# OminiX-ai/OminiX-MLX

Measured on AMD Instinct MI355X. Metric: decode_tokens_per_sec, higher is better.
Workload: dtype bf16

## Files before the change

ominix-mlx_amd/csrc/attn.hpp:

```cpp
#pragma once
#include "common.hpp"

namespace omx {

struct AttnDecodeArgs {
    const bf16_t* q;
    const bf16_t* k;
    const bf16_t* v;
    int64_t kv_batch_stride, kv_head_stride;
    int B, H, Hkv, Tk;
    float scale;
    int mask_mode;
    const void* mask;
    int nsplit;
    float* ws_o;
    float* ws_ml;
    bf16_t* out;
    int64_t q_bs, q_hs;
    int causal_tail;
};

constexpr int kAttnTraceWords = 16;
struct AttnStepArgs {
    const bf16_t* qkv;
    bf16_t* k;
    bf16_t* v;
    int64_t kv_head_stride;
    int H, Hkv, cap;
    float scale, eps;
    const bf16_t* q_norm_w;
    const bf16_t* k_norm_w;
    const float* rope_cur;
    const int* pos_ptr;
    const unsigned* seq_ptr;
    unsigned tag_mul, tag_add;
    int chunk;
    int nsplit;
    uint64_t* ws;
    bf16_t* out;
    unsigned* abort_flag;
    unsigned long long* trace;
    const bf16_t* o_w;
    const bf16_t* o_resid;
    bf16_t* o_out;
    float* o_out_f32;
    int o_rows;
    int o_rpw, o_nhi;
    uint64_t* xg;
    const uint32_t* o_wq;
    const uint32_t* o_sb;
    int o_group;
    int f16;
    const bf16_t* gu_gate;
    const bf16_t* gu_up;
    const bf16_t* gu_norm_w;
    bf16_t* gu_out;
    int gu_rows;
    uint64_t* hg;
};
bool attn_step_oproj_ok(int H, int Hkv, int D, int nsplit, int o_rows);
bool attn_step_gateup_ok(int H, int Hkv, int D, int nsplit, int o_rows, int gu_rows);
bool attn_step_oproj_q4_ok(int H, int Hkv, int D, int nsplit, int o_rows, int group);
int attn_step_block_tokens(int D);
void attn_step_plan(int tk_max, int Hkv, int G, int D, int* chunk, int* nsplit);
size_t attn_step_ws_granules(int H, int D);
int launch_attn_step(const AttnStepArgs& a, int D, hipStream_t s);

size_t attn_decode_ws_bytes(int BH, int nsplit, int D);
int decode_nsplit(int Tk, int BHkv);
int launch_attn_decode(const AttnDecodeArgs& a, int D, hipStream_t s);

}
```

ominix-mlx_amd/csrc/attn_step.hip:

```cpp
#include <algorithm>

#include "attn.hpp"
#include "act16.hpp"
#include "gemv_parts.hpp"
#include "granule.hpp"
#include "launch_timing.hpp"

namespace omx {

namespace {

constexpr int kBlock = 512;
constexpr int kWaves = 8;
constexpr unsigned kSpinLimit = 1u << 15;

template <int N>
__device__ __forceinline__ float swap_halves(float v) {
    if (N == 16) return dpp_f<0x128>(v);
    return dpp_f<0x1B>(dpp_f<kDppHalfMirror>(v));
}

template <bool F16 = false>
__device__ __forceinline__ void unpack8(const u32x4 r, float (&x)[8]) {
#pragma unroll
    for (int e = 0; e < 4; ++e) {
        x[2 * e] = Act16<F16>::lo(r[e]);
        x[2 * e + 1] = Act16<F16>::hi(r[e]);
    }
}

template <int D, int NB, bool F16 = false>
__device__ __forceinline__ void gather_head(const AttnStepArgs& a, const uint64_t* base, int n_active, unsigned tag, int lane,
                                            int dim, bf16_t* out, uint64_t* xg_head) {
    constexpr int STRIDE = D + 2;
    unsigned long long ml0 = 0, ml1 = 0, og[NB][16];
    bool ok_ml = false, ok_b[NB];
#pragma unroll
    for (int b = 0; b < NB; ++b) ok_b[b] = b * 16 >= n_active;
    const int sl = min(lane, n_active - 1);
    for (unsigned spins = 0;; ++spins) {
        if (!ok_ml) {
            ml0 = ld_granule(base + (size_t)sl * STRIDE + D);
            ml1 = ld_granule(base + (size_t)sl * STRIDE + D + 1);
        }
#pragma unroll
        for (int b = 0; b < NB; ++b) {
            if (ok_b[b]) continue;
#pragma unroll
            for (int j = 0; j < 16; ++j) og[b][j] = ld_granule(base + (size_t)min(b * 16 + j, n_active - 1) * STRIDE + dim);
        }
        bool all = true;
        if (!ok_ml) ok_ml = __all((unsigned)(ml0 >> 32) == tag && (unsigned)(ml1 >> 32) == tag);
        all = ok_ml;
#pragma unroll
        for (int b = 0; b < NB; ++b) {
            if (!ok_b[b]) {
                bool ok = true;
#pragma unroll
                for (int j = 0; j < 16; ++j) ok &= (unsigned)(og[b][j] >> 32) == tag;
                ok_b[b] = __all(ok);
            }
            all = all && ok_b[b];
        }
        if (all) break;
        if (spins >= kSpinLimit) {
            if (lane == 0) __hip_atomic_store(a.abort_flag, 1u, __ATOMIC_RELAXED, __HIP_MEMORY_SCOPE_AGENT);
            break;
        }
        __builtin_amdgcn_s_sleep(1);
    }
    const float m = lane < n_active ? __uint_as_float((unsigned)ml0) : -INFINITY;
    const float l = lane < n_active ? __uint_as_float((unsigned)ml1) : 0.f;
    const float M = wave_max(m);
    const float f = (m == -INFINITY) ? 0.f : __expf(m - M);
    const float L = wave_sum(f * l);
    float acc = 0.f;
#pragma unroll
    for (int b = 0; b < NB; ++b) {
        if (b * 16 >= n_active) break;
#pragma unroll
        for (int j = 0; j < 16; ++j)
            acc = fmaf(readlane_f(f, b * 16 + j), __uint_as_float((unsigned)og[b][j]), acc);
    }
    const bf16_t r = Act16<F16>::bits(acc / L);
    out[dim] = r;
    if (xg_head) {
        const float nb = dpp_f<kDppXor1>(bf16_to_f32(r));
        if (!(lane & 1)) st_granule_u32(xg_head + dim / 2, tag, (unsigned)r | ((unsigned)f32_to_bf16(nb) << 16));
    }
}

typedef __attribute__((ext_vector_type(2))) __bf16 bf16x2_t;
typedef __attribute__((ext_vector_type(2))) float f32x2;

typedef __attribute__((ext_vector_type(8))) __bf16 bf16x8_t;
__device__ __forceinline__ float dot8_bf16(const u32x4 a, const u32x4 b) {
    const bf16x8_t A = __builtin_bit_cast(bf16x8_t, a), B = __builtin_bit_cast(bf16x8_t, b);
    float d = 0.f;
    d = __builtin_amdgcn_fdot2_f32_bf16(__builtin_shufflevector(A, A, 0, 1), __builtin_shufflevector(B, B, 0, 1), d, false);
    d = __builtin_amdgcn_fdot2_f32_bf16(__builtin_shufflevector(A, A, 2, 3), __builtin_shufflevector(B, B, 2, 3), d, false);
    d = __builtin_amdgcn_fdot2_f32_bf16(__builtin_shufflevector(A, A, 4, 5), __builtin_shufflevector(B, B, 4, 5), d, false);
    d = __builtin_amdgcn_fdot2_f32_bf16(__builtin_shufflevector(A, A, 6, 7), __builtin_shufflevector(B, B, 6, 7), d, false);
    return d;
}

constexpr int kKU = 3;

template <bool F16>
__device__ __forceinline__ float dot8_16(const u32x4 a, const u32x4 b) {
    if constexpr (!F16) return dot8_bf16(a, b);
    float d = 0.f;
#pragma unroll
    for (int e = 0; e < 4; ++e) d = Act16<true>::dot2(a[e], b[e], d);
    return d;
}

__device__ __forceinline__ float dot8_chain(const u32x4 w, const u32x4 xp, float acc) {
#pragma unroll
    for (int i = 0; i < 4; ++i) {
        acc = fmaf(bf16lo(w[i]), bf16lo(xp[i]), acc);
        acc = fmaf(bf16hi(w[i]), bf16hi(xp[i]), acc);
    }
    return acc;
}

constexpr int kORows = 4;

constexpr int kGuBlockPairs = 48, kGuHidden = 4096, kGuNV = kGuHidden / 512;
enum { kGuTicket = 0, kGuReduced = 1, kGuWords = 4 };

__device__ __forceinline__ int gateup_claim(int* sm_gu, int lane) {
    int t = 0;
    if (lane == 0) t = __hip_atomic_fetch_add(sm_gu + kGuTicket, 1, __ATOMIC_RELAXED, __HIP_MEMORY_SCOPE_WORKGROUP);
    return __builtin_amdgcn_readfirstlane(t);
}

__device__ __forceinline__ void gateup_issue(const AttnStepArgs& a, u32x4 (*w)[kGuNV], int pair, int lane) {
    const u32x4* g = reinterpret_cast<const u32x4*>(a.gu_gate + (size_t)pair * kGuHidden);
    const u32x4* u = reinterpret_cast<const u32x4*>(a.gu_up + (size_t)pair * kGuHidden);
#pragma unroll
    for (int j = 0; j < kGuNV; ++j) {
        w[0][j] = ld_nt(g + j * 64 + lane);
        w[1][j] = ld_nt(u + j * 64 + lane);
    }
    __builtin_amdgcn_sched_barrier(0);
}

template <int NVW>
__device__ __forceinline__ void oproj_await_vector(const AttnStepArgs& a, u32x4* sm_x, unsigned tag, int lane, int wave) {
    asm volatile("s_waitcnt vmcnt(0)" ::: "memory");
    if (wave == 0) {
        constexpr int SEGS = NVW * 8;
        const uint64_t* probe = a.xg + (size_t)min(lane, SEGS - 1) * 32 + 31;
        for (unsigned spins = 0; spins < kSpinLimit; ++spins) {
            const unsigned long long g = ld_granule(probe);
            if (__all((unsigned)(g >> 32) == tag)) break;
            __builtin_amdgcn_s_sleep(4);
        }
    }
    __syncthreads();
    constexpr int GP = (NVW + 1) / 2;
    static_assert((NVW * 256) % GP == 0, "a thread takes all of its granules or none");
    bool done = (int)threadIdx.x * GP >= NVW * 256;
    unsigned* sx = reinterpret_cast<unsigned*>(sm_x);
    for (unsigned spins = 0;; ++spins) {
        if (!done) {
            unsigned long long g[GP];
#pragma unroll
            for (int i = 0; i < GP; ++i) g[i] = ld_granule(a.xg + (size_t)threadIdx.x * GP + i);
            bool ok = true;
#pragma unroll
            for (int i = 0; i < GP; ++i) ok &= (unsigned)(g[i] >> 32) == tag;
            if (ok) {
#pragma unroll
                for (int i = 0; i < GP; ++i) sx[threadIdx.x * GP + i] = (unsigned)g[i];
                done = true;
            }
        }
        if (__syncthreads_and(done)) break;
        if (spins >= kSpinLimit) {
            if (threadIdx.x == 0) __hip_atomic_store(a.abort_flag, 1u, __ATOMIC_RELAXED, __HIP_MEMORY_SCOPE_AGENT);
            break;
        }
        __builtin_amdgcn_s_sleep(2);
    }
}

__device__ __forceinline__ void gateup_reduce(const AttnStepArgs& a, const u32x4 (*w)[kGuNV], const u32x4* xs, int pair, int lane) {
    typedef Act16<false> A;
    float acc[2] = {0.f, 0.f};
#pragma unroll
    for (int j = 0; j < kGuNV; ++j) {
        const u32x4 xp = xs[j * 64 + lane];
        float xf[8];
#pragma unroll
        for (int q = 0; q < 4; ++q) {
            xf[2 * q] = A::lo(xp[q]);
            xf[2 * q + 1] = A::hi(xp[q]);
        }
#pragma unroll
        for (int r = 0; r < 2; ++r) acc[r] = dot8(w[r][j], xf, acc[r]);
    }
#pragma unroll
    for (int r = 0; r < 2; ++r) acc[r] = wave_sum(acc[r]);
    if (lane == 0) a.gu_out[pair] = epi_bits<EPI_SWIGLU, A>(acc[0], acc[1], (bf16_t)0, 0);
}

template <bool TRACE>
__device__ __forceinline__ void gateup_phase(const AttnStepArgs& a, u32x4* xs, float* red, int* sm_gu, const uint16_t* sm_pub, unsigned tag,
                                             int lane, int wave, int pub_row0, int pub_rows, unsigned long long* tr) {
    typedef Act16<false> A;
    const int pair0 = ((int)blockIdx.y * (int)gridDim.x + (int)blockIdx.x) * kGuBlockPairs;
    constexpr int PV = kGuNV * 64 / 256;
    u32x4 nwv[PV];
#pragma unroll
    for (int i = 0; i < PV; ++i) nwv[i] = *(reinterpret_cast<const u32x4*>(a.gu_norm_w) + (threadIdx.x & 255) + i * 256);
    u32x4 wA[2][kGuNV], wB[2][kGuNV];
    int tA = 0, tB;
    if (wave != 0) {
        tA = gateup_claim(sm_gu, lane);
        gateup_issue(a, wA, pair0 + tA, lane);
    }
    lds_barrier();
    if (wave == 0) {
        if (lane < pub_rows / 2) st_granule_u32(a.hg + pub_row0 / 2 + lane, tag, reinterpret_cast<const unsigned*>(sm_pub)[lane]);
        constexpr int GPL = kGuHidden / 2 / 64;
        for (unsigned spins = 0; spins < kSpinLimit; ++spins) {
            const unsigned long long g = ld_granule(a.hg + (size_t)lane * GPL + (GPL - 1));
            if (__all((unsigned)(g >> 32) == tag)) break;
            __builtin_amdgcn_s_sleep(4);
        }
        unsigned long long g[GPL];
#pragma unroll
        for (int i = 0; i < GPL; ++i) g[i] = ld_granule(a.hg + (size_t)i * 64 + lane);
        __builtin_amdgcn_sched_barrier(0);
        lds_barrier();
        tA = gateup_claim(sm_gu, lane);
        gateup_issue(a, wA, pair0 + tA, lane);
        unsigned bad = 0;
#pragma unroll
        for (int i = 0; i < GPL; ++i) bad |= (unsigned)(g[i] >> 32) ^ tag;
        asm volatile("; hidden row: tags read behind the first (gate, up) pair" : "+v"(bad));
        if (!__all(bad == 0)) {
            for (unsigned spins = 0;; ++spins) {
#pragma unroll
                for (int i = 0; i < GPL; ++i) g[i] = ld_granule(a.hg + (size_t)i * 64 + lane);
                bool ok = true;
#pragma unroll
                for (int i = 0; i < GPL; ++i) ok &= (unsigned)(g[i] >> 32) == tag;
                if (__all(ok)) break;
                if (spins >= kSpinLimit) {
                    if (lane == 0) __hip_atomic_store(a.abort_flag, 1u, __ATOMIC_RELAXED, __HIP_MEMORY_SCOPE_AGENT);
                    break;
                }
                __builtin_amdgcn_s_sleep(4);
            }
        }
        unsigned* sx = reinterpret_cast<unsigned*>(xs);
#pragma unroll
        for (int i = 0; i < GPL; ++i) sx[i * 64 + lane] = (unsigned)g[i];
        if (TRACE && lane == 0 && pub_rows > 0) tr[4] = wall_clock64();
        tB = gateup_claim(sm_gu, lane);
    } else {
        lds_barrier();
        tB = gateup_claim(sm_gu, lane);
        gateup_issue(a, wB, pair0 + tB, lane);
    }
    lds_barrier();
    rmsnorm_in_lds<A, PV>(xs, red, nwv, kGuHidden, a.eps, threadIdx.x < 256);
    if (wave == 0) {
        gateup_issue(a, wB, pair0 + tB, lane);
        gateup_reduce(a, wA, xs, pair0 + tA, lane);
        if (TRACE && threadIdx.x == 0) tr[7] = wall_clock64();
        asm volatile("; first pair reduced: wave 0, its second pair just asked for" ::: "memory");
    } else {
        gateup_reduce(a, wA, xs, pair0 + tA, lane);
        asm volatile("; first pair reduced: the second pair came in through the hop" ::: "memory");
    }
    int n_reduced = 1;
    int nA = gateup_claim(sm_gu, lane), nB;
    for (;;) {
        if (nA >= kGuBlockPairs) {
            gateup_reduce(a, wB, xs, pair0 + tB, lane);
            ++n_reduced;
            break;
        }
        tA = nA;
        gateup_issue(a, wA, pair0 + tA, lane);
        nB = gateup_claim(sm_gu, lane);
        gateup_reduce(a, wB, xs, pair0 + tB, lane);
        if (nB >= kGuBlockPairs) {
            gateup_reduce(a, wA, xs, pair0 + tA, lane);
            n_reduced += 2;
            break;
        }
        tB = nB;
        gateup_issue(a, wB, pair0 + tB, lane);
        nA = gateup_claim(sm_gu, lane);
        gateup_reduce(a, wA, xs, pair0 + tA, lane);
        n_reduced += 2;
    }
    if constexpr (TRACE) {
        if (lane == 0) {
            __hip_atomic_fetch_add(sm_gu + kGuReduced, n_reduced, __ATOMIC_RELAXED, __HIP_MEMORY_SCOPE_WORKGROUP);
            if (wave == 0) tr[8] = wall_clock64();
            if (wave == kWaves - 1) tr[9] = wall_clock64();
        }
        lds_barrier();
        if (threadIdx.x == 0) tr[10] = (unsigned long long)sm_gu[kGuReduced];
    }
}

template <int NVW, int R, bool GU = false>
__device__ __forceinline__ void oproj_phase(const AttnStepArgs& a, u32x4* sm_x, unsigned tag, int lane, int wave, int o_row0,
                                            unsigned long long* tr, uint16_t* sm_pub = nullptr, int pub_row0 = 0) {
    u32x4 ow[R][NVW];
#pragma unroll
    for (int r = 0; r < R; ++r) {
        const int row = min(o_row0 + r, a.o_rows - 1);
        const u32x4* p = reinterpret_cast<const u32x4*>(a.o_w + (size_t)row * (NVW * 512));
#pragma unroll
        for (int j = 0; j < NVW; ++j) ow[r][j] = __builtin_nontemporal_load(p + j * 64 + lane);
    }
    bf16_t o_res[R];
#pragma unroll
    for (int r = 0; r < R; ++r) o_res[r] = a.o_resid[min(o_row0 + r, a.o_rows - 1)];
    __builtin_amdgcn_sched_barrier(0);
    oproj_await_vector<NVW>(a, sm_x, tag, lane, wave);
    if (tr && threadIdx.x == 0) tr[5] = wall_clock64();
    float acc[R];
#pragma unroll
    for (int r = 0; r < R; ++r) acc[r] = 0.f;
#pragma unroll
    for (int j = 0; j < NVW; ++j) {
        const u32x4 xp = sm_x[j * 64 + lane];
#pragma unroll
        for (int r = 0; r < R; ++r) acc[r] = dot8_chain(ow[r][j], xp, acc[r]);
    }
#pragma unroll
    for (int r = 0; r < R; ++r) acc[r] = wave_sum(acc[r]);
    if (lane == 0) {
#pragma unroll
        for (int r = 0; r < R; ++r)
            if (o_row0 + r < a.o_rows) {
                if (a.o_out_f32) a.o_out_f32[o_row0 + r] = acc[r];
                else {
                    const bf16_t hb = f32_to_bf16(bf16_to_f32(o_res[r]) + round_bf16(acc[r]));
                    a.o_out[o_row0 + r] = hb;
                    if (GU) sm_pub[o_row0 + r - pub_row0] = hb;
                }
            }
    }
    if (tr && threadIdx.x == 0) tr[6] = wall_clock64();
}


template <int NVW, int R>
__device__ __forceinline__ void oproj_phase_q4(const AttnStepArgs& a, u32x4* sm_x, float* sm_xsum, unsigned tag, int lane, int wave,
                                               int o_row0, unsigned long long* tr) {
    static_assert(NVW % 4 == 0, "K must be a multiple of 2048");
    constexpr int ST = NVW / 4;
    u32x4 ow[R][ST];
    uint32_t sbv[R][ST];
    const int words_per_row = NVW * 64, groups_per_row = NVW * 512 / a.o_group;
#pragma unroll
    for (int r = 0; r < R; ++r) {
        const int row = min(o_row0 + r, a.o_rows - 1);
        const uint32_t* p = a.o_wq + (size_t)row * words_per_row;
        const uint32_t* psb = a.o_sb + (size_t)row * groups_per_row;
#pragma unroll
        for (int st = 0; st < ST; ++st) {
            const int chunk = st * 64 + lane;
            ow[r][st] = __builtin_nontemporal_load(reinterpret_cast<const u32x4*>(p + (size_t)chunk * 4));
            sbv[r][st] = psb[chunk * 32 / a.o_group];
        }
    }
    bf16_t o_res[R];
#pragma unroll
    for (int r = 0; r < R; ++r) o_res[r] = a.o_resid[min(o_row0 + r, a.o_rows - 1)];
    __builtin_amdgcn_sched_barrier(0);
    oproj_await_vector<NVW>(a, sm_x, tag, lane, wave);
    if ((int)threadIdx.x < NVW * 64) {
        const u32x4 o = sm_x[threadIdx.x];
        u32x4 t;
        t[0] = __builtin_amdgcn_perm(o[1], o[0], 0x05040100u); t[1] = __builtin_amdgcn_perm(o[3], o[2], 0x05040100u);
        t[2] = __builtin_amdgcn_perm(o[1], o[0], 0x07060302u); t[3] = __builtin_amdgcn_perm(o[3], o[2], 0x07060302u);
        sm_x[threadIdx.x] = t;
        float sv = 0.f;
#pragma unroll
        for (int q = 0; q < 4; ++q) sv += bf16lo(o[q]) + bf16hi(o[q]);
        sv += dpp_f<kDppXor1>(sv);
        sv += dpp_f<kDppXor2>(sv);
        if ((threadIdx.x & 3) == 0) sm_xsum[threadIdx.x >> 2] = sv;
    }
    __syncthreads();
    if (tr && threadIdx.x == 0) tr[5] = wall_clock64();
    float acc[R];
#pragma unroll
    for (int r = 0; r < R; ++r) acc[r] = 0.f;
#pragma unroll
    for (int st = 0; st < ST; ++st) {
        const int chunk = st * 64 + lane;
        uint32_t xp[16];
#pragma unroll
        for (int j = 0; j < 4; ++j) {
            const u32x4 xv = sm_x[chunk * 4 + j];
#pragma unroll
            for (int q = 0; q < 4; ++q) xp[j * 4 + q] = xv[q];
        }
        const float xsm = sm_xsum[chunk];
#pragma unroll
        for (int r = 0; r < R; ++r) {
            float d = 0.f;
            const float scl = bf16lo(sbv[r][st]);
            float bia = bf16hi(sbv[r][st]);
#pragma unroll
            for (int wi = 0; wi < 4; ++wi) {
                const uint32_t wdw = ow[r][st][wi];
                const uint32_t lo = wdw & 0x0F0F0F0Fu, hi = (wdw >> 4) & 0x0F0F0F0Fu;
                const uint32_t c43 = 0x43434343u;
                const uint32_t q0 = __builtin_amdgcn_perm(c43, lo, 0x04010400u), q1 = __builtin_amdgcn_perm(c43, lo, 0x04030402u);
                const uint32_t q2 = __builtin_amdgcn_perm(c43, hi, 0x04010400u), q3 = __builtin_amdgcn_perm(c43, hi, 0x04030402u);
                d = __builtin_amdgcn_fdot2_f32_bf16(__builtin_bit_cast(bf16x2_t, xp[wi * 4 + 0]), __builtin_bit_cast(bf16x2_t, q0), d, false);
                d = __builtin_amdgcn_fdot2_f32_bf16(__builtin_bit_cast(bf16x2_t, xp[wi * 4 + 1]), __builtin_bit_cast(bf16x2_t, q1), d, false);
                d = __builtin_amdgcn_fdot2_f32_bf16(__builtin_bit_cast(bf16x2_t, xp[wi * 4 + 2]), __builtin_bit_cast(bf16x2_t, q2), d, false);
                d = __builtin_amdgcn_fdot2_f32_bf16(__builtin_bit_cast(bf16x2_t, xp[wi * 4 + 3]), __builtin_bit_cast(bf16x2_t, q3), d, false);
            }
            bia = fmaf(-128.0f, scl, bia);
            acc[r] = fmaf(scl, d, acc[r]);
            acc[r] = fmaf(bia, xsm, acc[r]);
        }
    }
#pragma unroll
    for (int r = 0; r < R; ++r) acc[r] = wave_sum(acc[r]);
    if (lane == 0) {
#pragma unroll
        for (int r = 0; r < R; ++r)
            if (o_row0 + r < a.o_rows) a.o_out[o_row0 + r] = f32_to_bf16(bf16_to_f32(o_res[r]) + round_bf16(acc[r]));
    }
    if (tr && threadIdx.x == 0) tr[6] = wall_clock64();
}


template <int D, int GT, bool TRACE, int NVW, bool F16 = false, bool GU = false>
__global__ __launch_bounds__(kBlock, 1) void attn_step_kernel(const AttnStepArgs a) {
    static_assert(!F16 || NVW == 0, "the O projection rides in the launch for bfloat16 models only");
    static_assert(!GU || (NVW == kGuNV && D == 128), "gate/up follows the bf16 O projection of hidden 4096 only");
    typedef Act16<F16> A16;
    constexpr int LPR = D / 8;
    constexpr int TPW = 64 / LPR;
    constexpr bool QO = NVW >= 100;
    constexpr int NV = QO ? NVW - 100 : NVW;
    constexpr bool OPROJ = NV > 0;
    extern __shared__ __attribute__((aligned(16))) unsigned char smem[];
    float* sm_o = reinterpret_cast<float*>(smem);
    float* sm_m = sm_o + kWaves * TPW * GT * D;
    float* sm_l = sm_m + kWaves * GT;
    u32x4* sm_q = reinterpret_cast<u32x4*>(sm_l + kWaves * GT);
    u32x4* sm_x = sm_q + (GT + 1) * LPR;
    float* sm_xsum = reinterpret_cast<float*>(sm_x + NV * 64);
    int* sm_gu = reinterpret_cast<int*>(sm_x + NV * 64);

    const int lane = threadIdx.x & 63;
    const int wave = threadIdx.x >> 6;
    const int c = lane % LPR;
    const int sg = lane / LPR;
    const int kvh = blockIdx.x, split = blockIdx.y;
    const int G = a.H / a.Hkv;
    unsigned long long* tr = TRACE ? a.trace + ((size_t)split * a.Hkv + kvh) * kAttnTraceWords : nullptr;
    if (TRACE && threadIdx.x == 0) tr[0] = wall_clock64();
    if constexpr (GU) {
        if (threadIdx.x < kGuWords) sm_gu[threadIdx.x] = 0;
    }

    bf16_t* Kb = a.k + (size_t)kvh * a.kv_head_stride;
    bf16_t* Vb = a.v + (size_t)kvh * a.kv_head_stride;
    const int t_begin = split * a.chunk;
    const int n_units = a.chunk / TPW;

    const bf16_t* kraw = a.qkv + (size_t)a.H * D + (size_t)kvh * D;
    const bool does_q = wave < GT, does_k = wave == GT % kWaves;
    const bf16_t* my_raw = does_q ? a.qkv + (size_t)(kvh * G + min(wave, G - 1)) * D : kraw;
    const u32x4 raw0 = *reinterpret_cast<const u32x4*>(my_raw + c * 8);
    const u32x4 raw1 = *reinterpret_cast<const u32x4*>(kraw + c * 8);
    const u32x4 vnew = *reinterpret_cast<const u32x4*>(kraw + (size_t)a.Hkv * D + c * 8);
    const int i0 = (c % (LPR / 2)) * 8;
    const f32x4* cp = reinterpret_cast<const f32x4*>(a.rope_cur + i0);
    const f32x4* sp = reinterpret_cast<const f32x4*>(a.rope_cur + D / 2 + i0);
    const f32x4 c0 = cp[0], c1 = cp[1], s0 = sp[0], s1 = sp[1];
    u32x4 wq_raw = {0, 0, 0, 0}, wk_raw = {0, 0, 0, 0};
    if (a.q_norm_w) {
        wq_raw = *reinterpret_cast<const u32x4*>(a.q_norm_w + c * 8);
        wk_raw = *reinterpret_cast<const u32x4*>(a.k_norm_w + c * 8);
    }
    u32x4 kr[kKU], vr[kKU];
    auto issue_kv = [&](int u0) {
#pragma unroll
        for (int u = 0; u < kKU; ++u) {
            const int tc = min(t_begin + (u0 + u * kWaves) * TPW + sg, a.cap - 1);
            kr[u] = *reinterpret_cast<const u32x4*>(Kb + (size_t)tc * D + c * 8);
            vr[u] = *reinterpret_cast<const u32x4*>(Vb + (size_t)tc * D + c * 8);
        }
    };
    issue_kv(wave);
    const int pos = *a.pos_ptr;
    const unsigned tag = *a.seq_ptr * a.tag_mul + a.tag_add;

    {
        float cs[8], sn[8];
#pragma unroll
        for (int e = 0; e < 4; ++e) {
            cs[e] = c0[e]; cs[4 + e] = c1[e];
            sn[e] = s0[e]; sn[4 + e] = s1[e];
        }
        const bool first_half = c < LPR / 2;
        auto norm_rope = [&](const u32x4 raw, const u32x4 w_raw) -> u32x4 {
            float x[8], w[8];
            unpack8<F16>(raw, x);
            unpack8<F16>(w_raw, w);
            float ss = 0.f;
#pragma unroll
            for (int e = 0; e < 8; ++e) ss = fmaf(x[e], x[e], ss);
            ss = group_sum<LPR>(ss);
            const float rstd = a.q_norm_w ? 1.0f / sqrtf(ss / (float)D + a.eps) : 1.0f;
            float y[8];
#pragma unroll
            for (int e = 0; e < 8; ++e) {
                const float xn = a.q_norm_w ? A16::rnd(x[e] * rstd * w[e]) : x[e];
                const float other = swap_halves<LPR>(xn);
                y[e] = first_half ? xn * cs[e] - other * sn[e] : other * sn[e] + xn * cs[e];
            }
            u32x4 out;
#pragma unroll
            for (int e = 0; e < 4; ++e) out[e] = A16::pack(y[2 * e], y[2 * e + 1]);
            return out;
        };
        if (does_q && sg == 0) sm_q[wave * LPR + c] = norm_rope(raw0, wq_raw);
        if (does_k && sg == 0) sm_q[GT * LPR + c] = norm_rope(does_q ? raw1 : raw0, wk_raw);
    }
    asm volatile("s_waitcnt lgkmcnt(0)\n\ts_barrier" ::: "memory");
    u32x4 q[GT];
#pragma unroll
    for (int g = 0; g < GT; ++g) q[g] = sm_q[g * LPR + c];
    const u32x4 knew = sm_q[GT * LPR + c];

    const int Tk = pos + 1;
    const int n_active = (Tk + a.chunk - 1) / a.chunk;
    const int t_end = min(Tk, t_begin + a.chunk);
    const bool active = split < n_active;
    if (TRACE && threadIdx.x == 0) tr[1] = wall_clock64();

    float m[GT], l[GT];
    f32x2 o[GT][4];
#pragma unroll
    for (int g = 0; g < GT; ++g) {
        m[g] = -INFINITY;
        l[g] = 0.f;
#pragma unroll
        for (int e = 0; e < 4; ++e) o[g][e] = f32x2{0.f, 0.f};
    }
    auto round = [&](const int u0) {
        float s[kKU][GT];
        f32x2 vf[kKU][4];
#pragma unroll
        for (int u = 0; u < kKU; ++u) {
            const int unit = u0 + u * kWaves;
            const int tok = t_begin + unit * TPW + sg;
            const bool live = unit < n_units && tok < t_end;
            u32x4 kp = kr[u], vp = vr[u];
            if (tok == pos && unit < n_units) {
                kp = knew;
                vp = vnew;
                *reinterpret_cast<u32x4*>(Kb + (size_t)pos * D + c * 8) = kp;
                *reinterpret_cast<u32x4*>(Vb + (size_t)pos * D + c * 8) = vp;
            }
#pragma unroll
            for (int e = 0; e < 4; ++e)
                vf[u][e] = live ? f32x2{A16::lo(vp[e]), A16::hi(vp[e])} : f32x2{0.f, 0.f};
#pragma unroll
            for (int g = 0; g < GT; ++g) {
                const float d = group_sum<LPR>(dot8_16<F16>(q[g], kp)) * a.scale;
                s[u][g] = live ? d : -INFINITY;
            }
        }
        if (u0 + kWaves * kKU < n_units && t_begin + (u0 + kWaves * kKU) * TPW < t_end) issue_kv(u0 + kWaves * kKU);
#pragma unroll
        for (int g = 0; g < GT; ++g) {
            float mx = s[0][g];
#pragma unroll
            for (int u = 1; u < kKU; ++u) mx = fmaxf(mx, s[u][g]);
            float wmx = readlane_f(mx, 0);
#pragma unroll
            for (int r = 1; r < TPW; ++r) wmx = fmaxf(wmx, readlane_f(mx, r * LPR));
            const float mn = fmaxf(m[g], wmx);
            const float alpha = (mn == -INFINITY) ? 1.f : __expf(m[g] - mn);
            m[g] = mn;
            l[g] *= alpha;
            const f32x2 al = {alpha, alpha};
#pragma unroll
            for (int e = 0; e < 4; ++e) o[g][e] *= al;
#pragma unroll
            for (int u = 0; u < kKU; ++u) {
                const float p = (mn == -INFINITY) ? 0.f : __expf(s[u][g] - mn);
                l[g] += p;
                const f32x2 pp = {p, p};
#pragma unroll
                for (int e = 0; e < 4; ++e) o[g][e] = __builtin_elementwise_fma(pp, vf[u][e], o[g][e]);
            }
        }
    };
    if (wave < n_units && t_begin + wave * TPW < t_end) round(wave);
    for (int u0 = wave + kWaves * kKU; u0 < n_units && t_begin + u0 * TPW < t_end; u0 += kWaves * kKU) round(u0);
    if (TRACE && threadIdx.x == 0) tr[2] = wall_clock64();

    if (active) {
#pragma unroll
        for (int g = 0; g < GT; ++g) {
            float* dst = sm_o + (((size_t)(wave * TPW + sg) * GT + g) * D + c * 8);
            *reinterpret_cast<f32x4*>(dst) = f32x4{o[g][0][0], o[g][0][1], o[g][1][0], o[g][1][1]};
            *reinterpret_cast<f32x4*>(dst + 4) = f32x4{o[g][2][0], o[g][2][1], o[g][3][0], o[g][3][1]};
            float lw = readlane_f(l[g], 0);
#pragma unroll
            for (int r = 1; r < TPW; ++r) lw += readlane_f(l[g], r * LPR);
            if (lane == 0) {
                sm_m[wave * GT + g] = m[g];
                sm_l[wave * GT + g] = lw;
            }
        }
        __syncthreads();
        if (TRACE && !GU && threadIdx.x == 0) tr[7] = wall_clock64();
        for (int idx = threadIdx.x; idx < G * D; idx += kBlock) {
            const int g = idx / D, d = idx % D;
            float M = sm_m[g];
#pragma unroll
            for (int w = 1; w < kWaves; ++w) M = fmaxf(M, sm_m[w * GT + g]);
            float L = 0.f, O = 0.f;
#pragma unroll
            for (int w = 0; w < kWaves; ++w) {
                const float mw = sm_m[w * GT + g];
                const float f = (mw == -INFINITY) ? 0.f : __expf(mw - M);
                float ow = 0.f;
#pragma unroll
                for (int r = 0; r < TPW; ++r) ow += sm_o[((size_t)(w * TPW + r) * GT + g) * D + d];
                L = fmaf(f, sm_l[w * GT + g], L);
                O = fmaf(f, ow, O);
            }
            uint64_t* gr = a.ws + ((size_t)(kvh * G + g) * a.nsplit + split) * (D + 2);
            st_granule(gr + d, tag, O);
            if (d == 0) {
                st_granule(gr + D, tag, M);
                st_granule(gr + D + 1, tag, L);
            }
        }
    }
    if (TRACE && threadIdx.x == 0) tr[3] = wall_clock64();

    if (OPROJ && split >= G) {
        const int g = ((split - G) * (int)gridDim.x + kvh) * kWaves + wave;
        const bool hi = g < a.o_nhi;
        const int rows = hi ? a.o_rpw : a.o_rpw - 1;
        const int o_row0 = hi ? g * a.o_rpw : a.o_nhi * a.o_rpw + (g - a.o_nhi) * (a.o_rpw - 1);
        unsigned long long* otr = TRACE ? tr : nullptr;
        if constexpr (GU) {
            auto row0_of = [&](int w) { return w < a.o_nhi ? w * a.o_rpw : a.o_nhi * a.o_rpw + (w - a.o_nhi) * (a.o_rpw - 1); };
            const int pub_row0 = row0_of(g - wave), pub_rows = row0_of(g - wave + kWaves) - pub_row0;
            uint16_t* sm_pub = reinterpret_cast<uint16_t*>(sm_l);
            if (rows == 2) oproj_phase<NV, 2, true>(a, sm_x, tag, lane, wave, o_row0, otr, sm_pub, pub_row0);
            else oproj_phase<NV, 3, true>(a, sm_x, tag, lane, wave, o_row0, otr, sm_pub, pub_row0);
            gateup_phase<TRACE>(a, sm_x, sm_m, sm_gu, sm_pub, tag, lane, wave, pub_row0, pub_rows, otr);
            return;
        } else
        if constexpr (QO) {
            if (rows <= 1) oproj_phase_q4<NV, 1>(a, sm_x, sm_xsum, tag, lane, wave, o_row0, otr);
            else if (rows == 2) oproj_phase_q4<NV, 2>(a, sm_x, sm_xsum, tag, lane, wave, o_row0, otr);
            else if (rows == 3) oproj_phase_q4<NV, 3>(a, sm_x, sm_xsum, tag, lane, wave, o_row0, otr);
            else oproj_phase_q4<NV, 4>(a, sm_x, sm_xsum, tag, lane, wave, o_row0, otr);
        } else {
            if (rows <= 1) oproj_phase<(NV > 0 ? NV : 1), 1>(a, sm_x, tag, lane, wave, o_row0, otr);
            else if (rows == 2) oproj_phase<(NV > 0 ? NV : 1), 2>(a, sm_x, tag, lane, wave, o_row0, otr);
            else if (rows == 3) oproj_phase<(NV > 0 ? NV : 1), 3>(a, sm_x, tag, lane, wave, o_row0, otr);
            else oproj_phase<(NV > 0 ? NV : 1), 4>(a, sm_x, tag, lane, wave, o_row0, otr);
        }
        return;
    }

    if (split < G && wave < D / 64) {
        const int head = kvh * G + split;
        const uint64_t* base = a.ws + (size_t)head * a.nsplit * (D + 2);
        bf16_t* out = a.out + (size_t)head * D;
        const int dim = wave * 64 + lane;
        const int nb = (a.nsplit + 15) / 16;
        uint64_t* xg_head = OPROJ ? a.xg + (size_t)head * (D / 2) : nullptr;
        if (nb <= 1) gather_head<D, 1, F16>(a, base, n_active, tag, lane, dim, out, xg_head);
        else if (nb == 2) gather_head<D, 2, F16>(a, base, n_active, tag, lane, dim, out, xg_head);
        else gather_head<D, 3, F16>(a, base, n_active, tag, lane, dim, out, xg_head);
        if (TRACE && threadIdx.x == 0) tr[4] = wall_clock64();
    }
    if constexpr (GU) {
        lds_barrier();
        gateup_phase<TRACE>(a, sm_x, sm_m, sm_gu, nullptr, tag, lane, wave, 0, 0, TRACE ? tr : nullptr);
    }
}

}

int attn_step_block_tokens(int D) { return 64 / (D / 8); }

constexpr int kMaxSplits = 48;
void attn_step_plan(int tk_max, int Hkv, int G, int D, int* chunk, int* nsplit) {
    const int unit = attn_step_block_tokens(D);
    int target = std::max(1, std::min(kMaxSplits, 256 / std::max(Hkv, 1)));
    if (const char* v = getenv("OMX_ATTN_STEP_SPLITS")) target = std::max(1, std::min(kMaxSplits, atoi(v)));
    int ch = unit * ((tk_max + unit * target - 1) / (unit * target));
    if (ch < unit) ch = unit;
    int ns = (tk_max + ch - 1) / ch;
    if (ns < G) ns = G;
    *chunk = ch;
    *nsplit = ns;
}

size_t attn_step_ws_granules(int H, int D) { return (size_t)H * kMaxSplits * (D + 2); }

static int oproj_rows_per_wave(int H, int Hkv, int nsplit, int o_rows) {
    const int waves = (Hkv * nsplit - H) * kWaves;
    return waves > 0 ? (o_rows + waves - 1) / waves : 1 << 20;
}
bool attn_step_oproj_ok(int H, int Hkv, int D, int nsplit, int o_rows) {
    const int K = H * D, nvw = K / 512;
    return K % 512 == 0 && (nvw == 1 || nvw == 2 || nvw == 4 || nvw == 7 || nvw == 8) && oproj_rows_per_wave(H, Hkv, nsplit, o_rows) <= kORows;
}

bool attn_step_oproj_q4_ok(int H, int Hkv, int D, int nsplit, int o_rows, int group) {
    const int K = H * D;
    return (K == 2048 || K == 4096) && (group == 32 || group == 64 || group == 128) && attn_step_oproj_ok(H, Hkv, D, nsplit, o_rows);
}

bool attn_step_gateup_ok(int H, int Hkv, int D, int nsplit, int o_rows, int gu_rows) {
    const int blocks = Hkv * nsplit, waves = (blocks - H) * kWaves;
    if (D != 128 || H * D != kGuHidden || o_rows != kGuHidden || H / std::max(Hkv, 1) != 4 || blocks != 256) return false;
    if (gu_rows != blocks * kGuBlockPairs || !attn_step_oproj_ok(H, Hkv, D, nsplit, o_rows)) return false;
    return oproj_rows_per_wave(H, Hkv, nsplit, o_rows) == 3 && (o_rows - waves * 2) % kWaves == 0;
}

int launch_attn_step(const AttnStepArgs& a_in, int D, hipStream_t s) {
    AttnStepArgs a = a_in;
    const int G = a.H / a.Hkv;
    OMX_REQUIRE(a.H % a.Hkv == 0 && G >= 1 && G <= 8, "decode attention: %d query heads over %d KV heads unsupported (group of at most 8)", a.H, a.Hkv);
    OMX_REQUIRE(a.nsplit >= G && a.nsplit <= kMaxSplits && a.chunk > 0 && a.chunk % attn_step_block_tokens(D) == 0 && a.Hkv * a.nsplit <= 256,
                "decode attention: bad split plan (chunk %d, %d splits, group %d, %d kv heads)", a.chunk, a.nsplit, G, a.Hkv);
    OMX_REQUIRE(a.ws && a.rope_cur && a.pos_ptr && a.seq_ptr && a.abort_flag && a.tag_mul > a.tag_add - 1u && a.tag_add >= 1u,
                "decode attention: missing step state");
    int nvw = 0;
    const bool qo = a.o_wq != nullptr;
    if (qo)
        OMX_REQUIRE(!a.o_w && a.o_sb && a.o_out && !a.o_out_f32 && attn_step_oproj_q4_ok(a.H, a.Hkv, D, a.nsplit, a.o_rows, a.o_group),
                    "decode attention + packed O projection: shape does not qualify (H*D = %d, group %d)", a.H * D, a.o_group);
    if (a.o_w || qo) {
        OMX_REQUIRE(a.o_resid && (a.o_out || a.o_out_f32) && a.xg && attn_step_oproj_ok(a.H, a.Hkv, D, a.nsplit, a.o_rows),
                    "decode attention + O projection: shape does not qualify (H*D = %d, %d rows, %d blocks)", a.H * D, a.o_rows, a.Hkv * a.nsplit);
        nvw = a.H * D / 512;
        a.o_rpw = oproj_rows_per_wave(a.H, a.Hkv, a.nsplit, a.o_rows);
        const int waves = (a.Hkv * a.nsplit - a.H) * kWaves;
        a.o_nhi = a.o_rpw > 1 ? a.o_rows - waves * (a.o_rpw - 1) : waves;
    }
    if (a.gu_gate)
        OMX_REQUIRE(a.o_w && a.o_out && !a.o_out_f32 && !a.f16 && a.gu_up && a.gu_norm_w && a.gu_out && a.hg &&
                        attn_step_gateup_ok(a.H, a.Hkv, D, a.nsplit, a.o_rows, a.gu_rows),
                    "decode attention + gate/up: shape does not qualify (%d blocks, %d O rows, %d pairs)", a.Hkv * a.nsplit, a.o_rows, a.gu_rows);
    const dim3 grid(a.Hkv, a.nsplit), block(kBlock);
    const int gt = G <= 1 ? 1 : G <= 2 ? 2 : G <= 4 ? 4 : 8;
#define OMX_ATTN_LAUNCH(DD, GG, TT, NN)                                                                                  \
    {                                                                                                                    \
        if (shmem > 48 * 1024)                                                                                           \
            OMX_HIP_CHECK(hipFuncSetAttribute((const void*)attn_step_kernel<DD, GG, TT, NN>,                            \
                                              hipFuncAttributeMaxDynamicSharedMemorySize, (int)shmem));                  \
        OMX_LAUNCH_TIMED((attn_step_kernel<DD, GG, TT, NN>), grid, block, shmem, s, a);                                  \
        OMX_LAUNCH_CHECK();                                                                                              \
        return 0;                                                                                                        \
    }
#define OMX_ATTN_LAUNCH_GU(TT)                                                                                           \
    {                                                                                                                    \
        OMX_HIP_CHECK(hipFuncSetAttribute((const void*)attn_step_kernel<128, 4, TT, kGuNV, false, true>,                 \
                                          hipFuncAttributeMaxDynamicSharedMemorySize, (int)shmem));                      \
        OMX_LAUNCH_TIMED((attn_step_kernel<128, 4, TT, kGuNV, false, true>), grid, block, shmem, s, a);                  \
        OMX_LAUNCH_CHECK();                                                                                              \
        return 0;                                                                                                        \
    }
#define OMX_ATTN_STEP_CASE(DD, GG)                                                                                       \
    if (D == DD && gt == GG) {                                                                                           \
        const size_t shmem = ((size_t)kWaves * (64 / (DD / 8)) * GG * DD + 2 * kWaves * GG) * sizeof(float) +            \
                             (size_t)(GG + 1) * (DD / 8) * 16 + (size_t)nvw * 64 * 16 + (qo ? (size_t)nvw * 64 : 0) +    \
                             (a.gu_gate ? kGuWords * sizeof(int) : 0);                                                   \
        if (a.gu_gate) {                            \
            if constexpr (DD == 128 && GG == 4) {                                                                        \
                if (a.trace) OMX_ATTN_LAUNCH_GU(true)                                                                    \
                OMX_ATTN_LAUNCH_GU(false)                                                                                \
            }                                                                                                            \
            return set_error("decode attention + gate/up: no instantiation for head_dim %d, group %d", DD, GG);         \
        }                                                                                                                \
        if (a.trace && !qo) {                           \
            if (nvw == 0) OMX_ATTN_LAUNCH(DD, GG, true, 0)                                                               \
            if (nvw == 8) OMX_ATTN_LAUNCH(DD, GG, true, 8)                                                               \
            return set_error("decode attention: no traced instantiation for H*D = %d", a.H * DD);                       \
        }                                                                                                                \
        if (qo) {                                                                                                        \
            if (nvw == 4) OMX_ATTN_LAUNCH(DD, GG, false, 104)                                                            \
            OMX_ATTN_LAUNCH(DD, GG, false, 108)                                                                          \
        }                                                                                                                \
        if (a.f16) {    \
            if constexpr (DD == 128) {                                                                                   \
                if (nvw == 0) {                                                                                          \
                    if (shmem > 48 * 1024)                                                                               \
                        OMX_HIP_CHECK(hipFuncSetAttribute((const void*)attn_step_kernel<DD, GG, false, 0, true>,        \
                                                          hipFuncAttributeMaxDynamicSharedMemorySize, (int)shmem));      \
                    OMX_LAUNCH_TIMED((attn_step_kernel<DD, GG, false, 0, true>), grid, block, shmem, s, a);              \
                    OMX_LAUNCH_CHECK();                                                                                  \
                    return 0;                                                                                            \
                }                                                                                                        \
            }                                                                                                            \
            return set_error("decode attention: float16 models take head_dim 128 without the O projection in the launch"); \
        }                                                                                                                \
        if (nvw == 0) OMX_ATTN_LAUNCH(DD, GG, false, 0)                                                                  \
        if (nvw == 1) OMX_ATTN_LAUNCH(DD, GG, false, 1)                                                                  \
        if (nvw == 2) OMX_ATTN_LAUNCH(DD, GG, false, 2)                                                                  \
        if (nvw == 4) OMX_ATTN_LAUNCH(DD, GG, false, 4)                                                                  \
        if (nvw == 7) OMX_ATTN_LAUNCH(DD, GG, false, 7)                                                                  \
        OMX_ATTN_LAUNCH(DD, GG, false, 8)                                                                                \
    }
    OMX_ATTN_STEP_CASE(128, 1) OMX_ATTN_STEP_CASE(128, 2) OMX_ATTN_STEP_CASE(128, 4) OMX_ATTN_STEP_CASE(128, 8)
    OMX_ATTN_STEP_CASE(64, 1) OMX_ATTN_STEP_CASE(64, 2) OMX_ATTN_STEP_CASE(64, 4) OMX_ATTN_STEP_CASE(64, 8)
#undef OMX_ATTN_STEP_CASE
#undef OMX_ATTN_LAUNCH_GU
#undef OMX_ATTN_LAUNCH
    return set_error("decode attention: head_dim %d unsupported (64 or 128)", D);
}

}
```

ominix-mlx_amd/csrc/engine.hip:

```cpp
#include "engine_model.hpp"

namespace omx {
namespace {

__global__ void rope_table_kernel(float* cos_t, float* sin_t, int cap, int half, double neg_log_base_over_half,
                                  double scale) {
    const int idx = blockIdx.x * blockDim.x + threadIdx.x;
    if (idx >= cap * half) return;
    const int t = idx / half, i = idx % half;
    const double ang = ((double)t * scale) * exp((double)i * neg_log_base_over_half);
    double s, c;
    sincos(ang, &s, &c);
    cos_t[idx] = (float)c;
    sin_t[idx] = (float)s;
}


}
}

extern "C" {

int omx_qwen3_create(omx_qwen3* out, const omx_qwen3_config* cfg) {
    OMX_REQUIRE(out && cfg, "omx_qwen3_create: null argument");
    const omx_qwen3_config& c = *cfg;
    OMX_REQUIRE(c.tp_size >= 1 && c.tp_rank >= 0 && c.tp_rank < c.tp_size, "InvalidConfig: tp rank %d of %d", c.tp_rank, c.tp_size);
    OMX_REQUIRE(c.hidden_size > 0 && c.hidden_size % 64 == 0, "InvalidConfig: hidden_size %d must be a multiple of 64", c.hidden_size);
    OMX_REQUIRE(c.head_dim == 64 || c.head_dim == 128, "InvalidConfig: head_dim %d (64 or 128 supported)", c.head_dim);
    OMX_REQUIRE(c.num_attention_heads % c.num_key_value_heads == 0, "InvalidConfig: heads %d not a multiple of kv heads %d", c.num_attention_heads, c.num_key_value_heads);
    OMX_REQUIRE(c.num_attention_heads % c.tp_size == 0 && c.intermediate_size % c.tp_size == 0 && c.vocab_size % c.tp_size == 0,
                "InvalidConfig: heads %d / intermediate %d / vocab %d must divide by tp_size %d", c.num_attention_heads, c.intermediate_size, c.vocab_size, c.tp_size);
    OMX_REQUIRE(c.num_key_value_heads >= c.tp_size ? c.num_key_value_heads % c.tp_size == 0
                    : (c.tp_size % c.num_key_value_heads == 0 &&
                       (c.num_attention_heads / c.num_key_value_heads) % (c.tp_size / c.num_key_value_heads) == 0),
                "InvalidConfig: %d kv heads cannot be split or replicated over tp_size %d", c.num_key_value_heads, c.tp_size);
    OMX_REQUIRE(c.quant_bits == 0 || c.quant_bits == 2 || c.quant_bits == 3 || c.quant_bits == 4 || c.quant_bits == 5 || c.quant_bits == 6 ||
                    c.quant_bits == 8, "InvalidConfig: quantization bits %d (0 = bf16, 2, 3, 4, 5, 6, 8)", c.quant_bits);
    OMX_REQUIRE(!quant_chunked(c.quant_bits) || (c.num_experts == 0 && c.tp_size <= 1 && c.ep_size <= 1),
                "InvalidConfig: %d-bit quantization runs on dense single-rank models (num_experts %d, tp_size %d, ep_size %d; experts and "
                "tensor / expert parallelism take bits 4 or 8)", c.quant_bits, c.num_experts, c.tp_size, c.ep_size);
    omx_qwen3 m = new omx_qwen3_();
    m->cfg = c;
    if (m->cfg.rope_scale == 0.f) m->cfg.rope_scale = 1.f;
    if (m->cfg.ep_size < 1) m->cfg.ep_size = 1;
    if (m->cfg.quant_bits && m->cfg.quant_group == 0) m->cfg.quant_group = 64;
    OMX_REQUIRE(!m->cfg.quant_bits || m->cfg.quant_group == 32 || m->cfg.quant_group == 64 || m->cfg.quant_group == 128,
                "InvalidConfig: quantization group_size %d (32, 64, 128)", m->cfg.quant_group);
    OMX_REQUIRE(!m->cfg.quant_scales_f16 || (m->cfg.quant_bits && m->cfg.head_dim == 128),
                "InvalidConfig: a float16 checkpoint (quantization scales_dtype float16) runs as a packed model with head_dim 128");
    OMX_REQUIRE(!c.float16_weights || !c.quant_bits,
                "InvalidConfig: float16_weights marks a dense checkpoint (quant_bits 0, got %d); a packed float16 checkpoint sets quant_scales_f16", c.quant_bits);
    OMX_REQUIRE(!c.float16_weights || c.num_experts == 0, "InvalidConfig: float16_weights with experts (dense float16 MoE is not supported)");
    OMX_REQUIRE(!c.float16_weights || (c.tp_size <= 1 && m->cfg.ep_size <= 1),
                "InvalidConfig: float16_weights under tensor / expert parallelism (tp_size %d, ep_size %d) is not supported", c.tp_size, m->cfg.ep_size);
    OMX_REQUIRE(!c.float16_weights || !c.attention_bias, "InvalidConfig: float16_weights with attention_bias (dense float16 Qwen2) is not supported");
    OMX_REQUIRE(!c.float16_weights || c.head_dim == 128, "InvalidConfig: float16_weights needs head_dim 128 (got %d)", c.head_dim);
    m->f16 = c.quant_scales_f16 || c.float16_weights;
    m->H = c.num_attention_heads / c.tp_size;
    m->Hkv = c.num_key_value_heads >= c.tp_size ? c.num_key_value_heads / c.tp_size : 1;
    m->I = c.intermediate_size / c.tp_size;
    m->V = c.vocab_size / c.tp_size;
    OMX_REQUIRE(c.num_experts > 0 || m->I % 64 == 0, "InvalidConfig: per-rank intermediate %d must be a multiple of 64", m->I);
    OMX_REQUIRE(!c.quant_bits || (c.hidden_size % 512 == 0 && (m->H * c.head_dim) % 512 == 0 && (c.num_experts > 0 || m->I % 512 == 0)),
                "InvalidConfig: quantized checkpoints need hidden %d, attention width %d and intermediate %d to be multiples of 512", c.hidden_size, m->H * c.head_dim, m->I);
    OMX_REQUIRE(!c.attention_bias || !c.quant_bits, "InvalidConfig: attention_bias (Qwen2) runs on bf16 checkpoints");
    const int step = 256;
    m->cap = ((c.max_context > 0 ? c.max_context : 4096) + step - 1) / step * step;
    OMX_HIP_CHECK(hipStreamCreateWithFlags(&m->stream, hipStreamNonBlocking));
    OMX_HIP_CHECK(hipEventCreate(&m->ev0));
    OMX_HIP_CHECK(hipEventCreate(&m->ev1));
    const int D = c.head_dim, L = c.num_hidden_layers;
    m->kcache.resize(L);
    m->vcache.resize(L);
    for (int l = 0; l < L; ++l) {
        if (dev_alloc(m, &m->kcache[l], (size_t)m->Hkv * m->cap * D)) return 1;
        if (dev_alloc(m, &m->vcache[l], (size_t)m->Hkv * m->cap * D)) return 1;
    }
    if (dev_alloc(m, &m->rope_cos, (size_t)m->cap * D / 2) || dev_alloc(m, &m->rope_sin, (size_t)m->cap * D / 2)) return 1;
    {
        const int n = m->cap * D / 2;
        rope_table_kernel<<<(n + 255) / 256, 256, 0, m->stream>>>(m->rope_cos, m->rope_sin, m->cap, D / 2,
                                                                  -log((double)m->cfg.rope_theta) / (double)(D / 2),
                                                                  (double)m->cfg.rope_scale);
        OMX_LAUNCH_CHECK();
    }
    if (c.num_experts > 0) {
        OMX_REQUIRE(c.tp_size == 1 || (c.ep_size <= 1 && c.moe_intermediate_size % ((c.quant_bits ? 512 : 64) * c.tp_size) == 0),
                    "InvalidConfig: expert tensor parallelism (tp_size %d with experts) needs ep_size 1 and moe_intermediate_size %d divisible by %d * tp_size",
                    c.tp_size, c.moe_intermediate_size, c.quant_bits ? 512 : 64);
        m->moe_I = c.moe_intermediate_size / c.tp_size;
        OMX_REQUIRE(c.ep_size <= 1 || (c.ep_rank >= 0 && c.ep_rank < c.ep_size && c.num_experts % c.ep_size == 0),
                    "InvalidConfig: expert parallel rank %d of %d over %d experts", c.ep_rank, c.ep_size, c.num_experts);
        OMX_REQUIRE(!c.quant_bits || c.moe_intermediate_size % 512 == 0, "InvalidConfig: quantised experts need moe_intermediate_size %% 512 == 0 (%d)", c.moe_intermediate_size);
        OMX_REQUIRE(c.num_experts_per_tok >= 1 && c.num_experts_per_tok <= c.num_experts && c.moe_intermediate_size > 0 &&
                        c.moe_intermediate_size % 64 == 0 && (c.moe_mode == 0 || c.moe_mode == 1) && (c.tp_size > 1 || m->H * D >= c.hidden_size),
                    "InvalidConfig: experts %d top-%d moe_intermediate_size %d mode %d", c.num_experts, c.num_experts_per_tok,
                    c.moe_intermediate_size, c.moe_mode);
        size_t need = 0;
        omx_moe_workspace_bytes(m->cap, c.hidden_size, c.moe_intermediate_size, c.num_experts, c.num_experts_per_tok, &need);
        void* ws = nullptr;
        if (get_workspace(&ws, need)) return 1;
        if (c.ep_size > 1 && get_workspace_aux(&ws, need, m->stream)) return 1;
        if (c.tp_size > 1) {
            omx_moe_workspace_bytes(m->cap, c.hidden_size, m->moe_I, c.num_experts, c.num_experts_per_tok, &need);
            if (get_workspace_aux(&ws, need, m->stream)) return 1;
        }
        if (dev_alloc(m, &m->moe_xn, (size_t)c.hidden_size) || dev_alloc(m, &m->moe_out, (size_t)c.hidden_size)) return 1;
        if (c.tp_size > 1 && (dev_alloc(m, &m->moe_y, (size_t)c.num_experts_per_tok * c.hidden_size) ||
                              dev_alloc(m, &m->moe_inds, (size_t)c.num_experts_per_tok) || dev_alloc(m, &m->moe_scores, (size_t)c.num_experts_per_tok)))
            return 1;
    }
    if (dev_alloc(m, &m->rope_cur, (size_t)D) || dev_alloc(m, &m->attn_gran, attn_step_ws_granules(m->H, D)) ||
        dev_alloc(m, &m->attn_xg, (size_t)m->H * D / 2 + 8) || dev_alloc(m, &m->chain_gran, (size_t)c.hidden_size / 2 + 8) ||
        dev_alloc(m, &m->gateup_gran, (size_t)c.hidden_size / 2 + 8))
        return 1;
    if (dev_alloc(m, &m->step_seq, 16) || dev_alloc(m, &m->wait_abort, 16)) return 1;
    {
        int dev = 0;
        hipDeviceProp_t prop;
        OMX_HIP_CHECK(hipGetDevice(&dev));
        OMX_HIP_CHECK(hipGetDeviceProperties(&prop, dev));
        m->cus = prop.multiProcessorCount;
        if (c.num_experts == 0 && !c.quant_bits && dev_alloc(m, &m->se_gran, step_engine_granules(c.hidden_size, m->H, m->Hkv, D, m->I))) return 1;
    }
    if (dev_alloc(m, &m->st, 1) || dev_alloc(m, &m->out_ring, (size_t)m->ring_cap) ||
        dev_alloc(m, &m->h, (size_t)c.hidden_size) || dev_alloc(m, &m->h2, (size_t)c.hidden_size) ||
        dev_alloc(m, &m->qkv, (size_t)(m->H + 2 * m->Hkv) * D) || dev_alloc(m, &m->attn_out, (size_t)m->H * D) ||
        dev_alloc(m, &m->act, (size_t)m->I) || dev_alloc(m, &m->logits, (size_t)m->V) ||
        dev_alloc(m, &m->partial_a, (size_t)c.hidden_size) || dev_alloc(m, &m->partial_b, (size_t)c.hidden_size) ||
        dev_alloc(m, &m->argmax_key, 1))
        return 1;
    if (c.num_experts > 0 && dev_alloc(m, &m->moe_partials, (size_t)c.num_experts_per_tok * c.hidden_size)) return 1;
    m->prompt_cap = m->cap;
    if (dev_alloc(m, &m->prompt_dev, (size_t)m->prompt_cap + 1)) return 1;
    m->n_argmax_partials = m->cfg.quant_bits ? qgemv_grid(m->V) : gemv_grid(m->V, c.hidden_size, EPI_ARGMAX, 0);
    if (dev_alloc(m, &m->argmax_partials, (size_t)m->n_argmax_partials)) return 1;
    OMX_HIP_CHECK(hipStreamSynchronize(m->stream));
    *out = m;
    return 0;
}

int omx_qwen3_destroy(omx_qwen3 m) {
    if (!m) return 0;
    if (m->stream) (void)hipStreamSynchronize(m->stream);
    drop_graphs(m);
    for (const bf16_t* k : m->sb_keys) quant_unregister_sb(k);
    for (void* p : m->owned) (void)hipFree(p);
    if (m->dq_buf) (void)hipFree(m->dq_buf);
    if (m->dq_slab) (void)hipFree(m->dq_slab);
    if (m->verify_logits) (void)hipFree(m->verify_logits);
    if (m->verify_tokens) (void)hipFree(m->verify_tokens);
    score_release(m);
    if (m->pf_ep_partial) (void)hipFree(m->pf_ep_partial);
    for (bf16_t* p : {m->pf_h, m->pf_h2, m->pf_xn, m->pf_q, m->pf_k, m->pf_v, m->pf_qt, m->pf_attn, m->pf_g, m->pf_u})
        if (p) (void)hipFree(p);
    if (m->ev0) (void)hipEventDestroy(m->ev0);
    if (m->ev1) (void)hipEventDestroy(m->ev1);
    if (m->stream) {
        gemm_release_stream(m->stream);
        workspace_release_stream(m->stream);
        (void)hipStreamDestroy(m->stream);
    }
    delete m;
    return 0;
}

int omx_qwen3_set_comm(omx_qwen3 m, void* comm, void* allreduce_fn) {
    OMX_REQUIRE(m, "omx_qwen3_set_comm: null model");
    OMX_REQUIRE(m->g_full == nullptr && !m->eager, "omx_qwen3_set_comm: communicator must be set before the first step");
    m->comm = comm;
    m->allreduce = (nccl_allreduce_fn)allreduce_fn;
    const bool fused = env_on("OMX_PEER_FUSED");
    m->peer_dev = (allreduce_fn == omx_peer_allreduce_fn() && fused && m->cfg.hidden_size <= kPeerMaxWords)
                      ? static_cast<const PeerDev*>(omx_peer_comm_device(comm)) : nullptr;
    return 0;
}

int omx_qwen3_set_sampler(omx_qwen3 m, float temperature, uint64_t seed) {
    OMX_REQUIRE(m, "omx_qwen3_set_sampler: null model");
    OMX_REQUIRE(temperature >= 0.f && temperature == temperature, "omx_qwen3_set_sampler: temperature %f must be >= 0", (double)temperature);
    if (!m->rng && dev_alloc(m, &m->rng, 4)) return 1;
    if (omx_random_key(m->rng, seed, (omx_stream)m->stream)) return 1;
    OMX_HIP_CHECK(hipStreamSynchronize(m->stream));
    if (temperature != m->temperature) {
        recapture_step(m);
        m->temperature = temperature;
    }
    if (m->filter_on) {
        recapture_step(m);
        m->filter_on = false;
        m->sampling = {temperature, 0, 1.f, 1.f, 0.f};
    }
    return 0;
}

int omx_qwen3_set_sampling(omx_qwen3 m, const omx_sampling* p, uint64_t seed) {
    OMX_REQUIRE(m && p, "omx_qwen3_set_sampling: null argument");
    OMX_REQUIRE(p->temperature >= 0.f && p->temperature == p->temperature, "omx_qwen3_set_sampling: temperature %f must be >= 0", (double)p->temperature);
    OMX_REQUIRE(p->top_k >= 0, "omx_qwen3_set_sampling: top_k %d must be >= 0 (0 = off)", p->top_k);
    OMX_REQUIRE(p->top_p > 0.f && p->top_p <= 1.f, "omx_qwen3_set_sampling: top_p %f must be in (0, 1] (1 = off)", (double)p->top_p);
    OMX_REQUIRE(p->repetition_penalty > 0.f && p->repetition_penalty < INFINITY,
                "omx_qwen3_set_sampling: repetition_penalty %f must be positive (1 = off)", (double)p->repetition_penalty);
    OMX_REQUIRE(fabsf(p->presence_penalty) < INFINITY, "omx_qwen3_set_sampling: presence_penalty %f must be finite (0 = off)", (double)p->presence_penalty);
    const bool on = sampling_penalised(*p) || (p->temperature != 0.f && (p->top_k > 0 || p->top_p < 1.f));
    if (!on) return omx_qwen3_set_sampler(m, p->temperature, seed);
    OMX_REQUIRE(m->cfg.tp_size <= 1 && m->allreduce == nullptr,
                "omx_qwen3_set_sampling: filtered sampling is not supported under tensor parallelism (tp_size %d): each rank holds a "
                "vocabulary shard, the selection would need a histogram all-reduce", m->cfg.tp_size);
    OMX_REQUIRE(env_int("OMX_STEP_ENGINE", 0) <= 0 && env_int("OMX_STEP_AQL", 0) <= 0,
                "omx_qwen3_set_sampling: filtered sampling is not supported with the OMX_STEP_ENGINE / OMX_STEP_AQL step modes");
    OMX_REQUIRE(m->V <= (1 << 23), "omx_qwen3_set_sampling: vocabulary %d exceeds 2^23 entries", m->V);
    if (!m->rng && dev_alloc(m, &m->rng, 4)) return 1;
    if (!m->seen && dev_alloc(m, &m->seen, (size_t)m->V)) return 1;
    if (!m->sel && dev_alloc(m, &m->sel, sample_select_ws_bytes())) return 1;
    if (omx_random_key(m->rng, seed, (omx_stream)m->stream)) return 1;
    if (reset_sampler_history(m)) return 1;
    OMX_HIP_CHECK(hipStreamSynchronize(m->stream));
    recapture_step(m);
    m->temperature = p->temperature;
    m->sampling = *p;
    m->filter_on = true;
    return 0;
}

int omx_qwen3_set_logprobs(omx_qwen3 m, int top_n) {
    OMX_REQUIRE(m, "omx_qwen3_set_logprobs: null model");
    const omx_qwen3_config& c = m->cfg;
    OMX_REQUIRE(top_n < 0 || (c.tp_size <= 1 && c.ep_size <= 1 && m->allreduce == nullptr),
                "omx_qwen3_set_logprobs: tensor / expert parallel models are not supported (tp_size %d, ep_size %d: a rank holds a "
                "vocabulary shard, the row's log-sum-exp would need an all-reduce)", c.tp_size, c.ep_size);
    OMX_REQUIRE(top_n < 0 || !m->f16, "omx_qwen3_set_logprobs: float16 models (float16 weights or float16 triplets) are not supported: the row reduction "
                "reads bfloat16 logits");
    OMX_REQUIRE(top_n >= -1 && top_n <= OMX_LOGPROBS_MAX_TOP && top_n <= m->V,
                "omx_qwen3_set_logprobs: top_n = %d is outside -1..min(%d, V = %d) (-1 = off, 0 = the drawn token only)", top_n,
                OMX_LOGPROBS_MAX_TOP, m->V);
    OMX_REQUIRE(top_n < 0 || (m->V % 8 == 0 && m->V <= (1 << 20)),
                "omx_qwen3_set_logprobs: vocabulary %d must be a multiple of 8 and at most 2^20 (omx_logprob_rows' shapes)", m->V);
    if (top_n >= 0 && !m->lp_ring) {
        uint8_t* scratch = nullptr;
        if (dev_alloc(m, &m->lp_ring, (size_t)m->ring_cap) || dev_alloc(m, &m->top_lp_ring, (size_t)m->ring_cap * OMX_LOGPROBS_MAX_TOP) ||
            dev_alloc(m, &m->top_id_ring, (size_t)m->ring_cap * OMX_LOGPROBS_MAX_TOP) ||
            dev_alloc(m, &scratch, logprob_top_scratch_bytes(1, m->V, OMX_LOGPROBS_MAX_TOP)))
            return 1;
        m->lp_scratch = scratch;
        OMX_HIP_CHECK(hipStreamSynchronize(m->stream));
    }
    if (top_n != m->lp_top) {
        recapture_step(m);
        m->lp_top = top_n;
        m->lp_valid = false;
    }
    return 0;
}

int omx_qwen3_sampler_state(omx_qwen3 m, uint32_t* state2, int set) {
    OMX_REQUIRE(m && state2, "omx_qwen3_sampler_state: null argument");
    OMX_REQUIRE(m->rng, "omx_qwen3_sampler_state: no sampler set (omx_qwen3_set_sampler)");
    if (set) OMX_HIP_CHECK(hipMemcpyAsync(m->rng, state2, 8, hipMemcpyHostToDevice, m->stream));
    else OMX_HIP_CHECK(hipMemcpyAsync(state2, m->rng, 8, hipMemcpyDeviceToHost, m->stream));
    OMX_HIP_CHECK(hipStreamSynchronize(m->stream));
    return 0;
}

int omx_qwen3_encode(omx_qwen3 m, const uint32_t* ids, int n, const uint8_t* attention_mask, const int* tap_layers, int n_taps,
                     void* out_dev) {
    OMX_REQUIRE(m && ids && tap_layers && out_dev, "omx_qwen3_encode: null argument");
    OMX_REQUIRE(n >= 1 && n <= m->cap, "omx_qwen3_encode: %d tokens exceed max_context %d", n, m->cap);
    OMX_REQUIRE(n_taps >= 1 && n_taps <= 16, "omx_qwen3_encode: %d taps (1..16)", n_taps);
    OMX_REQUIRE(m->cfg.tp_size == 1 && !m->allreduce, "omx_qwen3_encode: single-GPU only");
    for (int i = 0; i < n_taps; ++i)
        OMX_REQUIRE(tap_layers[i] >= 0 && tap_layers[i] < m->cfg.num_hidden_layers && (i == 0 || tap_layers[i] > tap_layers[i - 1]),
                    "omx_qwen3_encode: tap layers must be ascending and < %d", m->cfg.num_hidden_layers);
    if (resolve_weights(m)) return 1;
    hipStream_t s = m->stream;
    OMX_HIP_CHECK(hipMemcpyAsync(m->prompt_dev, ids, (size_t)n * 4, hipMemcpyHostToDevice, s));
    bf16_t* mask = nullptr;
    uint8_t* am = nullptr;
    if (attention_mask) {
        OMX_HIP_CHECK(hipMalloc((void**)&mask, (size_t)n * n * 2));
        OMX_HIP_CHECK(hipMalloc((void**)&am, (size_t)n));
        OMX_HIP_CHECK(hipMemcpyAsync(am, attention_mask, (size_t)n, hipMemcpyHostToDevice, s));
        launch_encoder_mask(mask, am, n, s);
    }
    const EncodeOpts enc = {tap_layers, n_taps, (bf16_t*)out_dev, mask};
    OMX_HIP_CHECK(hipEventRecord(m->ev0, s));
    const int rc = prefill_prefix_batched(m, n, 0, &enc);
    OMX_HIP_CHECK(hipEventRecord(m->ev1, s));
    OMX_HIP_CHECK(hipStreamSynchronize(s));
    if (mask) { (void)hipFree(mask); (void)hipFree(am); }
    if (rc) return 1;
    OMX_HIP_CHECK(hipEventElapsedTime(&m->last_prefill_ms, m->ev0, m->ev1));
    return 0;
}

int omx_qwen3_reset(omx_qwen3 m) {
    OMX_REQUIRE(m, "omx_qwen3_reset: null model");
    OMX_HIP_CHECK(hipMemsetAsync(m->st, 0, sizeof(StepState), m->stream));
    m->lp_valid = false;
    if (reset_sampler_history(m)) return 1;
    OMX_HIP_CHECK(hipStreamSynchronize(m->stream));
    return 0;
}

int omx_qwen3_offset(omx_qwen3 m, int* offset) {
    OMX_REQUIRE(m && offset, "omx_qwen3_offset: null argument");
    StepState st;
    if (read_step_state(m, &st)) return 1;
    *offset = st.pos;
    return 0;
}

static int prefill_prompt(omx_qwen3 m, const uint32_t* prompt, int n_prompt, uint32_t* first_token, const RowSpan* span) {
    OMX_REQUIRE(n_prompt >= 1, "omx_qwen3_prefill: empty prompt");
    int off = 0;
    if (omx_qwen3_offset(m, &off)) return 1;
    OMX_REQUIRE(off + n_prompt + 1 <= m->cap, "omx_qwen3_prefill: %d cached + %d prompt tokens exceed max_context %d", off, n_prompt, m->cap);
    for (int i = 0; i < n_prompt; ++i) OMX_REQUIRE(prompt[i] < (uint32_t)m->cfg.vocab_size, "omx_qwen3_prefill: token id %u out of range (vocab %d)", prompt[i], m->cfg.vocab_size);
    OMX_REQUIRE(n_prompt <= m->prompt_cap, "omx_qwen3_prefill: prompt of %d tokens exceeds max_context %d", n_prompt, m->prompt_cap);
    const bool serial_on = env_on("OMX_PREFILL_SERIAL");
    if (span) {
        OMX_REQUIRE(!serial_on, "InvalidConfig: omx_qwen3_prefill_embeds: OMX_PREFILL_SERIAL=1 sends the prompt through the decode step, which "
                    "cannot take embedding rows; unset it");
        OMX_REQUIRE(!env_on("OMX_PREFILL_TAIL_STEP"), "InvalidConfig: omx_qwen3_prefill_embeds: OMX_PREFILL_TAIL_STEP=1 sends the last token through "
                    "the decode step, which cannot take embedding rows; unset it");
        OMX_REQUIRE(n_prompt >= 2, "InvalidConfig: omx_qwen3_prefill_embeds: a one-row prompt goes through the decode step, which cannot take "
                    "embedding rows; pass at least 2 rows");
        OMX_REQUIRE(!(m->f16 && n_prompt <= 16), "InvalidConfig: omx_qwen3_prefill_embeds: a float16 model sends prompts of 16 rows or fewer "
                    "through the decode step, which cannot take embedding rows (%d rows); pass at least 17", n_prompt);
    }
    const bool f16_serial = m->f16 && n_prompt <= 16;
    const bool serial = serial_on || n_prompt < 2 || f16_serial;
    if (prepare_step(m, serial ? off : off + n_prompt - 1)) return 1;
    if (!serial && m->cfg.quant_bits) dq_cache_prepare(m);
    if (!serial && prefill_reserve(m, n_prompt)) return 1;
    OMX_HIP_CHECK(hipMemcpyAsync(m->prompt_dev, prompt, (size_t)n_prompt * 4, hipMemcpyHostToDevice, m->stream));
    if (reset_sampler_history(m)) return 1;
    StepState st;
    if (read_step_state(m, &st)) return 1;
    st.cur_token = prompt[0];
    st.prompt_idx = 0;
    const int count_before = st.out_count;
    OMX_HIP_CHECK(hipEventRecord(m->ev0, m->stream));
    bool batched_head = false;
    if (serial) {
        if (write_step_state(m, st)) return 1;
        for (int i = 0; i < n_prompt - 1; ++i)
            if (run_step(m, false, st.pos + i)) return 1;
    } else {
        const bool tail_step = env_on("OMX_PREFILL_TAIL_STEP");
        const int nb = tail_step ? n_prompt - 1 : n_prompt;
        if (prefill_prefix_batched(m, nb, st.pos, nullptr, !tail_step, false, nullptr, nullptr, span)) return 1;
        st.pos += n_prompt - 1;
        st.prompt_idx = n_prompt - 1;
        st.cur_token = prompt[n_prompt - 1];
        if (write_step_state(m, st)) return 1;
        if (!tail_step) {
            const bool tp = m->allreduce != nullptr && m->cfg.ep_size <= 1;
            if (enqueue_step_tail(m, true, m->pf_h + (size_t)(n_prompt - 1) * m->cfg.hidden_size, nullptr, 0, tp)) return 1;
            batched_head = true;
        }
    }
    if (!batched_head && run_step(m, true, serial ? st.pos + n_prompt - 1 : st.pos)) return 1;
    OMX_HIP_CHECK(hipEventRecord(m->ev1, m->stream));
    OMX_HIP_CHECK(hipMemcpyAsync(first_token, m->out_ring + (count_before % m->ring_cap), 4, hipMemcpyDeviceToHost, m->stream));
    OMX_HIP_CHECK(hipStreamSynchronize(m->stream));
    OMX_HIP_CHECK(hipEventElapsedTime(&m->last_prefill_ms, m->ev0, m->ev1));
    m->lp_valid = m->lp_top >= 0;
    return step_health(m);
}

int omx_qwen3_prefill(omx_qwen3 m, const uint32_t* prompt, int n_prompt, uint32_t* first_token) {
    OMX_REQUIRE(m && prompt && first_token, "omx_qwen3_prefill: null argument");
    return prefill_prompt(m, prompt, n_prompt, first_token, nullptr);
}

int omx_qwen3_prefill_embeds(omx_qwen3 m, const uint32_t* prompt, int n_prompt, const void* rows, omx_dtype rows_dtype, int first_row,
                             int n_rows, uint32_t* first_token) {
    OMX_REQUIRE(m && prompt && first_token, "omx_qwen3_prefill_embeds: null argument");
    OMX_REQUIRE(n_rows >= 0, "omx_qwen3_prefill_embeds: n_rows %d is negative", n_rows);
    if (n_rows == 0) return prefill_prompt(m, prompt, n_prompt, first_token, nullptr);
    OMX_REQUIRE(rows != nullptr, "omx_qwen3_prefill_embeds: null rows with n_rows %d", n_rows);
    OMX_REQUIRE(rows_dtype == OMX_FLOAT32 || rows_dtype == OMX_BFLOAT16 || rows_dtype == OMX_FLOAT16,
                "omx_qwen3_prefill_embeds: rows of dtype %d (float32, bfloat16 or float16)", (int)rows_dtype);
    OMX_REQUIRE(first_row >= 0 && first_row <= n_prompt && n_rows <= n_prompt - first_row,
                "omx_qwen3_prefill_embeds: rows [%d, %d + %d) lie outside the prompt of %d tokens", first_row, first_row, n_rows, n_prompt);
    OMX_REQUIRE(m->allreduce == nullptr && m->cfg.tp_size <= 1 && m->cfg.ep_size <= 1,
                "omx_qwen3_prefill_embeds: tensor-parallel / expert-parallel engines are not supported (single-rank models only)");
    OMX_REQUIRE(m->cfg.num_experts == 0, "omx_qwen3_prefill_embeds: sparse-MoE models are not supported (dense models only)");
    const RowSpan span = {rows, rows_dtype, first_row, n_rows};
    return prefill_prompt(m, prompt, n_prompt, first_token, &span);
}

int omx_qwen3_embed_tokens(omx_qwen3 m, const uint32_t* ids, int n, void* out_rows) {
    OMX_REQUIRE(m && ids && out_rows, "omx_qwen3_embed_tokens: null argument");
    OMX_REQUIRE(n >= 1 && n <= m->prompt_cap, "omx_qwen3_embed_tokens: %d ids (1..%d, the prompt buffer)", n, m->prompt_cap);
    for (int i = 0; i < n; ++i) OMX_REQUIRE(ids[i] < (uint32_t)m->cfg.vocab_size, "omx_qwen3_embed_tokens: token id %u out of range (vocab %d)", ids[i], m->cfg.vocab_size);
    OMX_REQUIRE(m->allreduce == nullptr && m->cfg.tp_size <= 1 && m->cfg.ep_size <= 1,
                "omx_qwen3_embed_tokens: tensor-parallel / expert-parallel engines are not supported (single-rank models only)");
    if (resolve_weights(m)) return 1;
    if (m->cfg.quant_bits && prefill_reserve(m, n, false)) return 1;
    OMX_HIP_CHECK(hipMemcpyAsync(m->prompt_dev, ids, (size_t)n * 4, hipMemcpyHostToDevice, m->stream));
    if (embed_rows(m, (bf16_t*)out_rows, n, false)) return 1;
    OMX_HIP_CHECK(hipStreamSynchronize(m->stream));
    return 0;
}

int omx_qwen3_verify(omx_qwen3 m, const uint32_t* tokens, int n, uint32_t* greedy_out) {
    OMX_REQUIRE(m && tokens && greedy_out, "omx_qwen3_verify: null argument");
    OMX_REQUIRE(n >= 1 && n <= 64, "omx_qwen3_verify: %d tokens (1..64 per call)", n);
    OMX_REQUIRE(!m->filter_on, "omx_qwen3_verify: filtered sampling (top-k / top-p / penalties, omx_qwen3_set_sampling) is on: speculative "
                "verify draws from unfiltered rows; call omx_qwen3_set_sampler first");
    OMX_REQUIRE(m->allreduce == nullptr && m->cfg.tp_size <= 1 && m->cfg.ep_size <= 1,
                "omx_qwen3_verify: tensor / expert parallel models are not supported (single-rank models only)");
    const bool packed = m->cfg.quant_bits != 0;
    OMX_REQUIRE(!m->cfg.float16_weights, "omx_qwen3_verify: dense float16 models (float16_weights) are not supported; speculative verify runs "
                "on bf16 weights or bf16-scale packed weights");
    OMX_REQUIRE(!packed || !m->cfg.quant_scales_f16,
                "omx_qwen3_verify: float16 triplets (scales_dtype float16) are not supported on packed models; bf16 scales only");
    OMX_REQUIRE(!packed || m->cfg.num_experts == 0, "omx_qwen3_verify: packed models with experts (MoE) are not supported; dense models only");
    for (int i = 0; i < n; ++i) OMX_REQUIRE(tokens[i] < (uint32_t)m->cfg.vocab_size, "omx_qwen3_verify: token id %u out of range (vocab %d)", tokens[i], m->cfg.vocab_size);
    StepState st;
    if (read_step_state(m, &st)) return 1;
    OMX_REQUIRE(st.pos + n + 1 <= m->cap, "omx_qwen3_verify: %d cached + %d tokens exceed max_context %d", st.pos, n, m->cap);
    OMX_REQUIRE(n <= m->prompt_cap, "omx_qwen3_verify: %d tokens exceed the prompt buffer", n);
    if (resolve_weights(m)) return 1;
    hipStream_t s = m->stream;
    const int hd = m->cfg.hidden_size, V = m->V;
    if (n > m->verify_cap) {
        OMX_HIP_CHECK(hipStreamSynchronize(s));
        if (m->verify_logits) OMX_HIP_CHECK(hipFree(m->verify_logits));
        if (m->verify_tokens) OMX_HIP_CHECK(hipFree(m->verify_tokens));
        m->verify_logits = nullptr; m->verify_tokens = nullptr; m->verify_cap = 0;
        const int cap = std::max(n, 16);
        OMX_HIP_CHECK(hipMalloc((void**)&m->verify_logits, (size_t)cap * V * sizeof(bf16_t)));
        OMX_HIP_CHECK(hipMalloc((void**)&m->verify_tokens, (size_t)cap * 4));
        m->verify_cap = cap;
    }
    OMX_HIP_CHECK(hipMemcpyAsync(m->prompt_dev, tokens, (size_t)n * 4, hipMemcpyHostToDevice, s));
    if (prefill_prefix_batched(m, n, st.pos, nullptr, true, packed)) return 1;
    if (packed) {
        QGemvArgs a = {};
        a.m[0] = m->q_head; a.m[0].n = V; a.N = V; a.K = hd; a.group = m->q_head.group;
        a.x = m->pf_h; a.norm_w = m->final_norm; a.eps = m->cfg.rms_norm_eps; a.out = m->verify_logits;
        if (packed_rows(a, n, nullptr, m->q_head.bits, PRO_RMSNORM, EPI_STORE, s)) return 1;
    } else {
        if (omx_rms_norm(m->pf_xn, m->pf_h, m->final_norm, n, hd, m->cfg.rms_norm_eps, OMX_BFLOAT16, s)) return 1;
        if (launch_gemm_bf16(m->verify_logits, m->pf_xn, m->lm_head, nullptr, n, V, hd, s)) return 1;
    }
    if (m->temperature == 0.f) {
        if (omx_argmax(m->verify_tokens, m->verify_logits, n, V, OMX_BFLOAT16, s)) return 1;
    } else {
        for (int i = 0; i < n; ++i) {
            if (launch_rng_next(m->rng, s)) return 1;
            if (omx_random_categorical(m->verify_tokens + i, m->verify_logits + (size_t)i * V, 1, V, 1, 1.0f / m->temperature, m->rng + 2,
                                       OMX_BFLOAT16, (omx_stream)s))
                return 1;
        }
    }
    OMX_HIP_CHECK(hipMemcpyAsync(greedy_out, m->verify_tokens, (size_t)n * 4, hipMemcpyDeviceToHost, s));
    OMX_HIP_CHECK(hipStreamSynchronize(s));
    st.pos += n;
    st.cur_token = greedy_out[n - 1];
    if (write_step_state(m, st)) return 1;
    OMX_HIP_CHECK(hipStreamSynchronize(s));
    m->verify_rows = n;
    return 0;
}

int omx_qwen3_verify_logits(omx_qwen3 m, int row, void* host_bf16, int n) {
    OMX_REQUIRE(m && host_bf16, "omx_qwen3_verify_logits: null argument");
    OMX_REQUIRE(row >= 0 && row < m->verify_rows, "omx_qwen3_verify_logits: row %d of %d", row, m->verify_rows);
    OMX_REQUIRE(n == m->V, "omx_qwen3_verify_logits: expected %d entries, got %d", m->V, n);
    OMX_HIP_CHECK(hipMemcpyAsync(host_bf16, m->verify_logits + (size_t)row * m->V, (size_t)n * 2, hipMemcpyDeviceToHost, m->stream));
    OMX_HIP_CHECK(hipStreamSynchronize(m->stream));
    return 0;
}

int omx_qwen3_trim(omx_qwen3 m, int n, uint32_t next_token) {
    OMX_REQUIRE(m, "omx_qwen3_trim: null argument");
    OMX_REQUIRE(!m->filter_on, "omx_qwen3_trim: filtered sampling (top-k / top-p / penalties, omx_qwen3_set_sampling) is on: the token "
                "history on the device cannot be trimmed; call omx_qwen3_set_sampler first");
    OMX_REQUIRE(next_token < (uint32_t)m->cfg.vocab_size, "omx_qwen3_trim: token id %u out of range (vocab %d)", next_token, m->cfg.vocab_size);
    StepState st;
    if (read_step_state(m, &st)) return 1;
    OMX_REQUIRE(n >= 0 && n <= st.pos, "omx_qwen3_trim: cannot drop %d of %d cached tokens", n, st.pos);
    st.pos -= n;
    st.cur_token = next_token;
    if (write_step_state(m, st)) return 1;
    OMX_HIP_CHECK(hipStreamSynchronize(m->stream));
    return 0;
}

int omx_qwen3_dequant_bytes(omx_qwen3 m, size_t* bytes) {
    OMX_REQUIRE(m && bytes, "omx_qwen3_dequant_bytes: null argument");
    *bytes = (m->dq_slab ? m->dq_slab_bytes : 0) + (m->dq_buf ? m->dq_cap * sizeof(bf16_t) : 0);
    return 0;
}

int omx_qwen3_last_prefill_ms(omx_qwen3 m, float* ms) {
    OMX_REQUIRE(m && ms, "omx_qwen3_last_prefill_ms: null argument");
    *ms = m->last_prefill_ms;
    return 0;
}

static int decode_steps(omx_qwen3 m, int n, uint32_t* tokens_out, float* logprobs, uint32_t* top_ids, float* top_logprobs) {
    OMX_REQUIRE(n >= 0 && n <= m->ring_cap, "omx_qwen3_decode: n=%d out of range (1..%d per call)", n, m->ring_cap);
    if (n == 0) return 0;
    StepState st;
    if (read_step_state(m, &st)) return 1;
    if (prepare_step(m, st.pos)) return 1;
    OMX_REQUIRE(st.pos + n <= m->cap, "omx_qwen3_decode: %d cached + %d new tokens exceed max_context %d", st.pos, n, m->cap);
    for (;;) {
        const bool aql = m->aql_full && step_aql_mode(m) && context_bucket(m, st.pos + n) == m->graph_tk_max;
        if (aql) {
            double ms = 0.0;
            if (aql_replay(m->aql_full, n, &ms)) {
                m->aql_disabled = true;
                return 1;
            }
            m->last_decode_ms = (float)ms;
        } else {
            OMX_HIP_CHECK(hipEventRecord(m->ev0, m->stream));
            for (int i = 0; i < n; ++i)
                if (run_step(m, true, st.pos + i)) return 1;
            OMX_HIP_CHECK(hipEventRecord(m->ev1, m->stream));
            OMX_HIP_CHECK(hipStreamSynchronize(m->stream));
            OMX_HIP_CHECK(hipEventElapsedTime(&m->last_decode_ms, m->ev0, m->ev1));
        }
        unsigned gave_up = 0;
        if (step_gave_up(m, &gave_up)) return 1;
        if (!gave_up) break;
        if (step_fallback(m, st)) return step_health(m);
        if (prepare_step(m, st.pos)) return 1;
    }
    std::vector<uint32_t> ring(m->ring_cap);
    OMX_HIP_CHECK(hipMemcpy(ring.data(), m->out_ring, (size_t)m->ring_cap * 4, hipMemcpyDeviceToHost));
    for (int i = 0; i < n; ++i) tokens_out[i] = ring[(st.out_count + i) % m->ring_cap];
    m->lp_valid = m->lp_top >= 0;
    if (!logprobs) return 0;
    const size_t top = (size_t)m->lp_top;
    std::vector<float> lp(m->ring_cap), tlp(top_logprobs ? m->ring_cap * top : 0);
    std::vector<uint32_t> ids(top_ids ? m->ring_cap * top : 0);
    OMX_HIP_CHECK(hipMemcpy(lp.data(), m->lp_ring, lp.size() * 4, hipMemcpyDeviceToHost));
    if (!tlp.empty()) OMX_HIP_CHECK(hipMemcpy(tlp.data(), m->top_lp_ring, tlp.size() * 4, hipMemcpyDeviceToHost));
    if (!ids.empty()) OMX_HIP_CHECK(hipMemcpy(ids.data(), m->top_id_ring, ids.size() * 4, hipMemcpyDeviceToHost));
    for (int i = 0; i < n; ++i) {
        const size_t at = (size_t)((st.out_count + i) % m->ring_cap);
        logprobs[i] = lp[at];
        if (!tlp.empty()) memcpy(top_logprobs + i * top, tlp.data() + at * top, top * 4);
        if (!ids.empty()) memcpy(top_ids + i * top, ids.data() + at * top, top * 4);
    }
    return 0;
}

int omx_qwen3_decode(omx_qwen3 m, int n, uint32_t* tokens_out) {
    OMX_REQUIRE(m && tokens_out, "omx_qwen3_decode: null argument");
    return decode_steps(m, n, tokens_out, nullptr, nullptr, nullptr);
}

int omx_qwen3_decode_logprobs(omx_qwen3 m, int n, uint32_t* tokens_out, float* logprobs, uint32_t* top_ids, float* top_logprobs) {
    OMX_REQUIRE(m && tokens_out && logprobs, "omx_qwen3_decode_logprobs: null argument");
    OMX_REQUIRE(m->lp_top >= 0, "omx_qwen3_decode_logprobs: log-probabilities are off (omx_qwen3_set_logprobs)");
    return decode_steps(m, n, tokens_out, logprobs, top_ids, top_logprobs);
}

int omx_qwen3_last_logprobs(omx_qwen3 m, float* logprob, uint32_t* top_ids, float* top_logprobs) {
    OMX_REQUIRE(m && logprob, "omx_qwen3_last_logprobs: null argument");
    OMX_REQUIRE(m->lp_top >= 0, "omx_qwen3_last_logprobs: log-probabilities are off (omx_qwen3_set_logprobs)");
    OMX_REQUIRE(m->lp_valid, "omx_qwen3_last_logprobs: no token has been sampled since omx_qwen3_set_logprobs / omx_qwen3_reset");
    StepState st;
    if (read_step_state(m, &st)) return 1;
    OMX_REQUIRE(st.out_count >= 1, "omx_qwen3_last_logprobs: no token has been sampled yet");
    const size_t at = (size_t)((st.out_count - 1) % m->ring_cap), top = (size_t)m->lp_top;
    OMX_HIP_CHECK(hipMemcpy(logprob, m->lp_ring + at, 4, hipMemcpyDeviceToHost));
    if (top_ids && top) OMX_HIP_CHECK(hipMemcpy(top_ids, m->top_id_ring + at * top, top * 4, hipMemcpyDeviceToHost));
    if (top_logprobs && top) OMX_HIP_CHECK(hipMemcpy(top_logprobs, m->top_lp_ring + at * top, top * 4, hipMemcpyDeviceToHost));
    return 0;
}

int omx_qwen3_last_logits(omx_qwen3 m, void* host_bf16, int n) {
    OMX_REQUIRE(m && host_bf16, "omx_qwen3_last_logits: null argument");
    OMX_REQUIRE(n == m->V, "omx_qwen3_last_logits: expected %d entries, got %d", m->V, n);
    OMX_HIP_CHECK(hipMemcpyAsync(host_bf16, m->logits, (size_t)n * 2, hipMemcpyDeviceToHost, m->stream));
    OMX_HIP_CHECK(hipStreamSynchronize(m->stream));
    return 0;
}

static void* debug_buffer(omx_qwen3 m, const char* name) {
    void* src = nullptr;
    const std::string s(name);
    if (s == "h") src = m->h;
    else if (s == "h2") src = m->h2;
    else if (s == "qkv") src = m->qkv;
    else if (s == "attn_out") src = m->attn_out;
    else if (s == "act") src = m->act;
    else if (s.rfind("g_", 0) == 0 && m->se_gran) {
        const size_t hd = m->cfg.hidden_size, D = m->cfg.head_dim;
        uint64_t* g = m->se_gran;
        if (s == "g_x") src = g;
        else if (s == "g_x1") src = g + hd / 2;
        else if (s == "g_qkv") src = g + hd;
        else if (s == "g_attn") src = g + hd + (size_t)(m->H + 2 * m->Hkv) * D / 2;
        else if (s == "g_act") src = g + hd + (size_t)(m->H + 2 * m->Hkv) * D / 2 + (size_t)m->H * D / 2;
    }
    else if (s.size() > 1 && (s[0] == 'k' || s[0] == 'v')) {
        const int l = atoi(s.c_str() + 1);
        if (l >= 0 && l < (int)m->kcache.size()) src = s[0] == 'k' ? m->kcache[l] : m->vcache[l];
    }
    return src;
}

int omx_qwen3_debug_read(omx_qwen3 m, const char* name, void* host, size_t n_elems) {
    OMX_REQUIRE(m && name && host, "omx_qwen3_debug_read: null argument");
    const void* src = debug_buffer(m, name);
    OMX_REQUIRE(src != nullptr, "omx_qwen3_debug_read: unknown buffer or layer %s", name);
    OMX_HIP_CHECK(hipMemcpyAsync(host, src, n_elems * 2, hipMemcpyDeviceToHost, m->stream));
    OMX_HIP_CHECK(hipStreamSynchronize(m->stream));
    return 0;
}

int omx_qwen3_debug_write(omx_qwen3 m, const char* name, const void* host, size_t n_elems) {
    OMX_REQUIRE(m && name && host, "omx_qwen3_debug_write: null argument");
    void* dst = debug_buffer(m, name);
    OMX_REQUIRE(dst != nullptr, "omx_qwen3_debug_write: unknown buffer %s", name);
    OMX_HIP_CHECK(hipMemcpyAsync(dst, host, n_elems * 2, hipMemcpyHostToDevice, m->stream));
    OMX_HIP_CHECK(hipStreamSynchronize(m->stream));
    return 0;
}

int omx_qwen3_last_decode_ms(omx_qwen3 m, float* ms) {
    OMX_REQUIRE(m && ms, "omx_qwen3_last_decode_ms: null argument");
    *ms = m->last_decode_ms;
    return 0;
}

int omx_qwen3_stream(omx_qwen3 m, omx_stream* s) {
    OMX_REQUIRE(m && s, "omx_qwen3_stream: null argument");
    *s = (omx_stream)m->stream;
    return 0;
}

int omx_qwen3_debug_trace_step(omx_qwen3 m, unsigned long long* host, size_t n_words, int* blocks) {
    OMX_REQUIRE(m && host && blocks, "omx_qwen3_debug_trace_step: null argument");
    StepState st;
    if (read_step_state(m, &st)) return 1;
    if (prepare_step(m, st.pos)) return 1;
    const size_t per_layer = (size_t)m->attn_nsplit * m->Hkv * kAttnTraceWords, need = per_layer * m->cfg.num_hidden_layers;
    OMX_REQUIRE(n_words >= need, "omx_qwen3_debug_trace_step: buffer of %zu words, need %zu", n_words, need);
    unsigned long long* dev = nullptr;
    OMX_HIP_CHECK(hipMalloc(&dev, need * 8));
    OMX_HIP_CHECK(hipMemsetAsync(dev, 0, need * 8, m->stream));
    m->attn_trace = dev;
    const int rc = enqueue_step(m, true);
    m->attn_trace = nullptr;
    if (!rc) {
        OMX_HIP_CHECK(hipStreamSynchronize(m->stream));
        OMX_HIP_CHECK(hipMemcpy(host, dev, need * 8, hipMemcpyDeviceToHost));
    }
    (void)hipFree(dev);
    *blocks = m->attn_nsplit * m->Hkv;
    return rc ? 1 : step_health(m);
}

int omx_qwen3_time_step_kernels(omx_qwen3 m, int steps, float* us) {
    OMX_REQUIRE(m && us && steps > 0, "omx_qwen3_time_step_kernels: bad arguments");
    OMX_REQUIRE(!m->cfg.quant_bits && m->cfg.num_experts == 0 && m->allreduce == nullptr, "omx_qwen3_time_step_kernels: dense bf16 single-rank models only");
    const int L = m->cfg.num_hidden_layers;
    std::vector<hipEvent_t> ev((size_t)(L * kLayerClasses + 2) * 2);
    for (auto& e : ev) OMX_HIP_CHECK(hipEventCreate(&e));
    double sum[KC_COUNT] = {};
    int rc = 0;
    bool fused_o = false, engine = false, hybrid = false, chain = false;
    const double o_bytes = (double)m->H * m->cfg.head_dim * m->cfg.hidden_size, gu_bytes = 2.0 * m->cfg.hidden_size * m->I;
    const double qkv_bytes = (double)(m->H + 2 * m->Hkv) * m->cfg.head_dim * m->cfg.hidden_size, down_bytes = (double)m->cfg.hidden_size * m->I;
    arm_launch_events(nullptr, nullptr);
    for (int it = 0; it < steps && !rc; ++it) {
        StepState st;
        if (read_step_state(m, &st)) { rc = 1; break; }
        if (st.pos + 1 > m->cap) { set_error("omx_qwen3_time_step_kernels: context full"); rc = 1; break; }
        if (prepare_step(m, st.pos)) { rc = 1; break; }
        fused_o = any_layer_takes_oproj(m);
        engine = step_engine_mode(m) == 1;
        hybrid = step_engine_mode(m) == 2;
        chain = !engine && !hybrid && down_takes_qkv(m);
        m->kernel_events = &ev;
        rc = enqueue_step(m, true);
        m->kernel_events = nullptr;
        if (rc) break;
        OMX_HIP_CHECK(hipStreamSynchronize(m->stream));
        for (int l = (engine ? L : 0); l <= L; ++l)
            for (int k = 0; k < (l == L ? (engine ? 2 : 1) : kLayerClasses); ++k) {
                float ms = 0.f;
                const size_t i = ((size_t)l * kLayerClasses + k) * 2;
                if (l < L && k == KC_O && fused_o) continue;
                if (hybrid && l < L && (k == KC_GATE_UP || (k == KC_DOWN && l != L - 1))) continue;
                if (chain && l > 0 && l < L && k == KC_QKV) continue;
                const bool gateup = l < L && !engine && !hybrid && attention_takes_gateup(m, l);
                if (gateup && k == KC_GATE_UP) continue;
                OMX_HIP_CHECK(hipEventElapsedTime(&ms, ev[i], ev[i + 1]));
                if (gateup && k == KC_ATTN) {
                    const double attn_bytes = 2.0 * m->Hkv * m->cfg.head_dim * (st.pos + 1) + o_bytes;
                    sum[KC_GATE_UP] += ms * 1e3 * (gu_bytes / (gu_bytes + attn_bytes));
                    ms *= (float)(attn_bytes / (gu_bytes + attn_bytes));
                }
                if (chain && l < L - 1 && k == KC_DOWN) {
                    sum[KC_QKV] += ms * 1e3 * (qkv_bytes / (qkv_bytes + down_bytes));
                    ms *= (float)(down_bytes / (qkv_bytes + down_bytes));
                }
                sum[l == L ? (k == 0 ? KC_HEAD : KC_ENGINE) : k] += ms * 1e3;
            }
        rc = step_health(m);
    }
    arm_launch_events(nullptr, nullptr);
    for (auto& e : ev) (void)hipEventDestroy(e);
    if (rc) return 1;
    for (int k = 0; k < KC_COUNT; ++k) us[k] = (float)(sum[k] / ((k == KC_HEAD || k == KC_ENGINE ? 1.0 : (double)L) * steps));
    if (fused_o) us[KC_O] = 0.f;
    return 0;
}

int omx_qwen3_debug_trace_engine(omx_qwen3 m, unsigned long long* host, size_t n_words, int* cus_out) {
    OMX_REQUIRE(m && host && cus_out, "omx_qwen3_debug_trace_engine: null argument");
    StepState st;
    if (read_step_state(m, &st)) return 1;
    if (prepare_step(m, st.pos)) return 1;
    OMX_REQUIRE(step_engine_takes(m), "omx_qwen3_debug_trace_engine: the persistent step is off or the model does not qualify");
    const size_t need = (size_t)m->cus * kStepEngineTraceWords;
    OMX_REQUIRE(n_words >= need, "omx_qwen3_debug_trace_engine: buffer of %zu words, need %zu", n_words, need);
    unsigned long long* dev = nullptr;
    OMX_HIP_CHECK(hipMalloc(&dev, need * 8));
    OMX_HIP_CHECK(hipMemsetAsync(dev, 0, need * 8, m->stream));
    m->se_trace = dev;
    const int rc = enqueue_step(m, true);
    m->se_trace = nullptr;
    if (!rc) {
        OMX_HIP_CHECK(hipStreamSynchronize(m->stream));
        OMX_HIP_CHECK(hipMemcpy(host, dev, need * 8, hipMemcpyDeviceToHost));
    }
    (void)hipFree(dev);
    *cus_out = m->cus;
    return rc ? 1 : step_health(m);
}

int omx_qwen3_decode_path(omx_qwen3 m, int* path) {
    OMX_REQUIRE(m && path, "omx_qwen3_decode_path: null argument");
    *path = m->eager ? 2 : (m->aql_full && step_aql_mode(m)) ? 3 : m->g_full ? 1 : 0;
    *path |= (m->gateup_disabled ? 1 : 0) << 8 | (m->chain_disabled ? 1 : 0) << 9 | (m->se_disabled ? 1 : 0) << 10 | (m->oproj_disabled ? 1 : 0) << 11;
    return 0;
}

int omx_qwen3_step_bytes(omx_qwen3 m, int ctx, double* bytes) {
    OMX_REQUIRE(m && bytes, "omx_qwen3_step_bytes: null argument");
    const omx_qwen3_config& c = m->cfg;
    const double D = c.head_dim, hd = c.hidden_size;
    const double moe_i = c.tp_size > 1 && c.num_experts > 0 ? m->moe_I : c.moe_intermediate_size;
    const double ffn = c.num_experts > 0 ? hd * c.num_experts + 3.0 * hd * moe_i * c.num_experts_per_tok : 3.0 * hd * m->I;
    const double per_layer = hd * m->H * D + 2.0 * hd * m->Hkv * D + m->H * D * hd + ffn;
    const double bpe = c.quant_bits ? c.quant_bits / 8.0 + 4.0 / c.quant_group : 2.0;
    double w = bpe * (c.num_hidden_layers * per_layer + (double)m->V * hd);
    if (c.quant_bits && c.num_experts == 0 && !m->quant_formats.empty()) {
        auto at = [&](const std::string& prefix, double n, double k) {
            const std::pair<int, int> f = quant_format_of(m, prefix);
            return n * k * (f.first / 8.0 + 4.0 / f.second);
        };
        w = at(c.tie_word_embeddings ? "model.embed_tokens" : "lm_head", m->V, hd);
        for (int l = 0; l < c.num_hidden_layers; ++l) {
            const std::string p = "model.layers." + std::to_string(l) + ".";
            w += at(p + "self_attn.q_proj", m->H * D, hd) + at(p + "self_attn.k_proj", m->Hkv * D, hd) + at(p + "self_attn.v_proj", m->Hkv * D, hd) +
                 at(p + "self_attn.o_proj", hd, m->H * D) + at(p + "mlp.gate_proj", m->I, hd) + at(p + "mlp.up_proj", m->I, hd) + at(p + "mlp.down_proj", hd, m->I);
        }
    }
    const double kv = (double)ctx * (2.0 * c.num_hidden_layers * m->Hkv * D * 2.0) + 2.0 * c.num_hidden_layers * m->Hkv * D * 2.0;
    *bytes = w + kv;
    return 0;
}

}
```

ominix-mlx_amd/csrc/engine_model.hpp:

```cpp
#pragma once
#include <math.h>
#include <stdlib.h>
#include <string.h>

#include <algorithm>
#include <map>
#include <string>
#include <vector>

#include "attn.hpp"
#include "workspace.hpp"
#include "step_state.hpp"
#include "gemm.hpp"
#include "gemv.hpp"
#include "random.hpp"
#include "sample_filter.hpp"
#include "logprob.hpp"
#include "prefill.hpp"
#include "quant.hpp"
#include "launch_timing.hpp"
#include "aql_step.hpp"
#include "act16.hpp"
#include "peer.hpp"
#include "step_engine.hpp"
#include <hip/hip_fp16.h>

namespace omx {

typedef int (*nccl_allreduce_fn)(const void*, void*, size_t, int, int, void*, hipStream_t);

constexpr int kNcclFloat32 = 7, kNcclUint64 = 5, kNcclBfloat16 = 9, kNcclSum = 0, kNcclMax = 2;

struct LayerW {
    const bf16_t *q, *k, *v, *o, *gate, *up, *down, *q_norm, *k_norm, *in_ln, *post_ln;
    const bf16_t *moe_gate, *moe_wg, *moe_wu, *moe_wd;
    const bf16_t *q_bias, *k_bias, *v_bias, *qkv_bias;
};

struct LayerQ {
    QMat q, k, v, o, gate, up, down;
    QMat moe_router, moe_g, moe_u, moe_d;
};

enum { KC_QKV = 0, KC_ATTN, KC_O, KC_GATE_UP, KC_DOWN, KC_HEAD, KC_ENGINE, KC_COUNT };
constexpr int kLayerClasses = KC_HEAD;

struct EncodeOpts {
    const int* taps;
    int n_taps;
    bf16_t* out;
    const bf16_t* mask;
};


struct Kv8Layer {
    uint8_t *kq, *vq;
    uint32_t *ksb, *vsb;
};

struct KvSlabs {
    bf16_t* const* k;
    bf16_t* const* v;
    int cap;
    const Kv8Layer* packed = nullptr;
};

struct RaggedRows {
    BatchSlot* slots;
    const int* row_slot;
    bf16_t* const* kbase;
    bf16_t* const* vbase;
    size_t slot_stride;
    int cap, chunk, nsplit, nsplit_cap;
    float *ws_o, *ws_ml;
    int grp_owner[8], grp_shared[8];
    bool grouped;
    int group_min, group_rows;
    const Kv8Layer* kv8;
    size_t sb_stride;
};

struct RowSpan {
    const void* rows;
    omx_dtype dtype;
    int first, n;
};

}

using namespace omx;

struct omx_qwen3_ {
    omx_qwen3_config cfg;
    bool f16 = false;
    int H, Hkv, I, V;
    int cap;
    std::map<std::string, const void*> named;
    std::vector<void*> owned;
    std::vector<LayerW> layers;
    std::vector<LayerQ> qlayers;
    QMat q_embed = {}, q_head = {};
    std::map<std::string, std::pair<int, int>> quant_formats;
    std::vector<const bf16_t*> sb_keys;
    bf16_t* dq_buf = nullptr;
    size_t dq_cap = 0;
    std::map<const uint32_t*, bf16_t*> dq_cache;
    char* dq_slab = nullptr;
    size_t dq_slab_bytes = 0, dq_cache_bytes = 0;
    int dq_cache_mode = -1;
    const bf16_t *embed = nullptr, *final_norm = nullptr, *lm_head = nullptr;
    bool weights_resolved = false;

    hipStream_t stream = nullptr;
    std::vector<bf16_t*> kcache, vcache;
    float *rope_cos = nullptr, *rope_sin = nullptr;
    StepState* st = nullptr;
    uint32_t *out_ring = nullptr, *prompt_dev = nullptr;
    int ring_cap = 4096, prompt_cap = 0;
    bf16_t *h = nullptr, *h2 = nullptr, *qkv = nullptr, *attn_out = nullptr, *act = nullptr, *logits = nullptr;
    bf16_t *moe_xn = nullptr, *moe_out = nullptr;
    float *partial_a = nullptr, *partial_b = nullptr;
    float* moe_partials = nullptr;
    int moe_I = 0;
    float* moe_y = nullptr;
    uint32_t* moe_inds = nullptr;
    bf16_t* moe_scores = nullptr;
    unsigned long long *argmax_partials = nullptr, *argmax_key = nullptr;
    int n_argmax_partials = 0;
    unsigned *step_seq = nullptr, *wait_abort = nullptr;
    float* rope_cur = nullptr;
    uint64_t* attn_gran = nullptr;
    uint64_t* attn_xg = nullptr;
    uint64_t* chain_gran = nullptr;
    uint64_t* gateup_gran = nullptr;
    int attn_chunk = 0, attn_nsplit = 0, graph_tk_max = 0;
    unsigned long long* attn_trace = nullptr;
    bf16_t* verify_logits = nullptr;
    uint32_t* verify_tokens = nullptr;
    int verify_cap = 0, verify_rows = 0;
    bf16_t *score_panel_buf = nullptr, *score_dq = nullptr;
    float *score_part = nullptr, *score_tgt = nullptr, *score_lp = nullptr;
    uint32_t *score_arg = nullptr, *score_targets = nullptr, *score_greedy = nullptr;
    int score_rows = 0, score_panel = 0;
    bool score_dq_on = false;
    hipEvent_t score_ev[3] = {nullptr, nullptr, nullptr};
    float last_score_pass_ms = 0.f, last_score_head_ms = 0.f;
    std::vector<hipEvent_t>* kernel_events = nullptr;

    void* comm = nullptr;
    nccl_allreduce_fn allreduce = nullptr;
    const PeerDev* peer_dev = nullptr;

    float temperature = 0.f;
    uint32_t* rng = nullptr;
    bool filter_on = false;
    omx_sampling sampling = {0.f, 0, 1.f, 1.f, 0.f};
    uint8_t* seen = nullptr;
    uint8_t* sel = nullptr;

    int lp_top = -1;
    float *lp_ring = nullptr, *top_lp_ring = nullptr;
    uint32_t* top_id_ring = nullptr;
    void* lp_scratch = nullptr;
    bool lp_valid = false;

    int pf_cap = 0;
    bf16_t *pf_h = nullptr, *pf_h2 = nullptr, *pf_xn = nullptr, *pf_q = nullptr, *pf_k = nullptr, *pf_v = nullptr,
           *pf_qt = nullptr, *pf_attn = nullptr, *pf_g = nullptr, *pf_u = nullptr;
    float* pf_ep_partial = nullptr;
    int pf_ep_cap = 0;
    float last_prefill_ms = 0.f;

    int cus = 0;
    std::vector<StepEngineLayer> se_layers_host;
    StepEngineLayer* se_layers = nullptr;
    uint64_t* se_gran = nullptr;
    unsigned long long* se_trace = nullptr;
    bool se_disabled = false;
    bool oproj_disabled = false;
    bool chain_disabled = false;
    bool gateup_disabled = false;

    hipGraphExec_t g_full = nullptr, g_nohead = nullptr;
    AqlProgram* aql_full = nullptr;
    bool aql_disabled = false;
    bool eager = false;
    hipEvent_t ev0 = nullptr, ev1 = nullptr;
    float last_decode_ms = 0.f;
};

namespace omx {

inline bool env_on(const char* name, bool dflt = false) {
    const char* e = getenv(name);
    return e ? e[0] == '1' : dflt;
}

inline bool env_off(const char* name) {
    const char* e = getenv(name);
    return e && e[0] == '0';
}

inline int env_int(const char* name, int dflt) {
    const char* e = getenv(name);
    return e ? atoi(e) : dflt;
}

inline bool env_is(const char* name, const char* value) {
    const char* e = getenv(name);
    return e && strcmp(e, value) == 0;
}

#define OMX_QMAT3(q) (q).w, (q).scales, (q).biases
#define OMX_QMOE_ARGS(Q) OMX_QMAT3((Q).moe_router), OMX_QMAT3((Q).moe_g), OMX_QMAT3((Q).moe_u), OMX_QMAT3((Q).moe_d)

template <class T>
inline int dev_alloc(omx_qwen3 m, T** p, size_t n) {
    void* q = nullptr;
    OMX_HIP_CHECK(hipMalloc(&q, n * sizeof(T) + 64));
    OMX_HIP_CHECK(hipMemsetAsync(q, 0, n * sizeof(T) + 64, m->stream));
    *p = (T*)q;
    m->owned.push_back(q);
    return 0;
}

int resolve_weights(omx_qwen3 m);
std::pair<int, int> quant_format_of(omx_qwen3 m, const std::string& prefix);

void drop_graphs(omx_qwen3 m);
void recapture_step(omx_qwen3 m);
int rank_allreduce(omx_qwen3 m, void* buf, size_t n, int dtype, int op);
int allreduce_sum(omx_qwen3 m, float* buf, size_t n);
int read_step_state(omx_qwen3 m, StepState* st);
int write_step_state(omx_qwen3 m, const StepState& st);
int reset_sampler_history(omx_qwen3 m);
bool sampling_penalised(const omx_sampling& p);
bool attention_takes_oproj(omx_qwen3 m, int layer);
bool any_layer_takes_oproj(omx_qwen3 m);
bool down_takes_qkv(omx_qwen3 m);
bool attention_takes_gateup(omx_qwen3 m, int layer);
int step_engine_mode(omx_qwen3 m);
bool step_engine_takes(omx_qwen3 m);
int step_aql_mode(omx_qwen3 m);
int enqueue_step(omx_qwen3 m, bool with_head);
int enqueue_step_tail(omx_qwen3 m, bool with_head, const bf16_t* h, const float* pending, int pending_n, bool tp);
int context_bucket(omx_qwen3 m, int tk);
int prepare_step(omx_qwen3 m, int pos);
int run_step(omx_qwen3 m, bool with_head, int pos);
int step_gave_up(omx_qwen3 m, unsigned* code);
int step_health(omx_qwen3 m);
int step_fallback(omx_qwen3 m, const StepState& st);
int launch_ep_fold(int grid, bf16_t* out, const bf16_t* resid, const float* partial, int64_t n, bool f16, hipStream_t s);

int prefill_reserve(omx_qwen3 m, int T, bool dequant = true);
void dq_cache_prepare(omx_qwen3 m);
int packed_rows(const QGemvArgs& g, int T, bf16_t* const* mout, int bits, int pro, int epi, hipStream_t s);
int prefill_prefix_batched(omx_qwen3 m, int T, int off, const EncodeOpts* enc = nullptr, bool full_last = false, bool packed_rows_pass = false,
                           const KvSlabs* kv = nullptr, const RaggedRows* rag = nullptr, const RowSpan* span = nullptr);
int embed_rows(omx_qwen3 m, bf16_t* out, int T, bool rows_form);
void launch_encoder_mask(bf16_t* mask, const uint8_t* am, int T, hipStream_t s);

void score_release(omx_qwen3 m);

int launch_batch_embed(omx_qwen3 m, const RaggedRows& rag, int T, hipStream_t s);
int launch_batch_scatter(omx_qwen3 m, int layer, const RaggedRows& rag, int T, hipStream_t s);
int launch_batch_attention(omx_qwen3 m, int layer, const RaggedRows& rag, int T, hipStream_t s);
int launch_kv8_rows(const Kv8Layer& L, bf16_t* ks, bf16_t* vs, int Hkv, int D, int cap, int r0, int n, bool pack, hipStream_t s);

}
```

ominix-mlx_amd/csrc/engine_step.hip:

```cpp
#include "engine_model.hpp"

namespace omx {
namespace {

__device__ __forceinline__ void step_begin(const StepState* st, unsigned* seq, float* rope_cur, const float* rope_cos,
                                           const float* rope_sin, int half) {
    if (blockIdx.x != 0) return;
    if (seq && threadIdx.x == 0) *seq += 1u;
    if (rope_cur && (int)threadIdx.x < 2 * half) {
        const int t = threadIdx.x, pos = st->pos;
        rope_cur[t] = t < half ? rope_cos[(size_t)pos * half + t] : rope_sin[(size_t)pos * half + t - half];
    }
}

template <int BITS>
__global__ __launch_bounds__(256) void qembed_kernel(bf16_t* __restrict__ h, const uint32_t* __restrict__ w,
                                                     const bf16_t* __restrict__ scales, const bf16_t* __restrict__ biases,
                                                     const StepState* st, int hidden, int group, unsigned* seq, float* rope_cur,
                                                     const float* rope_cos, const float* rope_sin, int half, bool scales_f16) {
    constexpr int EPW = 32 / BITS;
    step_begin(st, seq, rope_cur, rope_cos, rope_sin, half);
    const size_t row = st->cur_token;
    const int words = hidden / EPW;
    for (int i = blockIdx.x * blockDim.x + threadIdx.x; i < words; i += gridDim.x * blockDim.x) {
        const uint32_t wd = w[row * words + i];
        const int g = i * EPW / group;
        const bf16_t sb16 = scales[row * (hidden / group) + g], bb16 = biases ? biases[row * (hidden / group) + g] : (bf16_t)0;
        const float sc = scales_f16 ? __half2float(__ushort_as_half(sb16)) : bf16_to_f32(sb16);
        const float bi = scales_f16 ? __half2float(__ushort_as_half(bb16)) : bf16_to_f32(bb16);
#pragma unroll
        for (int e = 0; e < EPW; ++e) {
            const float v = (float)((wd >> (e * BITS)) & ((1u << BITS) - 1u)) * sc + bi;
            h[i * EPW + e] = scales_f16 ? Act16<true>::bits(v) : f32_to_bf16(v);
        }
    }
}

template <int BITS>
__global__ __launch_bounds__(256) void qembed_chunk_kernel(bf16_t* __restrict__ h, const uint32_t* __restrict__ w,
                                                           const bf16_t* __restrict__ scales, const bf16_t* __restrict__ biases,
                                                           const StepState* st, int hidden, int group, unsigned* seq, float* rope_cur,
                                                           const float* rope_cos, const float* rope_sin, int half, bool scales_f16) {
    step_begin(st, seq, rope_cur, rope_cos, rope_sin, half);
    const size_t row = st->cur_token;
    const int chunks = hidden / 32;
    for (int i = blockIdx.x * blockDim.x + threadIdx.x; i < chunks; i += gridDim.x * blockDim.x) {
        uint32_t wd[BITS];
#pragma unroll
        for (int k = 0; k < BITS; ++k) wd[k] = w[(row * chunks + i) * BITS + k];
        const int g = i * 32 / group;
        const bf16_t sb16 = scales[row * (hidden / group) + g], bb16 = biases ? biases[row * (hidden / group) + g] : (bf16_t)0;
        const float sc = scales_f16 ? __half2float(__ushort_as_half(sb16)) : bf16_to_f32(sb16);
        const float bi = scales_f16 ? __half2float(__ushort_as_half(bb16)) : bf16_to_f32(bb16);
#pragma unroll
        for (int e = 0; e < 32; ++e) {
            const float v = (float)qfield<BITS>(wd, e) * sc + bi;
            h[i * 32 + e] = scales_f16 ? Act16<true>::bits(v) : f32_to_bf16(v);
        }
    }
}

__global__ void ep_fold_kernel(bf16_t* __restrict__ out, const bf16_t* __restrict__ resid, const float* __restrict__ partial, int64_t n, bool f16 = false) {
    for (int64_t i = blockIdx.x * (int64_t)blockDim.x + threadIdx.x; i < n; i += (int64_t)gridDim.x * blockDim.x) {
        if (f16) out[i] = Act16<true>::bits(Act16<true>::val(resid[i]) + Act16<true>::rnd(partial[i]));
        else out[i] = f32_to_bf16(bf16_to_f32(resid[i]) + round_bf16(partial[i]));
    }
}

__global__ void feed_prompt_kernel(StepState* st, const uint32_t* prompt) {
    st->pos += 1;
    st->prompt_idx += 1;
    st->cur_token = prompt[st->prompt_idx];
}

__global__ __launch_bounds__(256) void sample_finalize_kernel(StepState* st, const unsigned long long* partials,
                                                               int n_partials, uint32_t* out_ring, int ring_cap,
                                                               unsigned long long* key_out) {
    __shared__ unsigned long long red[4];
    unsigned long long best = 0;
    constexpr int kInFlight = 20;
    for (int i0 = threadIdx.x; i0 < n_partials; i0 += 256 * kInFlight) {
        unsigned long long k[kInFlight];
#pragma unroll
        for (int u = 0; u < kInFlight; ++u) k[u] = partials[min(i0 + u * 256, n_partials - 1)];
#pragma unroll
        for (int u = 0; u < kInFlight; ++u) best = k[u] > best ? k[u] : best;
    }
#pragma unroll
    for (int o = 32; o > 0; o >>= 1) {
        const unsigned long long other = __shfl_xor(best, o, 64);
        best = other > best ? other : best;
    }
    if ((threadIdx.x & 63) == 0) red[threadIdx.x >> 6] = best;
    __syncthreads();
    if (threadIdx.x == 0) {
        for (int w = 1; w < 4; ++w) best = red[w] > best ? red[w] : best;
        if (key_out) {
            *key_out = best;
        } else {
            const uint32_t tok = ~(uint32_t)(best & 0xFFFFFFFFull);
            out_ring[st->out_count % ring_cap] = tok;
            st->out_count += 1;
            st->cur_token = tok;
            st->pos += 1;
        }
    }
}

__global__ void apply_token_kernel(StepState* st, const unsigned long long* key, uint32_t* out_ring, int ring_cap) {
    const uint32_t tok = ~(uint32_t)(*key & 0xFFFFFFFFull);
    out_ring[st->out_count % ring_cap] = tok;
    st->out_count += 1;
    st->cur_token = tok;
    st->pos += 1;
}

__global__ __launch_bounds__(256) void embed_kernel(bf16_t* __restrict__ h, const bf16_t* __restrict__ table,
                                                    const StepState* st, int hidden, unsigned* seq, float* rope_cur,
                                                    const float* rope_cos, const float* rope_sin, int half) {
    step_begin(st, seq, rope_cur, rope_cos, rope_sin, half);
    const u32x4* src = reinterpret_cast<const u32x4*>(table + (size_t)st->cur_token * hidden);
    u32x4* dst = reinterpret_cast<u32x4*>(h);
    for (int i = blockIdx.x * blockDim.x + threadIdx.x; i < hidden / 8; i += gridDim.x * blockDim.x) dst[i] = src[i];
}

}

int launch_ep_fold(int grid, bf16_t* out, const bf16_t* resid, const float* partial, int64_t n, bool f16, hipStream_t s) {
    ep_fold_kernel<<<grid, 256, 0, s>>>(out, resid, partial, n, f16);
    OMX_LAUNCH_CHECK();
    return 0;
}

void drop_graphs(omx_qwen3 m) {
    if (m->g_full) { (void)hipGraphExecDestroy(m->g_full); m->g_full = nullptr; }
    if (m->g_nohead) { (void)hipGraphExecDestroy(m->g_nohead); m->g_nohead = nullptr; }
    if (m->aql_full) { aql_destroy(m->aql_full); m->aql_full = nullptr; }
    if (m->cfg.num_experts > 0 && (m->cfg.ep_size > 1 || m->cfg.tp_size > 1) && m->stream) workspace_aux_pin(m->stream, false);
}

void recapture_step(omx_qwen3 m) {
    drop_graphs(m);
    m->eager = false;
}

int rank_allreduce(omx_qwen3 m, void* buf, size_t n, int dtype, int op) {
    OMX_REQUIRE(m->allreduce != nullptr, "more than one rank (tp_size / ep_size) but no communicator set (omx_qwen3_set_comm)");
    OMX_REQUIRE(m->allreduce(buf, buf, n, dtype, op, m->comm, m->stream) == 0, "ncclAllReduce failed");
    return 0;
}

int allreduce_sum(omx_qwen3 m, float* buf, size_t n) { return rank_allreduce(m, buf, n, kNcclFloat32, kNcclSum); }

int read_step_state(omx_qwen3 m, StepState* st) {
    OMX_HIP_CHECK(hipMemcpyAsync(st, m->st, sizeof(*st), hipMemcpyDeviceToHost, m->stream));
    OMX_HIP_CHECK(hipStreamSynchronize(m->stream));
    return 0;
}

int write_step_state(omx_qwen3 m, const StepState& st) {
    OMX_HIP_CHECK(hipMemcpyAsync(m->st, &st, sizeof(st), hipMemcpyHostToDevice, m->stream));
    return 0;
}

int reset_sampler_history(omx_qwen3 m) {
    if (m->seen) OMX_HIP_CHECK(hipMemsetAsync(m->seen, 0, (size_t)m->V, m->stream));
    if (m->sel) OMX_HIP_CHECK(hipMemsetAsync(m->sel, 0, sample_select_ws_bytes(), m->stream));
    return 0;
}

bool sampling_penalised(const omx_sampling& p) { return p.repetition_penalty != 1.f || p.presence_penalty != 0.f; }

static int add_filtered_sampling(omx_qwen3 m, hipStream_t s) {
    const omx_sampling& p = m->sampling;
    const bool greedy = p.temperature == 0.f;
    const uint8_t* seen = sampling_penalised(p) ? m->seen : nullptr;
    if (!greedy && launch_rng_next(m->rng, s)) return 1;
    if (launch_sample_select(m->sel, m->logits, m->f16, m->V, p, seen, s)) return 1;
    return launch_sample_filtered_noise(m->argmax_partials, m->n_argmax_partials, m->logits, m->f16, m->V, p, seen, m->sel, m->rng + 2, s);
}

static int mark_sampled_token(omx_qwen3 m, hipStream_t s) {
    if (!m->filter_on || !sampling_penalised(m->sampling)) return 0;
    return launch_mark_seen(m->seen, m->V, m->st, s);
}

static int add_step_logprobs(omx_qwen3 m, hipStream_t s) {
    if (m->lp_top < 0) return 0;
    LogprobTopOut o = {};
    o.logprobs = m->lp_ring; o.top_ids = m->top_id_ring; o.top_lp = m->top_lp_ring;
    o.ring_count = &m->st->out_count; o.ring_cap = m->ring_cap;
    return launch_logprob_top(o, m->lp_scratch, m->logits, m->V, &m->st->cur_token, 1, m->V, m->lp_top, s);
}

static int add_sampling_noise(omx_qwen3 m, hipStream_t s) {
    if (m->filter_on) return add_filtered_sampling(m, s);
    if (m->temperature == 0.f) return 0;
    const omx_qwen3_config& c = m->cfg;
    const int tp = c.tp_size > 1 ? c.tp_size : 1;
    if (launch_rng_next(m->rng, s)) return 1;
    return launch_sample_noise(m->argmax_partials, m->n_argmax_partials, m->logits, m->rng + 2, m->V, c.tp_rank * m->V,
                               m->V * tp, 1.0f / m->temperature, m->f16, s);
}

bool attention_takes_oproj(omx_qwen3 m, int layer) {
    const bool off = env_off("OMX_ATTN_OPROJ");
    const omx_qwen3_config& c = m->cfg;
    if (off || m->oproj_disabled || m->Hkv * m->attn_nsplit > m->cus) return false;
    if (c.quant_bits) {
        if (c.ep_size > 1 || c.tp_size > 1 || c.quant_scales_f16 || layer < 0 || layer >= (int)m->qlayers.size()) return false;
        const QMat& o = m->qlayers[layer].o;
        return o.bits == 4 && o.sb != nullptr && attn_step_oproj_q4_ok(m->H, m->Hkv, c.head_dim, m->attn_nsplit, c.hidden_size, o.group);
    }
    return !m->f16 && attn_step_oproj_ok(m->H, m->Hkv, c.head_dim, m->attn_nsplit, c.hidden_size);
}

bool any_layer_takes_oproj(omx_qwen3 m) {
    for (int l = 0; l < m->cfg.num_hidden_layers; ++l)
        if (attention_takes_oproj(m, l)) return true;
    return false;
}

bool down_takes_qkv(omx_qwen3 m) {
    const bool off = env_off("OMX_DOWN_QKV");
    const omx_qwen3_config& c = m->cfg;
    if (off || m->chain_disabled || c.quant_bits != 0 || m->f16 || c.num_experts > 0 || c.tp_size > 1 || c.ep_size > 1 || m->allreduce != nullptr) return false;
    if (step_engine_mode(m) != 0 || env_int("OMX_GEMV_RPW_QKV", 0) != 0 || env_int("OMX_GEMV_RPW_DOWN", 0) != 0) return false;
    if (!m->chain_gran || !gemv_chain_ok(c.hidden_size, m->I, (m->H + 2 * m->Hkv) * c.head_dim)) return false;
    return gemv_chain_grid(c.hidden_size) <= kGemvChainBlocksPerCU * m->cus;
}

bool attention_takes_gateup(omx_qwen3 m, int layer) {
    const bool off = env_off("OMX_ATTN_GATEUP");
    const omx_qwen3_config& c = m->cfg;
    if (off || m->gateup_disabled || c.quant_bits != 0 || m->f16 || c.num_experts > 0 || c.tp_size > 1 || c.ep_size > 1 || m->allreduce != nullptr) return false;
    if (step_engine_mode(m) != 0 || env_int("OMX_GEMV_RPW_O", 0) != 0 || env_int("OMX_GEMV_RPW_GU", 0) != 0) return false;
    if (!m->gateup_gran || m->cus < 256 || !attention_takes_oproj(m, layer)) return false;
    return attn_step_gateup_ok(m->H, m->Hkv, c.head_dim, m->attn_nsplit, c.hidden_size, m->I);
}

static bool peer_fused_fits(omx_qwen3 m, int N, int K) {
    return m->peer_dev != nullptr && gemv_grid(N, K, EPI_F32, 0) <= 2 * m->cus;
}

static int enqueue_attention(omx_qwen3 m, int l, hipStream_t s, const bf16_t* resid = nullptr, bf16_t* out = nullptr, float* out_f32 = nullptr,
                             bool gateup = false) {
    const omx_qwen3_config& c = m->cfg;
    const int D = c.head_dim;
    const LayerW& L = m->layers[l];
    AttnStepArgs a = {};
    a.qkv = m->qkv;
    a.k = m->kcache[l]; a.v = m->vcache[l];
    a.kv_head_stride = (int64_t)m->cap * D;
    a.H = m->H; a.Hkv = m->Hkv; a.cap = m->cap;
    a.scale = 1.0f / sqrtf((float)D);
    a.eps = c.rms_norm_eps;
    a.q_norm_w = L.q_norm; a.k_norm_w = L.k_norm;
    a.rope_cur = m->rope_cur;
    a.pos_ptr = &m->st->pos;
    a.seq_ptr = m->step_seq;
    a.tag_mul = (unsigned)c.num_hidden_layers; a.tag_add = (unsigned)l + 1u;
    a.chunk = m->attn_chunk; a.nsplit = m->attn_nsplit;
    a.ws = m->attn_gran;
    a.out = m->attn_out;
    a.abort_flag = m->wait_abort;
    a.trace = m->attn_trace ? m->attn_trace + (size_t)l * m->attn_nsplit * m->Hkv * kAttnTraceWords : nullptr;
    a.f16 = m->f16;
    if (resid && (out || out_f32)) {
        a.o_resid = resid; a.o_out = out; a.o_out_f32 = out_f32; a.o_rows = c.hidden_size; a.xg = m->attn_xg;
        if (c.quant_bits) {
            const QMat& o = m->qlayers[l].o;
            a.o_wq = o.w; a.o_sb = o.sb; a.o_group = o.group;
        } else {
            a.o_w = L.o;
        }
    }
    if (gateup) {
        a.gu_gate = L.gate; a.gu_up = L.up; a.gu_norm_w = L.post_ln; a.gu_out = m->act; a.gu_rows = m->I;
        a.hg = m->gateup_gran;
    }
    return launch_attn_step(a, D, s);
}

int enqueue_step_tail(omx_qwen3 m, bool with_head, const bf16_t* h, const float* pending, int pending_n, bool tp) {
    const omx_qwen3_config& c = m->cfg;
    hipStream_t s = m->stream;
    if (!with_head) {
        OMX_LAUNCH(feed_prompt_kernel, 1, 1, 0, s, m->st, m->prompt_dev);
        OMX_LAUNCH_CHECK();
        return 0;
    }
    if (c.quant_bits) {
        QGemvArgs a = {};
        a.m[0] = m->q_head; a.m[0].n = m->V; a.N = m->V; a.K = c.hidden_size; a.group = m->q_head.group;
        a.x = h; a.norm_w = m->final_norm; a.eps = c.rms_norm_eps; a.out = m->logits; a.scales_f16 = c.quant_scales_f16 != 0;
        a.argmax_slot = m->argmax_partials;
        a.row_offset = c.tp_rank * m->V;
        if (launch_qgemv(a, m->q_head.bits, PRO_RMSNORM, EPI_ARGMAX, s)) return 1;
    } else {
        GemvArgs a = {};
        a.w0 = m->lm_head; a.n0 = m->V; a.N = m->V; a.K = c.hidden_size;
        a.x = h; a.x_partial = pending; a.x_partial_n = pending_n;
        a.norm_w = m->final_norm; a.eps = c.rms_norm_eps;
        a.out = m->logits;
        a.argmax_slot = m->argmax_partials;
        a.row_offset = c.tp_rank * m->V;
        a.f16 = m->f16;
        if (launch_gemv(a, PRO_RMSNORM, EPI_ARGMAX, s)) return 1;
    }
    if (add_sampling_noise(m, s)) return 1;
    OMX_LAUNCH(sample_finalize_kernel, 1, 256, 0, s, m->st, m->argmax_partials, m->n_argmax_partials, m->out_ring,
               m->ring_cap, tp ? m->argmax_key : nullptr);
    OMX_LAUNCH_CHECK();
    if (!tp) return mark_sampled_token(m, s) || add_step_logprobs(m, s);
    if (rank_allreduce(m, m->argmax_key, 1, kNcclUint64, kNcclMax)) return 1;
    OMX_LAUNCH(apply_token_kernel, 1, 1, 0, s, m->st, m->argmax_key, m->out_ring, m->ring_cap);
    OMX_LAUNCH_CHECK();
    return 0;
}

static int enqueue_step_quant(omx_qwen3 m, bool with_head) {
    const omx_qwen3_config& c = m->cfg;
    hipStream_t s = m->stream;
    const int hd = c.hidden_size, D = c.head_dim;
    const bool sf16 = c.quant_scales_f16 != 0;
#define OMX_QEMBED(KERNEL, B)                                                                                                      \
    case B: OMX_LAUNCH(KERNEL<B>, 4, 256, 0, s, m->h, m->q_embed.w, m->q_embed.scales, m->q_embed.biases, m->st, hd, m->q_embed.group, m->step_seq, \
                       m->rope_cur, m->rope_cos, m->rope_sin, D / 2, sf16); break;
    switch (m->q_embed.bits) {
        OMX_QEMBED(qembed_chunk_kernel, 2) OMX_QEMBED(qembed_chunk_kernel, 3) OMX_QEMBED(qembed_kernel, 4)
        OMX_QEMBED(qembed_chunk_kernel, 5) OMX_QEMBED(qembed_chunk_kernel, 6) OMX_QEMBED(qembed_kernel, 8)
    }
#undef OMX_QEMBED
    OMX_LAUNCH_CHECK();
    bf16_t* h = m->h;
    bf16_t* hn = m->h2;
    const bool tp = c.ep_size <= 1 && (c.tp_size > 1 || m->allreduce != nullptr);
    auto reduce_fold = [&](float* partial) -> int {
        if (allreduce_sum(m, partial, hd)) return 1;
        ep_fold_kernel<<<8, 256, 0, s>>>(hn, h, partial, (int64_t)hd, sf16);
        OMX_LAUNCH_CHECK();
        std::swap(h, hn);
        return 0;
    };
    for (int l = 0; l < c.num_hidden_layers; ++l) {
        const LayerW& L = m->layers[l];
        const LayerQ& Q = m->qlayers[l];
        {
            QGemvArgs a = {};
            a.m[0] = Q.q; a.m[1] = Q.k; a.m[2] = Q.v;
            a.N = (m->H + 2 * m->Hkv) * D; a.K = hd; a.group = Q.q.group;
            a.x = h; a.norm_w = L.in_ln; a.eps = c.rms_norm_eps; a.out = m->qkv; a.scales_f16 = sf16;
            if (launch_qgemv(a, Q.q.bits, PRO_RMSNORM, EPI_STORE, s)) return 1;
        }
        const bool fused_o = !tp && attention_takes_oproj(m, l);
        if (enqueue_attention(m, l, s, fused_o ? h : nullptr, fused_o ? hn : nullptr)) return 1;
        if (fused_o) {
            std::swap(h, hn);
        } else if (tp) {
            QGemvArgs a = {};
            a.m[0] = Q.o; a.N = hd; a.K = m->H * D; a.group = Q.o.group;
            a.x = m->attn_out; a.out_f32 = m->partial_a; a.scales_f16 = sf16;
            if (launch_qgemv(a, Q.o.bits, PRO_NONE, EPI_F32, s) || reduce_fold(m->partial_a)) return 1;
        } else {
            QGemvArgs a = {};
            a.m[0] = Q.o; a.N = hd; a.K = m->H * D; a.group = Q.o.group;
            a.x = m->attn_out; a.resid = h; a.out = hn; a.scales_f16 = sf16;
            if (launch_qgemv(a, Q.o.bits, PRO_NONE, EPI_RESIDUAL, s)) return 1;
            std::swap(h, hn);
        }
        if (c.num_experts > 0 && c.tp_size > 1) {
            if (omx_moe_block_partial_tp_q(m->moe_y, m->moe_inds, m->moe_scores, h, L.post_ln, c.rms_norm_eps, OMX_QMOE_ARGS(Q), 1, hd, m->moe_I, c.num_experts, c.num_experts_per_tok, c.moe_mode,
                                           c.norm_topk_prob, c.quant_group, c.quant_bits, sf16 ? 1 : 0, s))
                return 1;
            if (allreduce_sum(m, m->moe_y, (size_t)c.num_experts_per_tok * hd)) return 1;
            if (omx_moe_combine_slots_ex(hn, m->moe_y, m->moe_scores, h, 1, hd, c.num_experts_per_tok, sf16 ? 1 : 0, s)) return 1;
            std::swap(h, hn);
            continue;
        }
        if (c.num_experts > 0 && c.ep_size > 1) {
            const int el = c.num_experts / c.ep_size;
            if (omx_moe_block_partial_ep_q(m->partial_b, h, L.post_ln, c.rms_norm_eps, m->moe_xn, OMX_QMOE_ARGS(Q), 1, hd, c.moe_intermediate_size, c.num_experts,
                                           c.num_experts_per_tok, c.moe_mode, c.norm_topk_prob, c.ep_rank * el, el, c.quant_group, c.quant_bits, sf16 ? 1 : 0, s))
                return 1;
            if (reduce_fold(m->partial_b)) return 1;
            continue;
        }
        if (c.num_experts > 0) {
            if (omx_moe_block_forward_q_ex(hn, h, h, L.post_ln, c.rms_norm_eps, m->moe_xn, OMX_QMOE_ARGS(Q), 1, hd, c.moe_intermediate_size,
                                           c.num_experts, c.num_experts_per_tok, c.moe_mode, c.norm_topk_prob, c.quant_group, c.quant_bits, sf16 ? 1 : 0, s))
                return 1;
            std::swap(h, hn);
            continue;
        }
        {
            QGemvArgs a = {};
            a.m[0] = Q.gate; a.m[1] = Q.up; a.N = m->I; a.K = hd; a.group = Q.gate.group;
            a.x = h; a.norm_w = L.post_ln; a.eps = c.rms_norm_eps; a.out = m->act; a.scales_f16 = sf16;
            if (launch_qgemv(a, Q.gate.bits, PRO_RMSNORM, EPI_SWIGLU, s)) return 1;
        }
        if (tp) {
            QGemvArgs a = {};
            a.m[0] = Q.down; a.N = hd; a.K = m->I; a.group = Q.down.group;
            a.x = m->act; a.out_f32 = m->partial_b; a.scales_f16 = sf16;
            if (launch_qgemv(a, Q.down.bits, PRO_NONE, EPI_F32, s) || reduce_fold(m->partial_b)) return 1;
        } else {
            QGemvArgs a = {};
            a.m[0] = Q.down; a.N = hd; a.K = m->I; a.group = Q.down.group;
            a.x = m->act; a.resid = h; a.out = hn; a.scales_f16 = sf16;
            if (launch_qgemv(a, Q.down.bits, PRO_NONE, EPI_RESIDUAL, s)) return 1;
            std::swap(h, hn);
        }
    }
    return enqueue_step_tail(m, with_head, h, nullptr, 1, tp);
}

int step_engine_mode(omx_qwen3 m) {
    const int mode = env_int("OMX_STEP_ENGINE", 0);
    const omx_qwen3_config& c = m->cfg;
    const bool ok = mode > 0 && !m->se_disabled && !m->filter_on && m->lp_top < 0 && c.quant_bits == 0 && !m->f16 && c.num_experts == 0 && c.tp_size == 1 && c.ep_size <= 1 && m->allreduce == nullptr &&
           !c.attention_bias && m->se_gran != nullptr && m->cus > 0 &&
           step_engine_ok(c.hidden_size, m->H, m->Hkv, c.head_dim, m->I, m->attn_nsplit, m->cus);
    return ok ? (mode == 2 ? 2 : 1) : 0;
}

bool step_engine_takes(omx_qwen3 m) { return step_engine_mode(m) != 0; }

static int enqueue_step_engine(omx_qwen3 m, hipStream_t s, int seg_layer = -1) {
    const omx_qwen3_config& c = m->cfg;
    const int D = c.head_dim, hd = c.hidden_size;
    StepEngineArgs a = {};
    a.layers = m->se_layers;
    a.L = c.num_hidden_layers; a.hidden = hd; a.H = m->H; a.Hkv = m->Hkv; a.D = D; a.I = m->I; a.cap = m->cap;
    a.eps = c.rms_norm_eps; a.scale = 1.0f / sqrtf((float)D);
    a.embed = m->embed; a.st = m->st; a.seq_ptr = m->step_seq;
    a.rope_cos = m->rope_cos; a.rope_sin = m->rope_sin;
    a.chunk = m->attn_chunk; a.nsplit = m->attn_nsplit;
    uint64_t* g = m->se_gran;
    a.g_x = g; g += hd / 2;
    a.g_x1 = g; g += hd / 2;
    a.g_qkv = g; g += (size_t)(m->H + 2 * m->Hkv) * D / 2;
    a.g_attn = g; g += (size_t)m->H * D / 2;
    a.g_act = g;
    a.g_part = m->attn_gran;
    a.h_out = seg_layer < 0 ? m->h2 : m->h;
    a.seg_layer = seg_layer;
    a.x_in = m->h; a.x1_in = m->h2; a.qkv_out = m->qkv;
    if (seg_layer > 0) a.seg_m = m->se_layers_host[seg_layer - 1];
    if (seg_layer >= 0 && seg_layer < c.num_hidden_layers) a.seg_a = m->se_layers_host[seg_layer];
    a.xcd_major = env_int("OMX_SE_XCD_MAJOR", 1);
    a.abort_flag = m->wait_abort;
    a.nsweep = env_int("OMX_SE_NSWEEP", 1);
    a.inflight = env_int("OMX_SE_INFLIGHT", 2);
    a.thin_gather = env_int("OMX_SE_THIN", 1);
    a.trace = m->se_trace;
    return launch_step_engine(a, m->cus, s);
}

inline void time_next_launch(omx_qwen3 m, int layer, int cls) {
    if (g_launch_recorder) g_launch_recorder->next_tag = cls;
    if (!m->kernel_events) return;
    const size_t i = (cls == KC_HEAD ? (size_t)m->cfg.num_hidden_layers * kLayerClasses
                      : cls == KC_ENGINE ? (size_t)m->cfg.num_hidden_layers * kLayerClasses + 1 : (size_t)layer * kLayerClasses + cls) * 2;
    arm_launch_events((*m->kernel_events)[i], (*m->kernel_events)[i + 1]);
}

static int enqueue_step_hybrid(omx_qwen3 m, bool with_head) {
    const omx_qwen3_config& c = m->cfg;
    hipStream_t s = m->stream;
    const int hd = c.hidden_size, D = c.head_dim, L = c.num_hidden_layers;
    OMX_LAUNCH(embed_kernel, 2, 256, 0, s, m->h, m->embed, m->st, hd, m->step_seq, m->rope_cur, m->rope_cos, m->rope_sin, D / 2);
    OMX_LAUNCH_CHECK();
    for (int l = 0; l < L; ++l) {
        time_next_launch(m, l, KC_QKV);
        if (enqueue_step_engine(m, s, l)) return 1;
        const bool fused_o = attention_takes_oproj(m, l);
        time_next_launch(m, l, KC_ATTN);
        if (enqueue_attention(m, l, s, fused_o ? m->h : nullptr, fused_o ? m->h2 : nullptr, nullptr)) return 1;
        if (!fused_o) {
            GemvArgs a = {};
            a.w0 = m->layers[l].o; a.n0 = hd; a.N = hd; a.K = m->H * D;
            a.x = m->attn_out; a.resid = m->h; a.out = m->h2;
            time_next_launch(m, l, KC_O);
            if (launch_gemv(a, PRO_NONE, EPI_RESIDUAL, s)) return 1;
        }
    }
    time_next_launch(m, L - 1, KC_DOWN);
    if (enqueue_step_engine(m, s, L)) return 1;
    if (with_head) time_next_launch(m, 0, KC_HEAD);
    return enqueue_step_tail(m, with_head, m->h, nullptr, 1, false);
}

int enqueue_step(omx_qwen3 m, bool with_head) {
    if (m->cfg.quant_bits) return enqueue_step_quant(m, with_head);
    const omx_qwen3_config& c = m->cfg;
    hipStream_t s = m->stream;
    const int hd = c.hidden_size, D = c.head_dim;
    const bool ep = c.ep_size > 1;
    const bool tp = !ep && (c.tp_size > 1 || m->allreduce != nullptr);
    const int engine_mode = step_engine_mode(m);
    if (engine_mode == 2) return enqueue_step_hybrid(m, with_head);
    const bool engine = engine_mode == 1;
    if (engine) {
        time_next_launch(m, 0, KC_ENGINE);
        if (enqueue_step_engine(m, s)) return 1;
    } else {
        OMX_LAUNCH(embed_kernel, 2, 256, 0, s, m->h, m->embed, m->st, hd, m->step_seq, m->rope_cur, m->rope_cos, m->rope_sin, D / 2);
        OMX_LAUNCH_CHECK();
    }
    bf16_t* h = engine ? m->h2 : m->h;
    bf16_t* hn = engine ? m->h : m->h2;
    const float* pending = nullptr;
    int pending_n = 1;
    const bool moe_fold = env_on("OMX_MOE_FOLD", c.num_experts_per_tok <= 2) && c.num_experts > 0 && !ep && !tp;
    const bool chain = !engine && down_takes_qkv(m);
    for (int l = 0; l < (engine ? 0 : c.num_hidden_layers); ++l) {
        const LayerW& L = m->layers[l];
        if (!(chain && l > 0)) {
            GemvArgs a = {};
            a.w0 = L.q; a.n0 = m->H * D;
            a.w1 = L.k; a.n1 = m->Hkv * D;
            a.w2 = L.v; a.n2 = m->Hkv * D;
            a.N = (m->H + 2 * m->Hkv) * D;
            a.K = hd;
            a.x = h; a.x_partial = pending; a.x_partial_n = pending_n; a.x_out = pending ? hn : nullptr;
            a.norm_w = L.in_ln; a.eps = c.rms_norm_eps;
            a.out = m->qkv;
            a.out_bias = L.qkv_bias;
            a.f16 = m->f16;
            a.rows_per_wave = env_int("OMX_GEMV_RPW_QKV", 0);
            time_next_launch(m, l, KC_QKV);
            if (launch_gemv(a, PRO_RMSNORM, EPI_STORE, s)) return 1;
            if (pending) { std::swap(h, hn); pending = nullptr; pending_n = 1; }
        }
        const bool fused_o = attention_takes_oproj(m, l);
        time_next_launch(m, l, KC_ATTN);
        const bool gateup = fused_o && !tp && !pending && attention_takes_gateup(m, l);
        if (enqueue_attention(m, l, s, fused_o ? h : nullptr, fused_o && !tp ? hn : nullptr, fused_o && tp ? m->partial_a : nullptr, gateup)) return 1;
        if (fused_o && tp) {
            if (allreduce_sum(m, m->partial_a, hd)) return 1;
            pending = m->partial_a;
        } else if (fused_o) {
            std::swap(h, hn);
        } else {
            GemvArgs a = {};
            a.w0 = L.o; a.n0 = hd; a.N = hd; a.K = m->H * D;
            a.x = m->attn_out;
            a.f16 = m->f16;
            a.rows_per_wave = env_int("OMX_GEMV_RPW_O", 0);
            if (!tp) {
                a.resid = h; a.out = hn;
                time_next_launch(m, l, KC_O);
                if (launch_gemv(a, PRO_NONE, EPI_RESIDUAL, s)) return 1;
                std::swap(h, hn);
            } else {
                a.out = m->partial_a;
                a.peer = peer_fused_fits(m, a.N, a.K) ? m->peer_dev : nullptr;
                if (launch_gemv(a, PRO_NONE, EPI_F32, s)) return 1;
                if (!a.peer && allreduce_sum(m, m->partial_a, hd)) return 1;
                pending = m->partial_a;
            }
        }
        if (c.num_experts > 0 && tp && c.tp_size > 1) {
            ep_fold_kernel<<<8, 256, 0, s>>>(hn, h, pending, (int64_t)hd);
            OMX_LAUNCH_CHECK();
            std::swap(h, hn); pending = nullptr; pending_n = 1;
            if (omx_moe_block_partial_tp(m->moe_y, m->moe_inds, m->moe_scores, h, L.post_ln, c.rms_norm_eps, m->moe_xn, L.moe_gate, L.moe_wg,
                                         L.moe_wu, L.moe_wd, 1, hd, m->moe_I, c.num_experts, c.num_experts_per_tok, c.moe_mode, c.norm_topk_prob, s))
                return 1;
            if (allreduce_sum(m, m->moe_y, (size_t)c.num_experts_per_tok * hd)) return 1;
            if (omx_moe_combine_slots(hn, m->moe_y, m->moe_scores, h, 1, hd, c.num_experts_per_tok, s)) return 1;
            std::swap(h, hn);
            continue;
        }
        if (c.num_experts > 0 && ep) {
            const int el = c.num_experts / c.ep_size;
            if (omx_moe_block_partial_ep(m->partial_b, h, L.post_ln, c.rms_norm_eps, m->moe_xn, L.moe_gate, L.moe_wg, L.moe_wu, L.moe_wd,
                                         1, hd, c.moe_intermediate_size, c.num_experts, c.num_experts_per_tok, c.moe_mode,
                                         c.norm_topk_prob, c.ep_rank * el, el, s))
                return 1;
            if (allreduce_sum(m, m->partial_b, hd)) return 1;
            pending = m->partial_b;
            continue;
        }
        if (c.num_experts > 0) {
            if (moe_fold) {
                const int rc = omx_moe_block_partials(m->moe_partials, h, L.post_ln, c.rms_norm_eps, m->moe_xn, L.moe_gate, L.moe_wg, L.moe_wu,
                                                      L.moe_wd, hd, c.moe_intermediate_size, c.num_experts, c.num_experts_per_tok, c.moe_mode,
                                                      c.norm_topk_prob, s);
                if (rc == 0) { pending = m->moe_partials; pending_n = c.num_experts_per_tok; continue; }
                if (rc != 2) return 1;
            }
            if (omx_moe_block_forward(hn, h, h, L.post_ln, c.rms_norm_eps, m->moe_xn, L.moe_gate, L.moe_wg, L.moe_wu, L.moe_wd, 1, hd,
                                      c.moe_intermediate_size, c.num_experts, c.num_experts_per_tok, c.moe_mode, c.norm_topk_prob, s))
                return 1;
            std::swap(h, hn);
            continue;
        }
        if (!gateup) {
            GemvArgs a = {};
            a.w0 = L.gate; a.w1 = L.up; a.n0 = m->I; a.N = m->I; a.K = hd;
            a.x = h; a.x_partial = pending; a.x_partial_n = pending_n; a.x_out = pending ? hn : nullptr;
            a.norm_w = L.post_ln; a.eps = c.rms_norm_eps;
            a.out = m->act;
            a.f16 = m->f16;
            a.rows_per_wave = env_int("OMX_GEMV_RPW_GU", 0);
            time_next_launch(m, l, KC_GATE_UP);
            if (launch_gemv(a, PRO_RMSNORM, EPI_SWIGLU, s)) return 1;
            if (pending) { std::swap(h, hn); pending = nullptr; pending_n = 1; }
        }
        if (chain && l + 1 < c.num_hidden_layers) {
            const LayerW& Ln = m->layers[l + 1];
            GemvChainArgs a = {};
            a.w_down = L.down; a.N = hd; a.K = m->I;
            a.x = m->act; a.resid = h; a.out = hn;
            a.xg = m->chain_gran; a.seq_ptr = m->step_seq; a.abort_flag = m->wait_abort;
            a.tag_mul = (unsigned)c.num_hidden_layers; a.tag_add = (unsigned)l + 1u;
            a.w0 = Ln.q; a.n0 = m->H * D;
            a.w1 = Ln.k; a.n1 = m->Hkv * D;
            a.w2 = Ln.v; a.n2 = m->Hkv * D;
            a.NQ = (m->H + 2 * m->Hkv) * D;
            a.norm_w = Ln.in_ln; a.eps = c.rms_norm_eps;
            a.out_bias = Ln.qkv_bias;
            a.qkv_out = m->qkv;
            time_next_launch(m, l, KC_DOWN);
            if (launch_gemv_chain(a, s)) return 1;
            std::swap(h, hn);
        } else {
            GemvArgs a = {};
            a.w0 = L.down; a.n0 = hd; a.N = hd; a.K = m->I;
            a.x = m->act;
            a.f16 = m->f16;
            a.rows_per_wave = env_int("OMX_GEMV_RPW_DOWN", 0);
            if (!tp) {
                a.resid = h; a.out = hn;
                time_next_launch(m, l, KC_DOWN);
                if (launch_gemv(a, PRO_NONE, EPI_RESIDUAL, s)) return 1;
                std::swap(h, hn);
            } else {
                a.out = m->partial_b;
                a.peer = peer_fused_fits(m, a.N, a.K) ? m->peer_dev : nullptr;
                if (launch_gemv(a, PRO_NONE, EPI_F32, s)) return 1;
                if (!a.peer && allreduce_sum(m, m->partial_b, hd)) return 1;
                pending = m->partial_b;
            }
        }
    }
    if (with_head) time_next_launch(m, 0, KC_HEAD);
    return enqueue_step_tail(m, with_head, h, pending, pending_n, tp);
}

int step_aql_mode(omx_qwen3 m) {
    const int mode = env_int("OMX_STEP_AQL", 0);
    const omx_qwen3_config& c = m->cfg;
    if (mode <= 0 || m->aql_disabled || m->eager || m->allreduce != nullptr || c.tp_size > 1 || c.ep_size > 1 || c.num_experts > 0 ||
        m->temperature != 0.f || m->filter_on || m->lp_top >= 0 || step_engine_mode(m) != 0)
        return 0;
    return mode;
}

static void build_aql(omx_qwen3 m) {
    const int mode = step_aql_mode(m);
    if (!mode || m->aql_full) return;
    LaunchRecorder rec;
    hipGraph_t g = nullptr;
    if (hipStreamBeginCapture(m->stream, hipStreamCaptureModeThreadLocal) != hipSuccess) { (void)hipGetLastError(); m->aql_disabled = true; return; }
    g_launch_recorder = &rec;
    const int rc = enqueue_step(m, true);
    g_launch_recorder = nullptr;
    const hipError_t e = hipStreamEndCapture(m->stream, &g);
    size_t nodes = 0;
    if (g) { (void)hipGraphGetNodes(g, nullptr, &nodes); (void)hipGraphDestroy(g); }
    AqlProgram* p = nullptr;
    if (!rc && e == hipSuccess && nodes == 0) {
        const int fence = mode == 2 ? AQL_FENCE_NONE : mode == 3 ? AQL_FENCE_ACQUIRE : mode == 4 ? AQL_FENCE_RELEASE : AQL_FENCE_AGENT;
        p = aql_build(rec, fence);
    } else if (!rc && e == hipSuccess) {
        set_error("aql: %zu launches of the step are not recording sites", nodes);
    }
    if (!p) {
        if (getenv("OMX_STEP_AQL_VERBOSE")) fprintf(stderr, "omx: AQL step unavailable: %s\n", omx_last_error());
        (void)hipGetLastError();
        omx_clear_error();
        m->aql_disabled = true;
        return;
    }
    m->aql_full = p;
}

static int build_graphs(omx_qwen3 m) {
    if (m->g_full || m->eager) return 0;
    if (resolve_weights(m)) return 1;
    if (env_on("OMX_NO_GRAPH")) {
        m->eager = true;
        return 0;
    }
    for (int which = 0; which < 2; ++which) {
        hipGraph_t g = nullptr;
        OMX_HIP_CHECK(hipStreamBeginCapture(m->stream, hipStreamCaptureModeThreadLocal));
        const int rc = enqueue_step(m, which == 0);
        hipError_t e = hipStreamEndCapture(m->stream, &g);
        hipGraphExec_t ge = nullptr;
        if (!rc && e == hipSuccess) e = hipGraphInstantiate(&ge, g, nullptr, nullptr, 0);
        if (g) (void)hipGraphDestroy(g);
        if (rc || e != hipSuccess) {
            (void)hipGetLastError();
            if (m->allreduce != nullptr) {
                if (m->g_full) { (void)hipGraphExecDestroy(m->g_full); m->g_full = nullptr; }
                m->eager = true;
                omx_clear_error();
                return 0;
            }
            return rc ? 1 : set_error("step graph capture failed: %s", hipGetErrorString(e));
        }
        (which == 0 ? m->g_full : m->g_nohead) = ge;
    }
    if (m->cfg.num_experts > 0 && (m->cfg.ep_size > 1 || m->cfg.tp_size > 1)) workspace_aux_pin(m->stream, true);
    build_aql(m);
    return 0;
}

int context_bucket(omx_qwen3 m, int tk) {
    const int gran = tk <= 8192 ? 1024 : 4096;
    return std::min(m->cap, (tk + gran - 1) / gran * gran);
}
int prepare_step(omx_qwen3 m, int pos) {
    const int want = context_bucket(m, pos + 1);
    if (want != m->graph_tk_max) {
        drop_graphs(m);
        attn_step_plan(want, m->Hkv, m->H / m->Hkv, m->cfg.head_dim, &m->attn_chunk, &m->attn_nsplit);
        m->graph_tk_max = want;
    }
    return build_graphs(m);
}

int run_step(omx_qwen3 m, bool with_head, int pos) {
    if (prepare_step(m, pos)) return 1;
    if (m->eager) return enqueue_step(m, with_head);
    OMX_HIP_CHECK(hipGraphLaunch(with_head ? m->g_full : m->g_nohead, m->stream));
    return 0;
}

int step_gave_up(omx_qwen3 m, unsigned* code) {
    OMX_HIP_CHECK(hipMemcpy(code, m->wait_abort, 4, hipMemcpyDeviceToHost));
    return 0;
}
int step_health(omx_qwen3 m) {
    unsigned gave_up = 0;
    if (step_gave_up(m, &gave_up)) return 1;
    OMX_REQUIRE(gave_up == 0, "decode step: a wait inside a launch gave up (code 0x%x: a workgroup of the launch was not resident?)", gave_up);
    return 0;
}

int step_fallback(omx_qwen3 m, const StepState& st) {
    if (m->temperature != 0.f || m->filter_on) return 1;
    if (m->allreduce != nullptr || m->cfg.tp_size > 1 || m->cfg.ep_size > 1) return 1;
    bool gateup = false;
    for (int l = 0; l < m->cfg.num_hidden_layers && !m->gateup_disabled; ++l) gateup = gateup || attention_takes_gateup(m, l);
    const bool chain = !m->chain_disabled && down_takes_qkv(m);
    if (gateup || chain) {
        m->gateup_disabled = m->gateup_disabled || gateup;
        m->chain_disabled = m->chain_disabled || chain;
    }
    else if (!m->se_disabled && step_engine_takes(m)) m->se_disabled = true;
    else if (!m->oproj_disabled && any_layer_takes_oproj(m)) m->oproj_disabled = true;
    else return 1;
    drop_graphs(m);
    OMX_HIP_CHECK(hipMemsetAsync(m->wait_abort, 0, 4, m->stream));
    if (write_step_state(m, st)) return 1;
    OMX_HIP_CHECK(hipStreamSynchronize(m->stream));
    return 0;
}

}
```

ominix-mlx_amd/engine.py:

```python
from __future__ import annotations

import ctypes
import sys
from typing import Dict, Iterator, Optional

import numpy as np

from . import OmxError, Sampling, check, lib, require_device
from .ops import Tensor

c_int, c_float, c_void_p, c_uint32 = ctypes.c_int, ctypes.c_float, ctypes.c_void_p, ctypes.c_uint32


class Qwen3Config(ctypes.Structure):
    _fields_ = [("hidden_size", c_int), ("num_hidden_layers", c_int), ("intermediate_size", c_int),
                ("num_attention_heads", c_int), ("num_key_value_heads", c_int), ("head_dim", c_int),
                ("vocab_size", c_int), ("rms_norm_eps", c_float), ("rope_theta", c_float), ("rope_scale", c_float),
                ("tie_word_embeddings", c_int), ("max_context", c_int), ("tp_rank", c_int), ("tp_size", c_int),
                ("quant_bits", c_int), ("quant_group", c_int), ("num_experts", c_int), ("num_experts_per_tok", c_int),
                ("moe_intermediate_size", c_int), ("moe_mode", c_int), ("norm_topk_prob", c_int), ("no_qk_norm", c_int),
                ("ep_rank", c_int), ("ep_size", c_int), ("attention_bias", c_int), ("quant_scales_f16", c_int),
                ("float16_weights", c_int)]


# ... 245 lines not shown
    if stem == "model.norm":
        return (hd,) if leaf_kind == "weight" else None
    parts = stem.split(".")
    if len(parts) < 4 or parts[0] != "model" or parts[1] != "layers":
        return None
    sub = ".".join(parts[3:])
    table = {"self_attn.q_proj": (H * D, hd), "self_attn.k_proj": (Hkv * D, hd), "self_attn.v_proj": (Hkv * D, hd),
             "self_attn.o_proj": (hd, H * D), "mlp.gate_proj": (I, hd), "mlp.up_proj": (I, hd), "mlp.down_proj": (hd, I)}
    if sub in table:
        return lin(*table[sub])
    if sub in ("input_layernorm", "post_attention_layernorm"):
        return (hd,) if leaf_kind == "weight" else None
    if sub in ("self_attn.q_norm", "self_attn.k_norm"):
        return (D,) if leaf_kind == "weight" else None
    if E > 0:
        El = E // ep
        for mp in ("block_sparse_moe.", "mlp."):
            if sub == mp + "gate":
                return lin(E, hd)
            if sub in (mp + "switch_mlp.gate_proj", mp + "switch_mlp.up_proj"):
                return lin(Im, hd, (El,))
            if sub == mp + "switch_mlp.down_proj":
                return lin(hd, Im, (El,))
    return None


class Model:

    logprobs_top = None

    def __init__(self, *, hidden_size, num_hidden_layers, intermediate_size, num_attention_heads,
                 num_key_value_heads, head_dim, vocab_size, rms_norm_eps=1e-6, rope_theta=1e6,
                 tie_word_embeddings=False, rope_scaling=None, max_context=4096, tp_rank=0, tp_size=1, quantization=None,
                 num_experts=0, num_experts_per_tok=0, moe_intermediate_size=0, moe_mode="qwen3_moe", norm_topk_prob=False,
                 qk_norm=True, ep_rank=0, ep_size=1, attention_bias=False, dtype="bfloat16", **_ignored):
        require_device()
        q = quantization or {}
        _, table = quant_formats(quantization)
        f16_weights = dense_dtype_is_f16(dtype)
        self.cfg = Qwen3Config(hidden_size, num_hidden_layers, intermediate_size, num_attention_heads,
                               num_key_value_heads, head_dim, vocab_size, rms_norm_eps, rope_theta,
                               rope_scale_from_config(rope_scaling), int(bool(tie_word_embeddings)), max_context,
                               tp_rank, tp_size, int(q.get("bits", 0)), int(q.get("group_size", 64 if q else 0)),
                               int(num_experts), int(num_experts_per_tok), int(moe_intermediate_size),
                               {"mixtral": 0, "qwen3_moe": 1}[moe_mode], int(bool(norm_topk_prob)), int(not qk_norm),
                               int(ep_rank), int(ep_size), int(bool(attention_bias)),
                               int(str(q.get("scales_dtype", "bfloat16")).lower() in ("float16", "f16", "half")),
                               int(f16_weights))
        self._h = c_void_p()
        check(lib.omx_qwen3_create(ctypes.byref(self._h), ctypes.byref(self.cfg)))
        self._keep = []
        base = (self.cfg.quant_bits, self.cfg.quant_group)
        self.quant_table = {p: f for p, f in table.items() if f != base and not (p == "lm_head" and self.cfg.tie_word_embeddings)}
        for prefix, (bits, group) in self.quant_table.items():
            check(lib.omx_qwen3_set_quant_format(self._h, prefix.encode(), bits, group))

    def close(self) -> None:
        h = getattr(self, "_h", None)
        if h is not None and h.value:
            lib.omx_qwen3_destroy(h)
            self._h = c_void_p()

    def __del__(self):
        if sys is not None and not sys.is_finalizing():
            self.close()

    @property
    def f16(self) -> bool:
        return bool(self.cfg.quant_scales_f16 or self.cfg.float16_weights)

    @property
    def vocab_local(self) -> int:
        return self.cfg.vocab_size // self.cfg.tp_size

    def load_weights(self, weights: Dict[str, np.ndarray]) -> None:
        if self.cfg.tp_size > 1:
            from . import tp
            weights = tp.shard_state_dict(weights, self.cfg.tp_rank, self.cfg.tp_size, bool(self.cfg.tie_word_embeddings),
                                          self.cfg.num_key_value_heads, self.cfg.head_dim)
        if self.cfg.ep_size > 1:
            from . import ep
            weights = {k: (ep.shard_experts(v, self.cfg.ep_rank, self.cfg.ep_size) if ".switch_mlp." in k else v)
                       for k, v in weights.items()}
        for name, arr in weights.items():
            want = self.expected_shape(name)
            if want is not None and tuple(arr.shape) != want:
                raise OmxError(f"ShapeMismatch: {name} has shape {tuple(arr.shape)}, the config expects {want}")
            dt = np.asarray(arr).dtype
            if self.cfg.quant_bits and name.endswith((".scales", ".biases")):
                f16 = dt == np.float16
                if f16 != bool(self.cfg.quant_scales_f16):
                    raise OmxError(f"{name}: {'float16' if f16 else str(dt)} scales / biases, but the model was created with "
                                   f"quantization scales_dtype={'float16' if self.cfg.quant_scales_f16 else 'bfloat16'}")
                if f16:
                    t = Tensor.from_numpy(arr, "f16")
                    self._keep.append(t)
                    check(lib.omx_qwen3_set_weight(self._h, name.encode(), t.ptr, t.nbytes))
                    continue
            if self.cfg.quant_bits and name.endswith(".weight") and name[:-7] + ".scales" in weights and dt != np.uint32:
                raise OmxError(f"{name}: a quantized weight must be packed uint32, found {dt}")
            if self.f16 and dt != np.uint32 and type(arr).__name__ == "Bf16Bits":
                arr = (np.asarray(arr).astype(np.uint32) << np.uint32(16)).view(np.float32)
            t = Tensor.from_numpy(arr, "u32" if dt == np.uint32 else "f16" if self.f16 else "bf16")
            self._keep.append(t)
            check(lib.omx_qwen3_set_weight(self._h, name.encode(), t.ptr, t.nbytes))

    def expected_shape(self, name: str):
        return expected_shape(self.cfg, name, self.quant_table)

    def quant_format(self, prefix: str) -> tuple:
        bits, group = c_int(), c_int()
        check(lib.omx_qwen3_quant_format(self._h, prefix.encode(), ctypes.byref(bits), ctypes.byref(group)))
        return bits.value, group.value

    def synth_weights(self, base_seed: int = 0x0C0FFEE5, peaked: bool = False) -> None:
        fn = lib.omx_qwen3_synth_weights_peaked if peaked else lib.omx_qwen3_synth_weights
        check(fn(self._h, base_seed & 0xFFFFFFFF))

    def set_comm(self, comm_ptr: int, allreduce_fn_ptr: int) -> None:
        check(lib.omx_qwen3_set_comm(self._h, comm_ptr, allreduce_fn_ptr))

    def encode(self, input_ids, attention_mask=None, extract_layers=(8, 17, 26)):
        from .ops import Tensor
        ids = np.ascontiguousarray(np.asarray(input_ids, dtype=np.uint32).ravel())
        taps = (c_int * len(extract_layers))(*[int(t) for t in extract_layers])
        out = Tensor((ids.size, len(extract_layers) * self.cfg.hidden_size), "f16" if self.f16 else "bf16")
        am = None
        if attention_mask is not None:
            am = np.ascontiguousarray(np.asarray(attention_mask).ravel() != 0, dtype=np.uint8)
            if am.size != ids.size:
                raise OmxError("encode: attention_mask and input_ids differ in length")
        check(lib.omx_qwen3_encode(self._h, ids.ctypes.data_as(ctypes.POINTER(c_uint32)), ids.size,
                                   am.ctypes.data if am is not None else None, taps, len(extract_layers), out.ptr))
        return out

    def set_sampler(self, temperature: float, seed: int = 0, *, top_k: int = 0, top_p: float = 1.0, repetition_penalty: float = 1.0,
                    presence_penalty: float = 0.0) -> None:
        if top_k == 0 and top_p == 1.0 and repetition_penalty == 1.0 and presence_penalty == 0.0:
            check(lib.omx_qwen3_set_sampler(self._h, float(temperature), int(seed) & 0xFFFFFFFFFFFFFFFF))
            return
        p = Sampling(temperature, top_k, top_p, repetition_penalty, presence_penalty)
        check(lib.omx_qwen3_set_sampling(self._h, ctypes.byref(p), int(seed) & 0xFFFFFFFFFFFFFFFF))

    def sampler_state(self) -> tuple:
        st = (c_uint32 * 2)()
        check(lib.omx_qwen3_sampler_state(self._h, st, 0))
        return int(st[0]), int(st[1])

    def set_sampler_state(self, state) -> None:
        st = (c_uint32 * 2)(int(state[0]), int(state[1]))
        check(lib.omx_qwen3_sampler_state(self._h, st, 1))

    def reset(self) -> None:
        check(lib.omx_qwen3_reset(self._h))

    def offset(self) -> int:
        v = c_int()
        check(lib.omx_qwen3_offset(self._h, ctypes.byref(v)))
        return v.value

    def embed_tokens(self, ids):
        from .ops import Tensor
        p = np.ascontiguousarray(np.asarray(ids, dtype=np.uint32).ravel())
        out = Tensor((p.size, self.cfg.hidden_size), "f16" if self.f16 else "bf16")
        check(lib.omx_qwen3_embed_tokens(self._h, p.ctypes.data_as(ctypes.POINTER(c_uint32)), p.size, out.ptr))
        return out

    def prefill(self, prompt, embeds=None, embeds_at: int = 0) -> int:
        p = np.ascontiguousarray(prompt, dtype=np.uint32)
        first = c_uint32()
        if embeds is None:
            check(lib.omx_qwen3_prefill(self._h, p.ctypes.data_as(ctypes.POINTER(c_uint32)), p.size, ctypes.byref(first)))
            return first.value
        from .ops import Tensor
        if not isinstance(embeds, Tensor):
            a = np.asarray(embeds)
            embeds = Tensor.from_numpy(a, "f16" if a.dtype == np.float16 else "f32")
        if len(embeds.shape) != 2 or embeds.shape[1] != self.cfg.hidden_size:
            raise OmxError(f"ShapeMismatch: embeds has shape {embeds.shape}, the model expects [n_rows, {self.cfg.hidden_size}]")
        check(lib.omx_synchronize(None))
        check(lib.omx_qwen3_prefill_embeds(self._h, p.ctypes.data_as(ctypes.POINTER(c_uint32)), p.size, embeds.ptr if embeds.shape[0] else None,
                                           embeds.dtype, int(embeds_at), embeds.shape[0], ctypes.byref(first)))
        return first.value

    def set_logprobs(self, top_n=None) -> None:
        check(lib.omx_qwen3_set_logprobs(self._h, -1 if top_n is None else int(top_n)))
        self.logprobs_top = None if top_n is None or int(top_n) < 0 else int(top_n)

    def decode(self, n: int, return_logprobs: bool = False):
        out = np.empty(n, dtype=np.uint32)
        if not return_logprobs:
            check(lib.omx_qwen3_decode(self._h, n, out.ctypes.data_as(ctypes.POINTER(c_uint32))))
            return out
        top = self.logprobs_top or 0
        lp, ids, tlp = np.zeros(n, np.float32), np.zeros((n, top), np.uint32), np.zeros((n, top), np.float32)
        check(lib.omx_qwen3_decode_logprobs(self._h, n, out.ctypes.data_as(ctypes.POINTER(c_uint32)), lp.ctypes.data_as(ctypes.POINTER(c_float)),
                                            ids.ctypes.data if top else None, tlp.ctypes.data if top else None))
        return (out, lp, ids, tlp) if top else (out, lp)

    def last_logprobs(self):
        top = self.logprobs_top or 0
        lp, ids, tlp = c_float(), np.zeros(top, np.uint32), np.zeros(top, np.float32)
        check(lib.omx_qwen3_last_logprobs(self._h, ctypes.byref(lp), ids.ctypes.data if top else None, tlp.ctypes.data if top else None))
        return (np.float32(lp.value), ids, tlp) if top else np.float32(lp.value)

    def verify(self, tokens) -> np.ndarray:
        ids = np.ascontiguousarray(np.asarray(tokens, dtype=np.uint32).ravel())
        out = np.empty(ids.size, dtype=np.uint32)
        check(lib.omx_qwen3_verify(self._h, ids.ctypes.data_as(ctypes.POINTER(c_uint32)), ids.size, out.ctypes.data_as(ctypes.POINTER(c_uint32))))
        return out

    def verify_logits(self, row: int) -> np.ndarray:
        raw = np.empty(self.vocab_local, dtype=np.uint16)
        check(lib.omx_qwen3_verify_logits(self._h, row, raw.ctypes.data, raw.size))
        return (raw.astype(np.uint32) << np.uint32(16)).view(np.float32)

    def trim(self, n: int, next_token: int) -> None:
        check(lib.omx_qwen3_trim(self._h, n, int(next_token)))

    def score(self, tokens, next_token=None, return_greedy=False):
        ids = np.ascontiguousarray(np.asarray(tokens, dtype=np.uint32).ravel())
        last = 0xFFFFFFFF if next_token is None else int(next_token)
        targets = np.ascontiguousarray(np.concatenate([ids[1:], np.array([last], dtype=np.uint32)]), dtype=np.uint32)
        lp = np.zeros(ids.size, dtype=np.float32)
        greedy = np.zeros(ids.size, dtype=np.uint32)
        u32p = ctypes.POINTER(c_uint32)
        check(lib.omx_qwen3_score(self._h, ids.ctypes.data_as(u32p), ids.size, targets.ctypes.data_as(u32p),
                                  lp.ctypes.data_as(ctypes.POINTER(c_float)), greedy.ctypes.data_as(u32p)))
        if next_token is None:
            lp = lp[:-1]
        return (lp, greedy) if return_greedy else lp

    def last_score_ms(self) -> tuple:
        a, b = c_float(), c_float()
        check(lib.omx_qwen3_last_score_ms(self._h, ctypes.byref(a), ctypes.byref(b)))
        return a.value, b.value

    def last_decode_ms(self) -> float:
        v = c_float()
        check(lib.omx_qwen3_last_decode_ms(self._h, ctypes.byref(v)))
        return v.value

    def dequant_bytes(self) -> int:
        v = ctypes.c_size_t()
        check(lib.omx_qwen3_dequant_bytes(self._h, ctypes.byref(v)))
        return int(v.value)

    def last_prefill_ms(self) -> float:
        v = c_float()
        check(lib.omx_qwen3_last_prefill_ms(self._h, ctypes.byref(v)))
        return v.value

    def per_op_route(self, prompt, n_new: int) -> dict:
        ids = np.ascontiguousarray(np.asarray(prompt, dtype=np.uint32).ravel())
        toks = np.zeros(n_new + 1, np.uint32)
        pre, per, calls = ctypes.c_double(), ctypes.c_double(), ctypes.c_double()
        check(lib.omx_bench_qwen3_per_op(self._h, ctypes.byref(self.cfg), ids.ctypes.data_as(ctypes.POINTER(c_uint32)), ids.size, n_new,
                                         toks.ctypes.data_as(ctypes.POINTER(c_uint32)), ctypes.byref(pre), ctypes.byref(per), ctypes.byref(calls)))
        return {"tokens": toks, "prefill_ms": pre.value, "ms_per_token": per.value, "calls_per_token": calls.value}

    def per_op_route_forced(self, prompt, forced, logit_steps) -> dict:
        ids = np.ascontiguousarray(np.asarray(prompt, dtype=np.uint32).ravel())
        forced = np.ascontiguousarray(np.asarray(forced, dtype=np.uint32).ravel())
        steps = np.ascontiguousarray(np.asarray(logit_steps, dtype=np.int32).ravel())
        toks = np.zeros(forced.size + 1, np.uint32)
        raw = np.zeros((steps.size, self.cfg.vocab_size), np.uint16)
        fn = lib.omx_bench_qwen3_per_op_ex
        fn.restype = ctypes.c_int
        fn.argtypes = [c_void_p, c_void_p, ctypes.POINTER(c_uint32), c_int, c_int, ctypes.POINTER(c_uint32), c_void_p, c_void_p, c_void_p,
                       ctypes.POINTER(c_uint32), ctypes.POINTER(ctypes.c_int32), c_int, c_void_p]
        pre, per, calls = ctypes.c_double(), ctypes.c_double(), ctypes.c_double()
        check(fn(self._h, ctypes.addressof(self.cfg), ids.ctypes.data_as(ctypes.POINTER(c_uint32)), ids.size, forced.size,
                 toks.ctypes.data_as(ctypes.POINTER(c_uint32)), ctypes.addressof(pre), ctypes.addressof(per), ctypes.addressof(calls),
                 forced.ctypes.data_as(ctypes.POINTER(c_uint32)), steps.ctypes.data_as(ctypes.POINTER(ctypes.c_int32)), steps.size, raw.ctypes.data))
        return {"tokens": toks, "logits": (raw.astype(np.uint32) << np.uint32(16)).view(np.float32)}

    def last_logits(self) -> np.ndarray:
        raw = np.empty(self.vocab_local, dtype=np.uint16)
        check(lib.omx_qwen3_last_logits(self._h, raw.ctypes.data, raw.size))
        if self.f16:
            return raw.view(np.float16).astype(np.float32)
        return (raw.astype(np.uint32) << np.uint32(16)).view(np.float32)

    def stream(self) -> int:
        s = c_void_p()
        check(lib.omx_qwen3_stream(self._h, ctypes.byref(s)))
        return s.value or 0

    def decode_path(self) -> str:
        v = c_int()
        check(lib.omx_qwen3_decode_path(self._h, ctypes.byref(v)))
        path = ("unbuilt", "graph", "eager", "aql")[v.value & 0xFF]
        return path + "".join(" " + name for bit, name in enumerate(("gateup_disabled", "chain_disabled", "engine_disabled", "oproj_disabled"))
                              if v.value >> (8 + bit) & 1)

    KERNEL_CLASSES = ("qkv", "attention", "o", "gate_up", "down", "lm_head", "step_engine")

    def time_step_kernels(self, steps: int = 4) -> dict:
        us = (ctypes.c_float * 7)()
        check(lib.omx_qwen3_time_step_kernels(self._h, steps, us))
        return dict(zip(self.KERNEL_CLASSES, (float(v) for v in us)))

    def step_forms(self) -> dict:
        f = (c_int * 6)()
        check(lib.omx_qwen3_debug_step_forms(self._h, f))
        return {"down_qkv": bool(f[0]), "attn_oproj": bool(f[1]), "step_engine": int(f[2]), "down_qkv_gave_up": bool(f[3]),
                "attn_gateup": bool(f[4]), "attn_gateup_gave_up": bool(f[5])}

    def raise_give_up(self) -> None:
        check(lib.omx_qwen3_debug_raise_give_up(self._h))

    def step_bytes(self, ctx: int) -> float:
        v = ctypes.c_double()
        check(lib.omx_qwen3_step_bytes(self._h, ctx, ctypes.byref(v)))
        return v.value

    def batch(self, n_slots: int, max_context: int = 0, kv_bits: int = 0) -> "Batch":
        return Batch(self, n_slots, max_context, kv_bits)


class Batch:

    logprobs_top = None

    def __init__(self, model: Model, n_slots: int, max_context: int = 0, kv_bits: int = 0):
        self.model, self.n_slots, self.kv_bits = model, int(n_slots), int(kv_bits)
        self._h = c_void_p()
        if self.kv_bits == 0:
            check(lib.omx_qwen3_batch_create(ctypes.byref(self._h), model._h, int(n_slots), int(max_context)))
        else:
            check(lib.omx_qwen3_batch_create_kv(ctypes.byref(self._h), model._h, int(n_slots), int(max_context), self.kv_bits))

    def close(self) -> None:
        h = getattr(self, "_h", None)
        if h is not None and h.value:
            m = getattr(self.model, "_h", None)
            if m is not None and m.value:
                lib.omx_qwen3_batch_destroy(h)
            self._h = c_void_p()

    def __del__(self):
        if sys is not None and not sys.is_finalizing():
            self.close()

    def set_sampler(self, slot: int, temperature: float, seed: int = 0, *, top_k: int = 0, top_p: float = 1.0,
                    repetition_penalty: float = 1.0, presence_penalty: float = 0.0) -> None:
        if top_k == 0 and top_p == 1.0 and repetition_penalty == 1.0 and presence_penalty == 0.0:
            check(lib.omx_qwen3_batch_set_sampler(self._h, int(slot), float(temperature), int(seed) & 0xFFFFFFFFFFFFFFFF))
            return
        p = Sampling(temperature, top_k, top_p, repetition_penalty, presence_penalty)
        check(lib.omx_qwen3_batch_set_sampling(self._h, int(slot), ctypes.byref(p), int(seed) & 0xFFFFFFFFFFFFFFFF))

    def prefill(self, slot: int, prompt) -> int:
        p = np.ascontiguousarray(prompt, dtype=np.uint32)
        first = c_uint32()
        check(lib.omx_qwen3_batch_prefill(self._h, int(slot), p.ctypes.data_as(ctypes.POINTER(c_uint32)), p.size, ctypes.byref(first)))
        return first.value

    def fork(self, src: int, dst: int, resample: bool = True) -> int:
        first = c_uint32()
        check(lib.omx_qwen3_batch_fork(self._h, int(src), int(dst), int(bool(resample)), ctypes.byref(first)))
        return first.value

    def shared(self, slot: int):
        owner, n = c_int(), c_int()
        check(lib.omx_qwen3_batch_shared(self._h, int(slot), ctypes.byref(owner), ctypes.byref(n)))
        return owner.value, n.value

    def set_logprobs(self, top_n=None) -> None:
        check(lib.omx_qwen3_batch_set_logprobs(self._h, -1 if top_n is None else int(top_n)))
        self.logprobs_top = None if top_n is None or int(top_n) < 0 else int(top_n)

    def decode(self, n: int, slots=None, return_logprobs: bool = False):
        ids = np.ascontiguousarray(list(range(self.n_slots)) if slots is None else slots, dtype=np.int32).ravel()
        out = np.empty((int(n), ids.size), dtype=np.uint32)
        if not return_logprobs:
            check(lib.omx_qwen3_batch_decode(self._h, ids.ctypes.data_as(ctypes.POINTER(c_int)), ids.size, int(n),
                                             out.ctypes.data_as(ctypes.POINTER(c_uint32))))
            return out
        top = self.logprobs_top or 0
        lp = np.zeros((int(n), ids.size), np.float32)
        tid, tlp = np.zeros((int(n), ids.size, top), np.uint32), np.zeros((int(n), ids.size, top), np.float32)
        check(lib.omx_qwen3_batch_decode_logprobs(self._h, ids.ctypes.data_as(ctypes.POINTER(c_int)), ids.size, int(n),
                                                  out.ctypes.data_as(ctypes.POINTER(c_uint32)), lp.ctypes.data_as(ctypes.POINTER(c_float)),
                                                  tid.ctypes.data if top else None, tlp.ctypes.data if top else None))
        return (out, lp, tid, tlp) if top else (out, lp)

    def last_logprobs(self, slot: int):
        top = self.logprobs_top or 0
        lp, ids, tlp = c_float(), np.zeros(top, np.uint32), np.zeros(top, np.float32)
        check(lib.omx_qwen3_batch_last_logprobs(self._h, int(slot), ctypes.byref(lp), ids.ctypes.data if top else None,
                                                tlp.ctypes.data if top else None))
        return (np.float32(lp.value), ids, tlp) if top else np.float32(lp.value)

    def logits(self, slot: int) -> np.ndarray:
        raw = np.empty(self.model.vocab_local, dtype=np.uint16)
        check(lib.omx_qwen3_batch_logits(self._h, int(slot), raw.ctypes.data, raw.size))
        return (raw.astype(np.uint32) << np.uint32(16)).view(np.float32)

    def offset(self, slot: int) -> int:
        v = c_int()
        check(lib.omx_qwen3_batch_offset(self._h, int(slot), ctypes.byref(v)))
        return v.value

    def trim(self, slot: int, n: int, next_token: int) -> None:
        check(lib.omx_qwen3_batch_trim(self._h, int(slot), int(n), int(next_token)))

    def reset(self, slot: int) -> None:
        check(lib.omx_qwen3_batch_reset(self._h, int(slot)))

    def kv_bytes(self) -> int:
        v = ctypes.c_size_t()
        check(lib.omx_qwen3_batch_kv_bytes(self._h, ctypes.byref(v)))
        return v.value

    def kv_rows(self, slot: int, layer: int, first: int = 0, n=None):
        cfg = self.model.cfg
        Hkv, D = int(cfg.num_key_value_heads), int(cfg.head_dim)
        n = self.offset(slot) - int(first) if n is None else int(n)
        widen = lambda raw: (raw.astype(np.uint32) << np.uint32(16)).view(np.float32)
        if self.kv_bits == 0:
            k, v = (np.empty((Hkv, max(n, 0), D), dtype=np.uint16) for _ in range(2))
            check(lib.omx_qwen3_batch_kv_read(self._h, int(slot), int(layer), int(first), n, k.ctypes.data, v.ctypes.data, None, None, None, None))
            return widen(k), widen(v)
        k, v = (np.empty((Hkv, max(n, 0), D // 4), dtype=np.uint32) for _ in range(2))
        ks, kb, vs, vb = (np.empty((Hkv, max(n, 0), D // 64), dtype=np.uint16) for _ in range(4))
        check(lib.omx_qwen3_batch_kv_read(self._h, int(slot), int(layer), int(first), n, k.ctypes.data, v.ctypes.data, ks.ctypes.data,
                                          kb.ctypes.data, vs.ctypes.data, vb.ctypes.data))
        return (k, widen(ks), widen(kb)), (v, widen(vs), widen(vb))

    def debug_attention(self, layer: int, slots, q) -> np.ndarray:
        ids = np.ascontiguousarray(slots, dtype=np.int32).ravel()
        qf = np.ascontiguousarray(q, dtype=np.float32)
        H, D = int(self.model.cfg.num_attention_heads), int(self.model.cfg.head_dim)
        if qf.shape != (ids.size, H, D):
            raise ValueError(f"debug_attention: q must be [{ids.size}, {H}, {D}], got {qf.shape}")
        u = qf.view(np.uint32)
        raw = ((u + np.uint32(0x7FFF) + ((u >> np.uint32(16)) & np.uint32(1))) >> np.uint32(16)).astype(np.uint16)
        out = np.empty((ids.size, H * D), dtype=np.uint16)
        check(lib.omx_qwen3_batch_debug_attention(self._h, int(layer), ids.ctypes.data_as(ctypes.POINTER(c_int)), ids.size,
                                                  raw.ctypes.data, out.ctypes.data))
        return (out.astype(np.uint32) << np.uint32(16)).view(np.float32)

    def last_decode_ms(self) -> float:
        v = c_float()
        check(lib.omx_qwen3_batch_last_decode_ms(self._h, ctypes.byref(v)))
        return v.value


class Generate:

    def __init__(self, model: Model, temp: float, prompt_token, chunk: int = 16, seed: int = 0, *, top_k: int = 0, top_p: float = 1.0,
                 repetition_penalty: float = 1.0, presence_penalty: float = 0.0, logprobs=None):
        model.set_sampler(temp, seed, top_k=top_k, top_p=top_p, repetition_penalty=repetition_penalty, presence_penalty=presence_penalty)
        if logprobs is not None or model.logprobs_top is not None:
            model.set_logprobs(logprobs)
        self.model, self.prompt, self.chunk = model, np.asarray(prompt_token, dtype=np.uint32).ravel(), chunk
        self._prefilled = False
        self._buf = []
        self._with_logprobs = logprobs is not None
        self.logprobs, self.top_logprobs = [], []

    def __iter__(self) -> Iterator[int]:
        return self

    def _record(self, lp, ids=(), tlp=()) -> None:
        self.logprobs.append(float(lp))
        self.top_logprobs.append([(int(i), float(v)) for i, v in zip(ids, tlp)])

    def __next__(self) -> int:
        if not self._prefilled:
            self._prefilled = True
            first = self.model.prefill(self.prompt)
            if self._with_logprobs:
                last = self.model.last_logprobs()
                self._record(*(last if isinstance(last, tuple) else (last,)))
            return first
        if not self._buf:
            if self._with_logprobs:
                toks, lp, *top = self.model.decode(self.chunk, return_logprobs=True)
                ids, tlp = top if top else ([()] * len(toks), [()] * len(toks))
                self._buf = list(zip(toks, lp, ids, tlp))
            else:
                self._buf = [(t,) for t in self.model.decode(self.chunk)]
        tok, *rest = self._buf.pop(0)
        if rest:
            self._record(*rest)
        return int(tok)
```

Baseline: 350.0.

## Fuse down projection and next layer's qkv into the attention step kernel

Extends the persistent attention+O-proj+gate/up kernel with a further phase. It gathers the SwiGLU activations across blocks through granule tags, computes the down projection with the residual, then publishes the new hidden state, applies RMSNorm and computes the next layer's q/k/v rows. The aim is to remove the separate down/qkv kernel launch and its launch gap per layer. In exchange it adds more cross-block spin-waiting on a fixed 256-block grid and applies only to one specific shape (intermediate 12288, hidden 4096).

```diff
diff --git a/ominix-mlx_amd/csrc/attn.hpp b/ominix-mlx_amd/csrc/attn.hpp
--- a/ominix-mlx_amd/csrc/attn.hpp
+++ b/ominix-mlx_amd/csrc/attn.hpp
@@ -57,7 +57,19 @@
     bf16_t* gu_out;
     int gu_rows;
     uint64_t* hg;
+    const bf16_t* dn_w;
+    bf16_t* dn_out;
+    uint64_t* ag;
+    uint64_t* rg;
+    const bf16_t* nq_w0;
+    const bf16_t* nq_w1;
+    const bf16_t* nq_w2;
+    int nq_n0, nq_n1, nq_rows;
+    const bf16_t* nq_norm_w;
+    const bf16_t* nq_bias;
+    bf16_t* nq_out;
 };
+bool attn_step_down_ok(int o_rows, int gu_rows, int nq_rows);
 bool attn_step_oproj_ok(int H, int Hkv, int D, int nsplit, int o_rows);
 bool attn_step_gateup_ok(int H, int Hkv, int D, int nsplit, int o_rows, int gu_rows);
 bool attn_step_oproj_q4_ok(int H, int Hkv, int D, int nsplit, int o_rows, int group);
diff --git a/ominix-mlx_amd/csrc/attn_step.hip b/ominix-mlx_amd/csrc/attn_step.hip
--- a/ominix-mlx_amd/csrc/attn_step.hip
+++ b/ominix-mlx_amd/csrc/attn_step.hip
@@ -186,7 +186,9 @@
     }
 }
 
-__device__ __forceinline__ void gateup_reduce(const AttnStepArgs& a, const u32x4 (*w)[kGuNV], const u32x4* xs, int pair, int lane) {
+template <bool DN = false>
+__device__ __forceinline__ void gateup_reduce(const AttnStepArgs& a, const u32x4 (*w)[kGuNV], const u32x4* xs, int pair, int lane,
+                                              uint16_t* park = nullptr) {
     typedef Act16<false> A;
     float acc[2] = {0.f, 0.f};
 #pragma unroll
@@ -203,14 +205,234 @@
     }
 #pragma unroll
     for (int r = 0; r < 2; ++r) acc[r] = wave_sum(acc[r]);
+    if constexpr (DN) {
+        if (lane == 0) {
+            const uint16_t v = epi_bits<EPI_SWIGLU, A>(acc[0], acc[1], (bf16_t)0, 0);
+            a.gu_out[pair] = v;
+            *park = v;
+        }
+    } else
     if (lane == 0) a.gu_out[pair] = epi_bits<EPI_SWIGLU, A>(acc[0], acc[1], (bf16_t)0, 0);
 }
 
+constexpr int kDnInter = 12288, kDnBlockRows = 16, kDnNV = kDnInter / 512 / 4, kDnUnits = kDnBlockRows / 2 * 4, kDnQRows = 3;
+constexpr int kDnPartOff = kDnInter * 2, kDnParkOff = kDnPartOff + kDnBlockRows * 4 * 4, kDnLdsBytes = kDnParkOff + kGuBlockPairs * 2;
+enum { kDnTicket = 4, kDnReduced = 5, kDnStored = 6, kDnWords = 8 };
+
+__device__ __forceinline__ int down_claim(int* sm_gu, int lane) {
+    int t = 0;
+    if (lane == 0) t = __hip_atomic_fetch_add(sm_gu + kDnTicket, 1, __ATOMIC_RELAXED, __HIP_MEMORY_SCOPE_WORKGROUP);
+    return __builtin_amdgcn_readfirstlane(t);
+}
+
+__device__ __forceinline__ void down_issue(const AttnStepArgs& a, u32x4 (*w)[kDnNV], int row_begin, int u, int lane) {
+    const u32x4* p = reinterpret_cast<const u32x4*>(a.dn_w) + (size_t)(row_begin + 2 * (u >> 2)) * (kDnInter / 8) + (u & 3) * (kDnNV * 64) + lane;
+#pragma unroll
+    for (int r = 0; r < 2; ++r) {
+#pragma unroll
+        for (int j = 0; j < kDnNV; ++j) w[r][j] = ld_nt(p + (size_t)r * (kDnInter / 8) + j * 64);
+    }
+    __builtin_amdgcn_sched_barrier(0);
+}
+
+__device__ __forceinline__ void down_reduce(const u32x4 (*w)[kDnNV], const u32x4* xa, float* part, int u, int lane) {
+    typedef Act16<false> A;
+    float acc[2] = {0.f, 0.f};
+#pragma unroll
+    for (int j = 0; j < kDnNV; ++j) {
+        const u32x4 xp = xa[(u & 3) * (kDnNV * 64) + j * 64 + lane];
+        float xf[8];
+#pragma unroll
+        for (int q = 0; q < 4; ++q) {
+            xf[2 * q] = A::lo(xp[q]);
+            xf[2 * q + 1] = A::hi(xp[q]);
+        }
+#pragma unroll
+        for (int r = 0; r < 2; ++r) acc[r] = dot8(w[r][j], xf, acc[r]);
+    }
+#pragma unroll
+    for (int r = 0; r < 2; ++r) acc[r] = wave_sum(acc[r]);
+    if (lane == 0) {
+#pragma unroll
+        for (int r = 0; r < 2; ++r) part[(2 * (u >> 2) + r) * 4 + (u & 3)] = acc[r];
+    }
+}
+
+template <int N2, int NW>
+__device__ __forceinline__ void sweep_vector(const AttnStepArgs& a, const uint64_t* gr, unsigned* sx, int part, unsigned tag, int lane) {
+    constexpr int GPL = N2 / NW / 64;
+    static_assert(N2 % (NW * 64) == 0 && GPL <= 48, "whole lanes, at most 96 registers of granules");
+    gr += (size_t)part * (N2 / NW);
+    sx += part * (N2 / NW);
+    for (unsigned spins = 0; spins < kSpinLimit; ++spins) {
+        const unsigned long long g = ld_granule(gr + (size_t)lane * GPL + (GPL - 1));
+        if (__all((unsigned)(g >> 32) == tag)) break;
+        __builtin_amdgcn_s_sleep(4);
+    }
+    unsigned long long g[GPL];
+    for (unsigned spins = 0;; ++spins) {
+#pragma unroll
+        for (int i = 0; i < GPL; ++i) g[i] = ld_granule(gr + (size_t)i * 64 + lane);
+        bool ok = true;
+#pragma unroll
+        for (int i = 0; i < GPL; ++i) ok &= (unsigned)(g[i] >> 32) == tag;
+        if (__all(ok)) break;
+        if (spins >= kSpinLimit) {
+            if (lane == 0) __hip_atomic_store(a.abort_flag, 1u, __ATOMIC_RELAXED, __HIP_MEMORY_SCOPE_AGENT);
+            break;
+        }
+        __builtin_amdgcn_s_sleep(4);
+    }
+#pragma unroll
+    for (int i = 0; i < GPL; ++i) sx[i * 64 + lane] = (unsigned)g[i];
+}
+
+__device__ __forceinline__ const bf16_t* next_qkv_row(const AttnStepArgs& a, int row) {
+    if (row < a.nq_n0) return a.nq_w0 + (size_t)row * kGuHidden;
+    row -= a.nq_n0;
+    if (row < a.nq_n1) return a.nq_w1 + (size_t)row * kGuHidden;
+    row -= a.nq_n1;
+    return a.nq_w2 + (size_t)row * kGuHidden;
+}
+
 template <bool TRACE>
+__device__ __forceinline__ void down_qkv_phase(const AttnStepArgs& a, unsigned char* sm_dn, u32x4* xs, float* red, int* sm_gu, unsigned res2,
+                                               unsigned tag, int lane, int wave, unsigned long long* tr) {
+    typedef Act16<false> A;
+    u32x4* xa = reinterpret_cast<u32x4*>(sm_dn);
+    float* part = reinterpret_cast<float*>(sm_dn + kDnPartOff);
+    const int blk = (int)blockIdx.y * (int)gridDim.x + (int)blockIdx.x;
+    const int row_begin = blk * kDnBlockRows;
+    const int q_row0 = (blk * kWaves + __builtin_amdgcn_readfirstlane(wave)) * kDnQRows;
+    constexpr int PV = kGuNV * 64 / 256;
+    u32x4 nwv[PV];
+#pragma unroll
+    for (int i = 0; i < PV; ++i) nwv[i] = *(reinterpret_cast<const u32x4*>(a.nq_norm_w) + (threadIdx.x & 255) + i * 256);
+    bf16_t ob[kDnQRows];
+#pragma unroll
+    for (int r = 0; r < kDnQRows; ++r) ob[r] = *(a.nq_bias ? a.nq_bias + min(q_row0 + r, a.nq_rows - 1) : a.nq_norm_w);
+    u32x4 dA[2][kDnNV], dB[2][kDnNV];
+    int tA = 0, tB = 0;
+    u32x4 qw[kDnQRows][kGuNV];
+    auto issue_qkv = [&](const int r0, const int r1) {
+#pragma unroll
+        for (int r = r0; r < r1; ++r) {
+            const u32x4* p = reinterpret_cast<const u32x4*>(next_qkv_row(a, min(q_row0 + r, a.nq_rows - 1)));
+#pragma unroll
+            for (int j = 0; j < kGuNV; ++j) qw[r][j] = ld_nt(p + j * 64 + lane);
+        }
+        __builtin_amdgcn_sched_barrier(0);
+    };
+    const bool sweeper = (wave & (kWaves / 2 - 1)) == 0;
+    if (!sweeper) {
+        tA = down_claim(sm_gu, lane);
+        down_issue(a, dA, row_begin, tA, lane);
+        tB = down_claim(sm_gu, lane);
+        down_issue(a, dB, row_begin, tB, lane);
+        issue_qkv(0, kDnQRows - 1);
+    }
+    lds_barrier();
+    if (sweeper) {
+        if (wave == 0 && lane < kGuBlockPairs / 2)
+            st_granule_u32(a.ag + (size_t)blk * (kGuBlockPairs / 2) + lane, tag, reinterpret_cast<const unsigned*>(sm_dn + kDnParkOff)[lane]);
+        sweep_vector<kDnInter / 2, 2>(a, a.ag, reinterpret_cast<unsigned*>(xa), __builtin_amdgcn_readfirstlane(wave) / (kWaves / 2), tag, lane);
+        if (TRACE && threadIdx.x == 0) tr[11] = wall_clock64();
+        tA = down_claim(sm_gu, lane);
+        down_issue(a, dA, row_begin, tA, lane);
+        tB = down_claim(sm_gu, lane);
+        down_issue(a, dB, row_begin, tB, lane);
+        issue_qkv(0, kDnQRows - 1);
+    }
+    lds_barrier();
+    down_reduce(dA, xa, part, tA, lane);
+    if (TRACE && threadIdx.x == 0) tr[12] = wall_clock64();
+    int n_reduced = 1;
+    int nA = down_claim(sm_gu, lane), nB;
+    for (;;) {
+        if (nA >= kDnUnits) {
+            down_reduce(dB, xa, part, tB, lane);
+            ++n_reduced;
+            break;
+        }
+        tA = nA;
+        down_issue(a, dA, row_begin, tA, lane);
+        nB = down_claim(sm_gu, lane);
+        down_reduce(dB, xa, part, tB, lane);
+        if (nB >= kDnUnits) {
+            down_reduce(dA, xa, part, tA, lane);
+            n_reduced += 2;
+            break;
+        }
+        tB = nB;
+        down_issue(a, dB, row_begin, tB, lane);
+        nA = down_claim(sm_gu, lane);
+        down_reduce(dA, xa, part, tA, lane);
+        n_reduced += 2;
+    }
+    if (TRACE && lane == 0) __hip_atomic_fetch_add(sm_gu + kDnReduced, n_reduced, __ATOMIC_RELAXED, __HIP_MEMORY_SCOPE_WORKGROUP);
+    issue_qkv(kDnQRows - 1, kDnQRows);
+    lds_barrier();
+    if (wave == 0) {
+        if (lane < kDnBlockRows / 2) {
+            float v[2] = {0.f, 0.f};
+#pragma unroll
+            for (int e = 0; e < 2; ++e) {
+#pragma unroll
+                for (int w = 0; w < 4; ++w) v[e] += part[(2 * lane + e) * 4 + w];
+            }
+            const uint32_t o2 = (uint32_t)epi_bits<EPI_RESIDUAL, A>(v[0], 0.f, (bf16_t)(res2 & 0xFFFFu), 0) |
+                                ((uint32_t)epi_bits<EPI_RESIDUAL, A>(v[1], 0.f, (bf16_t)(res2 >> 16), 0) << 16);
+            reinterpret_cast<uint32_t*>(a.dn_out)[row_begin / 2 + lane] = o2;
+            st_granule_u32(a.rg + row_begin / 2 + lane, tag, o2);
+        }
+        sweep_vector<kGuHidden / 2, 1>(a, a.rg, reinterpret_cast<unsigned*>(xs), 0, tag, lane);
+        if (TRACE && lane == 0) tr[13] = wall_clock64();
+    }
+    lds_barrier();
+    rmsnorm_in_lds<A, PV>(xs, red, nwv, kGuHidden, a.eps, threadIdx.x < 256);
+    float acc[kDnQRows];
+#pragma unroll
+    for (int r = 0; r < kDnQRows; ++r) acc[r] = 0.f;
+#pragma unroll
+    for (int j = 0; j < kGuNV; ++j) {
+        const u32x4 xp = xs[j * 64 + lane];
+        float xf[8];
+#pragma unroll
+        for (int q = 0; q < 4; ++q) {
+            xf[2 * q] = A::lo(xp[q]);
+            xf[2 * q + 1] = A::hi(xp[q]);
+        }
+#pragma unroll
+        for (int r = 0; r < kDnQRows; ++r) acc[r] = dot8(qw[r][j], xf, acc[r]);
+    }
+#pragma unroll
+    for (int r = 0; r < kDnQRows; ++r) acc[r] = wave_sum(acc[r]);
+    if (lane == 0) {
+        int stored = 0;
+#pragma unroll
+        for (int r = 0; r < kDnQRows; ++r)
+            if (q_row0 + r < a.nq_rows) {
+                a.nq_out[q_row0 + r] = A::bits(a.nq_bias ? acc[r] + A::val(ob[r]) : acc[r]);
+                ++stored;
+            }
+        if (TRACE) __hip_atomic_fetch_add(sm_gu + kDnStored, stored, __ATOMIC_RELAXED, __HIP_MEMORY_SCOPE_WORKGROUP);
+    }
+    if constexpr (TRACE) {
+        lds_barrier();
+        if (threadIdx.x == 0) {
+            tr[14] = wall_clock64();
+            tr[15] = (unsigned long long)sm_gu[kDnReduced] | (unsigned long long)sm_gu[kDnStored] << 32;
+        }
+    }
+}
+
+template <bool TRACE, bool DN = false>
 __device__ __forceinline__ void gateup_phase(const AttnStepArgs& a, u32x4* xs, float* red, int* sm_gu, const uint16_t* sm_pub, unsigned tag,
-                                             int lane, int wave, int pub_row0, int pub_rows, unsigned long long* tr) {
+                                             int lane, int wave, int pub_row0, int pub_rows, unsigned long long* tr,
+                                             unsigned char* sm_dn = nullptr) {
     typedef Act16<false> A;
     const int pair0 = ((int)blockIdx.y * (int)gridDim.x + (int)blockIdx.x) * kGuBlockPairs;
+    uint16_t* park = DN ? reinterpret_cast<uint16_t*>(sm_dn + kDnParkOff) : nullptr;
     constexpr int PV = kGuNV * 64 / 256;
     u32x4 nwv[PV];
 #pragma unroll
@@ -267,37 +489,39 @@
         gateup_issue(a, wB, pair0 + tB, lane);
     }
     lds_barrier();
+    unsigned res2 = 0;
+    if constexpr (DN) res2 = reinterpret_cast<const unsigned*>(xs)[(pair0 / kGuBlockPairs) * (kDnBlockRows / 2) + (lane & (kDnBlockRows / 2 - 1))];
     rmsnorm_in_lds<A, PV>(xs, red, nwv, kGuHidden, a.eps, threadIdx.x < 256);
     if (wave == 0) {
         gateup_issue(a, wB, pair0 + tB, lane);
-        gateup_reduce(a, wA, xs, pair0 + tA, lane);
+        gateup_reduce<DN>(a, wA, xs, pair0 + tA, lane, park + tA);
         if (TRACE && threadIdx.x == 0) tr[7] = wall_clock64();
         asm volatile("; first pair reduced: wave 0, its second pair just asked for" ::: "memory");
     } else {
-        gateup_reduce(a, wA, xs, pair0 + tA, lane);
+        gateup_reduce<DN>(a, wA, xs, pair0 + tA, lane, park + tA);
         asm volatile("; first pair reduced: the second pair came in through the hop" ::: "memory");
     }
     int n_reduced = 1;
     int nA = gateup_claim(sm_gu, lane), nB;
     for (;;) {
         if (nA >= kGuBlockPairs) {
-            gateup_reduce(a, wB, xs, pair0 + tB, lane);
+            gateup_reduce<DN>(a, wB, xs, pair0 + tB, lane, park + tB);
             ++n_reduced;
             break;
         }
         tA = nA;
         gateup_issue(a, wA, pair0 + tA, lane);
         nB = gateup_claim(sm_gu, lane);
-        gateup_reduce(a, wB, xs, pair0 + tB, lane);
+        gateup_reduce<DN>(a, wB, xs, pair0 + tB, lane, park + tB);
         if (nB >= kGuBlockPairs) {
-            gateup_reduce(a, wA, xs, pair0 + tA, lane);
+            gateup_reduce<DN>(a, wA, xs, pair0 + tA, lane, park + tA);
             n_reduced += 2;
             break;
         }
         tB = nB;
         gateup_issue(a, wB, pair0 + tB, lane);
         nA = gateup_claim(sm_gu, lane);
-        gateup_reduce(a, wA, xs, pair0 + tA, lane);
+        gateup_reduce<DN>(a, wA, xs, pair0 + tA, lane, park + tA);
         n_reduced += 2;
     }
     if constexpr (TRACE) {
@@ -309,6 +533,7 @@
         lds_barrier();
         if (threadIdx.x == 0) tr[10] = (unsigned long long)sm_gu[kGuReduced];
     }
+    if constexpr (DN) down_qkv_phase<TRACE>(a, sm_dn, xs, red, sm_gu, res2, tag, lane, wave, tr);
 }
 
 template <int NVW, int R, bool GU = false>
@@ -442,8 +667,9 @@
 }
 
 
-template <int D, int GT, bool TRACE, int NVW, bool F16 = false, bool GU = false>
+template <int D, int GT, bool TRACE, int NVW, bool F16 = false, bool GU = false, bool DN = false>
 __global__ __launch_bounds__(kBlock, 1) void attn_step_kernel(const AttnStepArgs a) {
+    static_assert(!DN || GU, "down + the next q/k/v follow gate/up only");
     static_assert(!F16 || NVW == 0, "the O projection rides in the launch for bfloat16 models only");
     static_assert(!GU || (NVW == kGuNV && D == 128), "gate/up follows the bf16 O projection of hidden 4096 only");
     typedef Act16<F16> A16;
@@ -470,7 +696,7 @@
     unsigned long long* tr = TRACE ? a.trace + ((size_t)split * a.Hkv + kvh) * kAttnTraceWords : nullptr;
     if (TRACE && threadIdx.x == 0) tr[0] = wall_clock64();
     if constexpr (GU) {
-        if (threadIdx.x < kGuWords) sm_gu[threadIdx.x] = 0;
+        if (threadIdx.x < (DN ? kDnWords : kGuWords)) sm_gu[threadIdx.x] = 0;
     }
 
     bf16_t* Kb = a.k + (size_t)kvh * a.kv_head_stride;
@@ -667,7 +893,7 @@
             uint16_t* sm_pub = reinterpret_cast<uint16_t*>(sm_l);
             if (rows == 2) oproj_phase<NV, 2, true>(a, sm_x, tag, lane, wave, o_row0, otr, sm_pub, pub_row0);
             else oproj_phase<NV, 3, true>(a, sm_x, tag, lane, wave, o_row0, otr, sm_pub, pub_row0);
-            gateup_phase<TRACE>(a, sm_x, sm_m, sm_gu, sm_pub, tag, lane, wave, pub_row0, pub_rows, otr);
+            gateup_phase<TRACE, DN>(a, sm_x, sm_m, sm_gu, sm_pub, tag, lane, wave, pub_row0, pub_rows, otr, smem);
             return;
         } else
         if constexpr (QO) {
@@ -698,7 +924,7 @@
     }
     if constexpr (GU) {
         lds_barrier();
-        gateup_phase<TRACE>(a, sm_x, sm_m, sm_gu, nullptr, tag, lane, wave, 0, 0, TRACE ? tr : nullptr);
+        gateup_phase<TRACE, DN>(a, sm_x, sm_m, sm_gu, nullptr, tag, lane, wave, 0, 0, TRACE ? tr : nullptr, smem);
     }
 }
 
@@ -740,6 +966,11 @@
     if (D != 128 || H * D != kGuHidden || o_rows != kGuHidden || H / std::max(Hkv, 1) != 4 || blocks != 256) return false;
     if (gu_rows != blocks * kGuBlockPairs || !attn_step_oproj_ok(H, Hkv, D, nsplit, o_rows)) return false;
     return oproj_rows_per_wave(H, Hkv, nsplit, o_rows) == 3 && (o_rows - waves * 2) % kWaves == 0;
+}
+
+bool attn_step_down_ok(int o_rows, int gu_rows, int nq_rows) {
+    const int waves = 256 * kWaves;
+    return o_rows == 256 * kDnBlockRows && gu_rows == kDnInter && nq_rows > (kDnQRows - 1) * waves && nq_rows <= kDnQRows * waves;
 }
 
 int launch_attn_step(const AttnStepArgs& a_in, int D, hipStream_t s) {
@@ -767,6 +998,10 @@
         OMX_REQUIRE(a.o_w && a.o_out && !a.o_out_f32 && !a.f16 && a.gu_up && a.gu_norm_w && a.gu_out && a.hg &&
                         attn_step_gateup_ok(a.H, a.Hkv, D, a.nsplit, a.o_rows, a.gu_rows),
                     "decode attention + gate/up: shape does not qualify (%d blocks, %d O rows, %d pairs)", a.Hkv * a.nsplit, a.o_rows, a.gu_rows);
+    if (a.dn_w)
+        OMX_REQUIRE(a.gu_gate && a.dn_out && a.ag && a.rg && a.nq_w0 && a.nq_w1 && a.nq_w2 && a.nq_norm_w && a.nq_out &&
+                        a.nq_n0 > 0 && a.nq_n1 > 0 && a.nq_rows > a.nq_n0 + a.nq_n1 && attn_step_down_ok(a.o_rows, a.gu_rows, a.nq_rows),
+                    "decode attention + down + q/k/v: shape does not qualify (%d rows, %d pairs, %d q/k/v rows)", a.o_rows, a.gu_rows, a.nq_rows);
     const dim3 grid(a.Hkv, a.nsplit), block(kBlock);
     const int gt = G <= 1 ? 1 : G <= 2 ? 2 : G <= 4 ? 4 : 8;
 #define OMX_ATTN_LAUNCH(DD, GG, TT, NN)                                                                                  \
@@ -786,13 +1021,24 @@
         OMX_LAUNCH_CHECK();                                                                                              \
         return 0;                                                                                                        \
     }
+#define OMX_ATTN_LAUNCH_DN(TT)                                                                                           \
+    {                                                                                                                    \
+        OMX_HIP_CHECK(hipFuncSetAttribute((const void*)attn_step_kernel<128, 4, TT, kGuNV, false, true, true>,           \
+                                          hipFuncAttributeMaxDynamicSharedMemorySize, (int)shmem));                      \
+        OMX_LAUNCH_TIMED((attn_step_kernel<128, 4, TT, kGuNV, false, true, true>), grid, block, shmem, s, a);            \
+        OMX_LAUNCH_CHECK();                                                                                              \
+        return 0;                                                                                                        \
+    }
 #define OMX_ATTN_STEP_CASE(DD, GG)                                                                                       \
     if (D == DD && gt == GG) {                                                                                           \
         const size_t shmem = ((size_t)kWaves * (64 / (DD / 8)) * GG * DD + 2 * kWaves * GG) * sizeof(float) +            \
                              (size_t)(GG + 1) * (DD / 8) * 16 + (size_t)nvw * 64 * 16 + (qo ? (size_t)nvw * 64 : 0) +    \
-                             (a.gu_gate ? kGuWords * sizeof(int) : 0);                                                   \
+                             (a.dn_w ? kDnWords * sizeof(int) : a.gu_gate ? kGuWords * sizeof(int) : 0);                 \
         if (a.gu_gate) {                            \
             if constexpr (DD == 128 && GG == 4) {                                                                        \
+                static_assert(kDnLdsBytes <= kWaves * 4 * 4 * 128 * 4, "the down phase lives in the split-merge area");  \
+                if (a.dn_w && a.trace) OMX_ATTN_LAUNCH_DN(true)                                                          \
+                if (a.dn_w) OMX_ATTN_LAUNCH_DN(false)                                                                    \
                 if (a.trace) OMX_ATTN_LAUNCH_GU(true)                                                                    \
                 OMX_ATTN_LAUNCH_GU(false)                                                                                \
             }                                                                                                            \
@@ -830,6 +1076,7 @@
     OMX_ATTN_STEP_CASE(128, 1) OMX_ATTN_STEP_CASE(128, 2) OMX_ATTN_STEP_CASE(128, 4) OMX_ATTN_STEP_CASE(128, 8)
     OMX_ATTN_STEP_CASE(64, 1) OMX_ATTN_STEP_CASE(64, 2) OMX_ATTN_STEP_CASE(64, 4) OMX_ATTN_STEP_CASE(64, 8)
 #undef OMX_ATTN_STEP_CASE
+#undef OMX_ATTN_LAUNCH_DN
 #undef OMX_ATTN_LAUNCH_GU
 #undef OMX_ATTN_LAUNCH
     return set_error("decode attention: head_dim %d unsupported (64 or 128)", D);
diff --git a/ominix-mlx_amd/csrc/engine.hip b/ominix-mlx_amd/csrc/engine.hip
--- a/ominix-mlx_amd/csrc/engine.hip
+++ b/ominix-mlx_amd/csrc/engine.hip
@@ -112,7 +112,7 @@
     }
     if (dev_alloc(m, &m->rope_cur, (size_t)D) || dev_alloc(m, &m->attn_gran, attn_step_ws_granules(m->H, D)) ||
         dev_alloc(m, &m->attn_xg, (size_t)m->H * D / 2 + 8) || dev_alloc(m, &m->chain_gran, (size_t)c.hidden_size / 2 + 8) ||
-        dev_alloc(m, &m->gateup_gran, (size_t)c.hidden_size / 2 + 8))
+        dev_alloc(m, &m->gateup_gran, (size_t)c.hidden_size / 2 + 8) || dev_alloc(m, &m->act_gran, (size_t)m->I / 2 + 8))
         return 1;
     if (dev_alloc(m, &m->step_seq, 16) || dev_alloc(m, &m->wait_abort, 16)) return 1;
     {
@@ -697,11 +697,18 @@
                 if (chain && l > 0 && l < L && k == KC_QKV) continue;
                 const bool gateup = l < L && !engine && !hybrid && attention_takes_gateup(m, l);
                 if (gateup && k == KC_GATE_UP) continue;
+                const bool down = gateup && chain && attention_takes_down(m, l);
+                if (down && k == KC_DOWN) continue;
                 OMX_HIP_CHECK(hipEventElapsedTime(&ms, ev[i], ev[i + 1]));
                 if (gateup && k == KC_ATTN) {
                     const double attn_bytes = 2.0 * m->Hkv * m->cfg.head_dim * (st.pos + 1) + o_bytes;
-                    sum[KC_GATE_UP] += ms * 1e3 * (gu_bytes / (gu_bytes + attn_bytes));
-                    ms *= (float)(attn_bytes / (gu_bytes + attn_bytes));
+                    const double all_bytes = gu_bytes + attn_bytes + (down ? down_bytes + qkv_bytes : 0.0);
+                    sum[KC_GATE_UP] += ms * 1e3 * (gu_bytes / all_bytes);
+                    if (down) {
+                        sum[KC_DOWN] += ms * 1e3 * (down_bytes / all_bytes);
+                        sum[KC_QKV] += ms * 1e3 * (qkv_bytes / all_bytes);
+                    }
+                    ms *= (float)(attn_bytes / all_bytes);
                 }
                 if (chain && l < L - 1 && k == KC_DOWN) {
                     sum[KC_QKV] += ms * 1e3 * (qkv_bytes / (qkv_bytes + down_bytes));
diff --git a/ominix-mlx_amd/csrc/engine_model.hpp b/ominix-mlx_amd/csrc/engine_model.hpp
--- a/ominix-mlx_amd/csrc/engine_model.hpp
+++ b/ominix-mlx_amd/csrc/engine_model.hpp
@@ -133,6 +133,7 @@
     uint64_t* attn_xg = nullptr;
     uint64_t* chain_gran = nullptr;
     uint64_t* gateup_gran = nullptr;
+    uint64_t* act_gran = nullptr;
     int attn_chunk = 0, attn_nsplit = 0, graph_tk_max = 0;
     unsigned long long* attn_trace = nullptr;
     bf16_t* verify_logits = nullptr;
@@ -239,6 +240,7 @@
 bool any_layer_takes_oproj(omx_qwen3 m);
 bool down_takes_qkv(omx_qwen3 m);
 bool attention_takes_gateup(omx_qwen3 m, int layer);
+bool attention_takes_down(omx_qwen3 m, int layer);
 int step_engine_mode(omx_qwen3 m);
 bool step_engine_takes(omx_qwen3 m);
 int step_aql_mode(omx_qwen3 m);
diff --git a/ominix-mlx_amd/csrc/engine_step.hip b/ominix-mlx_amd/csrc/engine_step.hip
--- a/ominix-mlx_amd/csrc/engine_step.hip
+++ b/ominix-mlx_amd/csrc/engine_step.hip
@@ -239,12 +239,19 @@
     return attn_step_gateup_ok(m->H, m->Hkv, c.head_dim, m->attn_nsplit, c.hidden_size, m->I);
 }
 
+bool attention_takes_down(omx_qwen3 m, int layer) {
+    const bool off = env_off("OMX_ATTN_DOWN");
+    const omx_qwen3_config& c = m->cfg;
+    if (off || !m->act_gran || layer + 1 >= c.num_hidden_layers || !attention_takes_gateup(m, layer) || !down_takes_qkv(m)) return false;
+    return attn_step_down_ok(c.hidden_size, m->I, (m->H + 2 * m->Hkv) * c.head_dim);
+}
+
 static bool peer_fused_fits(omx_qwen3 m, int N, int K) {
     return m->peer_dev != nullptr && gemv_grid(N, K, EPI_F32, 0) <= 2 * m->cus;
 }
 
 static int enqueue_attention(omx_qwen3 m, int l, hipStream_t s, const bf16_t* resid = nullptr, bf16_t* out = nullptr, float* out_f32 = nullptr,
-                             bool gateup = false) {
+                             bool gateup = false, bool down = false) {
     const omx_qwen3_config& c = m->cfg;
     const int D = c.head_dim;
     const LayerW& L = m->layers[l];
@@ -279,6 +286,14 @@
         a.gu_gate = L.gate; a.gu_up = L.up; a.gu_norm_w = L.post_ln; a.gu_out = m->act; a.gu_rows = m->I;
         a.hg = m->gateup_gran;
     }
+    if (down) {
+        const LayerW& Ln = m->layers[l + 1];
+        a.dn_w = L.down; a.dn_out = const_cast<bf16_t*>(resid);
+        a.ag = m->act_gran; a.rg = m->chain_gran;
+        a.nq_w0 = Ln.q; a.nq_w1 = Ln.k; a.nq_w2 = Ln.v;
+        a.nq_n0 = m->H * D; a.nq_n1 = m->Hkv * D; a.nq_rows = (m->H + 2 * m->Hkv) * D;
+        a.nq_norm_w = Ln.in_ln; a.nq_bias = Ln.qkv_bias; a.nq_out = m->qkv;
+    }
     return launch_attn_step(a, D, s);
 }
 
@@ -536,7 +551,9 @@
         const bool fused_o = attention_takes_oproj(m, l);
         time_next_launch(m, l, KC_ATTN);
         const bool gateup = fused_o && !tp && !pending && attention_takes_gateup(m, l);
-        if (enqueue_attention(m, l, s, fused_o ? h : nullptr, fused_o && !tp ? hn : nullptr, fused_o && tp ? m->partial_a : nullptr, gateup)) return 1;
+        const bool down = gateup && chain && attention_takes_down(m, l);
+        if (enqueue_attention(m, l, s, fused_o ? h : nullptr, fused_o && !tp ? hn : nullptr, fused_o && tp ? m->partial_a : nullptr, gateup, down)) return 1;
+        if (down) continue;
         if (fused_o && tp) {
             if (allreduce_sum(m, m->partial_a, hd)) return 1;
             pending = m->partial_a;
diff --git a/ominix-mlx_amd/engine.py b/ominix-mlx_amd/engine.py
--- a/ominix-mlx_amd/engine.py
+++ b/ominix-mlx_amd/engine.py
@@ -571,10 +571,10 @@
         return dict(zip(self.KERNEL_CLASSES, (float(v) for v in us)))
 
     def step_forms(self) -> dict:
-        f = (c_int * 6)()
+        f = (c_int * 7)()
         check(lib.omx_qwen3_debug_step_forms(self._h, f))
         return {"down_qkv": bool(f[0]), "attn_oproj": bool(f[1]), "step_engine": int(f[2]), "down_qkv_gave_up": bool(f[3]),
-                "attn_gateup": bool(f[4]), "attn_gateup_gave_up": bool(f[5])}
+                "attn_gateup": bool(f[4]), "attn_gateup_gave_up": bool(f[5]), "attn_down": bool(f[6])}
 
     def raise_give_up(self) -> None:
         check(lib.omx_qwen3_debug_raise_give_up(self._h))
```

New measurement: 354.5, median of 6. 1.01x the previous value.
